# xiaochuanle/hifimeth

Measured on AMD Instinct MI355X. Metric: cytosine sites/sec (CpG+CHG+CHH), higher is better.
Workload: dtype f16x3+f32acc

## Files before the change

### hifimeth_amd/_lib.py

```python
from __future__ import annotations

import ctypes as C
import os
import subprocess

HERE = os.path.dirname(os.path.abspath(__file__))
LIB_PATH = os.environ.get("HM_LIB_PATH") or os.path.join(HERE, "libhifimeth_hip.so")
CSRC = os.path.join(HERE, "csrc")
WEIGHTS_DIR = os.path.join(HERE, "weights")


class hm_call_t(C.Structure):
    _fields_ = [("read_id", C.c_int32), ("qoff", C.c_int32), ("strand", C.c_uint8), ("ctx", C.c_uint8),
                ("scaled_prob", C.c_uint8), ("reserved", C.c_uint8), ("p", C.c_float)]


class hm_read_t(C.Structure):
    _fields_ = [("read_id", C.c_int32), ("l_qseq", C.c_int32), ("flag", C.c_int32), ("width", C.c_uint8 * 4),
                ("seq4", C.c_void_p), ("kin", C.c_void_p * 4)]


class hm_timing_t(C.Structure):
    _fields_ = [("prep_ms", C.c_double), ("scan_ms", C.c_double), ("emit_ms", C.c_double), ("window_ms", C.c_double),
                ("front_ms", C.c_double * 3), ("tail_ms", C.c_double * 3),
                ("prep_launches", C.c_int64), ("scan_launches", C.c_int64), ("emit_launches", C.c_int64),
                ("window_launches", C.c_int64), ("front_launches", C.c_int64 * 3), ("tail_launches", C.c_int64 * 3),
                ("front_sites", C.c_int64 * 3), ("window_sites", C.c_int64),
                ("pack_ms", C.c_double), ("empty_ms", C.c_double),
                ("pack_launches", C.c_int64), ("empty_launches", C.c_int64),
                ("trunk_ms", C.c_double * 3), ("edge_ms", C.c_double * 3),
                ("trunk_launches", C.c_int64 * 3), ("edge_launches", C.c_int64 * 3),
                ("trunk_positions", C.c_int64 * 3),
                ("trunk_list_steps", C.c_int64 * 3), ("trunk_const_steps", C.c_int64 * 3),
                ("group_bases", C.c_int64), ("group_bytes", C.c_int64), ("tail_strip_passes", C.c_int64)]


HM_ABI_VERSION = 5


def build(force: bool = False) -> str:
    if force:
        subprocess.check_call(["make", "-C", CSRC, "clean"], stdout=subprocess.DEVNULL)
    subprocess.check_call(["make", "-C", CSRC], stdout=subprocess.DEVNULL)
    return LIB_PATH


_lib = None


def lib():
    global _lib
    if _lib is not None:
        return _lib
    if not os.path.exists(LIB_PATH):
        raise ImportError(f"{LIB_PATH} is missing: run `python -c 'import __graft_entry__ as g; g.build()'` "
                          "(hifimeth_amd has no CPU fallback)")
    try:
        import torch
    except ImportError:
        pass
    L = C.CDLL(LIB_PATH)
    vp, i32, i64, cp = C.c_void_p, C.c_int32, C.c_int64, C.c_char_p
    sig = {
        "hm_create": (C.c_int, [C.POINTER(vp), cp, C.c_int, C.c_int]),
        "hm_destroy": (None, [vp]),
        "hm_last_error": (cp, [vp]),
        "hm_set_option": (C.c_int, [vp, cp, i64]),
        "hm_submit_read": (C.c_int, [vp, i32, i32, i32, vp, vp, C.c_int, vp, C.c_int, vp, C.c_int, vp, C.c_int]),
        "hm_clear": (C.c_int, [vp]),
        "hm_upload": (C.c_int, [vp]),
        "hm_run": (C.c_int, [vp]),
        "hm_sync": (C.c_int, [vp]),
        "hm_num_sites": (i64, [vp, C.c_int]),
        "hm_fetch": (i64, [vp, vp, i64]),
        "hm_flush": (C.c_int, [vp]),
        "hm_drain": (i64, [vp, vp, i64]),
        "hm_batch_begin": (vp, [vp]),
        "hm_batch_submit_read": (C.c_int, [vp, i32, i32, i32, vp, vp, C.c_int, vp, C.c_int, vp, C.c_int, vp, C.c_int]),
        "hm_batch_submit_reads": (i64, [vp, vp, i64, C.c_int, vp]),
        "hm_trunk_mask_for_reads": (C.c_int, [vp, i64, C.c_int]),
        "hm_batch_staged_bases": (i64, [vp]),
        "hm_batch_enqueue": (C.c_int, [vp]),
        "hm_batch_done": (C.c_int, [vp]),
        "hm_batch_wait": (i64, [vp, C.POINTER(vp)]),
        "hm_batch_num_sites": (i64, [vp, C.c_int]),
        "hm_batch_release": (C.c_int, [vp]),
        "hm_scan_sites": (i64, [vp, C.c_int, vp, vp, vp, i64]),
        "hm_site_logits": (i64, [vp, C.c_int, vp, i64]),
        "hm_windows": (C.c_int, [vp, C.c_int, i64, i64, vp]),
        "hm_cnn_logits": (C.c_int, [vp, C.c_int, vp, i64, vp, vp, vp]),
        "hm_debug_layer": (i64, [vp, C.c_int, vp, C.c_int, vp, i64]),
        "hm_convert_model": (C.c_int, [cp, cp]),
        "hm_get_stamps": (C.c_int, [vp, C.POINTER(C.c_uint64), C.c_int]),
        "hm_get_timing": (C.c_int, [vp, C.POINTER(hm_timing_t)]),
        "hm_abi_version": (C.c_int, []),
        "hm_timing_size": (C.c_size_t, []),
        "hm_reset_timing": (C.c_int, [vp]),
        "hm_pileup_create": (C.c_int, [C.POINTER(vp), C.c_int]),
        "hm_pileup_destroy": (None, [vp]),
        "hm_pileup_last_error": (cp, [vp]),
        "hm_pileup_set_option": (C.c_int, [vp, cp, C.c_double]),
        "hm_pileup_set_reference": (C.c_int, [vp, i32, vp, vp]),
        "hm_pileup_use_planes": (C.c_int, [vp, vp, vp, vp]),
        "hm_pileup_planes": (C.c_int, [vp, C.POINTER(vp), C.POINTER(vp), C.POINTER(vp), C.POINTER(i64)]),
        "hm_pileup_submit_read": (C.c_int, [vp, C.c_uint32, i32, i32, i64, i32, i32, vp, i32, vp, i64, vp]),
        "hm_pileup_submit_read_hp": (C.c_int, [vp, C.c_uint32, i32, i32, i64, i32, i32, vp, i32, vp, i64, vp, i32]),
        "hm_pileup_submit_read_calls": (C.c_int, [vp, C.c_uint32, i32, i32, i64, i32, i32, vp, i32, vp, i64, vp, i32]),
        "hm_pileup_use_partition_planes": (C.c_int, [vp, i32, vp, vp]),
        "hm_pileup_partition_planes": (C.c_int, [vp, i32, C.POINTER(vp), C.POINTER(vp)]),
        "hm_pileup_run": (C.c_int, [vp]),
        "hm_pileup_num_records": (i64, [vp]),
        "hm_pileup_histograms": (C.c_int, [vp, vp]),
        "hm_pileup_fetch_records": (i64, [vp, vp, vp, vp, vp, i64]),
        "hm_pileup_label_histograms": (C.c_int, [vp, vp, i64, vp]),
        "hm_pileup_count": (C.c_int, [vp, vp]),
        "hm_pileup_fetch_loci": (i64, [vp, vp, vp, vp, i64, i64, i64, vp, i64]),
        "hm_pileup_fetch_asm": (i64, [vp, vp, vp, vp, vp, vp, i64, i64, i64, i32, vp, i64]),
        "hm_pileup_asm_histogram": (i64, [vp, vp, vp, vp, vp, vp, i64, i64, i64, i32, vp, vp, i64]),
        "hm_pileup_asm_bin_pvalues": (i64, [vp, vp, vp, i64]),
        "hm_asm_qvalues": (C.c_int, [vp, i64, vp, i64, vp, vp]),
        "hm_pileup_fetch_asm_q": (i64, [vp, vp, vp, vp, vp, vp, i64, i64, i64, i32, vp, i64, vp, vp, i64, vp, i64]),
        "hm_pileup_fetch_asm_regions": (i64, [vp, vp, vp, vp, vp, vp, i64, i64, i64, i32, i32, C.c_double, i64, i32, i32,
                                              C.POINTER(i64), vp, i64]),
        "hm_pileup_load_loci": (i64, [vp, i32, vp, i64]),
        "hm_pileup_group_sample": (C.c_int, [vp, i32]),
        "hm_pileup_load_sample_loci": (i64, [vp, vp, i64]),
        "hm_pileup_fetch_groups": (i64, [vp, i64, i64, i32, vp, i64]),
        "hm_pileup_group_planes": (C.c_int, [vp, i32, i64, i64, vp, vp]),
        "hm_group_qvalues": (C.c_int, [vp, i64, vp, vp]),
        "hm_dmr_fetch_regions": (i64, [vp, i64, i64, i32, i32, C.c_double, C.c_double, i64, i32, i32, C.POINTER(i64),
                                       C.POINTER(i64), vp, i64]),
        "hm_dmr_p_cutoff": (C.c_int, [vp, vp, i64, C.c_double, vp]),
        "hm_sample_geometry": (C.c_int, [vp]),
        "hm_sample_open": (C.c_int, [vp]),
        "hm_sample_load": (i64, [vp, vp, i64]),
        "hm_sample_fetch_sums": (i64, [vp, i64, i64, i32, vp]),
        "hm_sample_plane": (C.c_int, [vp, i32, i64, i64, vp]),
        "hm_sample_corr": (C.c_int, [vp, i64, vp, vp, vp]),
        "hm_sample_fetch_intervals": (i64, [vp, i64, i64, i32, i32, vp, vp, i64, vp]),
        "hm_sample_interval_test": (C.c_int, [vp, i64, i32, vp, i64, i32, vp]),
        "hm_sample_qvalues": (C.c_int, [vp, i64, vp]),
        "hm_pileup_control_sums": (C.c_int, [vp, vp, vp, vp, i64, i64, vp]),
        "hm_pileup_site_histogram": (i64, [vp, vp, vp, vp, i64, i64, i64, vp, vp, i64]),
        "hm_sites_table": (C.c_int, [vp, vp, vp, i64, vp, vp, vp, vp, vp]),
        "hm_pileup_fetch_sites": (i64, [vp, vp, vp, vp, i64, i64, i64, i32, vp, vp, vp, vp, vp, i64, vp, i64]),
        "hm_pileup_fetch_domains": (i64, [vp, vp, vp, vp, i64, i64, i64, i32, i64, i64, i64, i64, C.POINTER(i64), vp, i64]),
        "hm_pileup_fetch_domains_part": (i64, [vp, vp, vp, vp, i64, i64, i64, i32, i64, i64, i64, i64, i32, vp, vp, i64]),
        "hm_domain_scores": (C.c_int, [C.c_double, C.c_double, C.c_double, C.POINTER(i64), C.POINTER(i64), C.POINTER(i64)]),
        "hm_pileup_domain_sums": (i64, [vp, vp, vp, vp, i64, i64, i64, i32, i64, i64, i64, i64, C.POINTER(i64)]),
        "hm_pileup_domain_sums_part": (i64, [vp, vp, vp, vp, i64, i64, i64, i32, i64, i64, i64, i64, vp, C.POINTER(i64)]),
        "hm_domain_refit": (C.c_int, [C.POINTER(i64), C.c_double, C.POINTER(C.c_double), C.POINTER(C.c_double)]),
        "hm_pileup_num_pattern_records": (i64, [vp]),
        "hm_pileup_fetch_patterns": (i64, [vp, i64, i64, i64, vp, i64]),
        "hm_pattern_stats": (C.c_int, [vp, vp]),
        "hm_pileup_fetch_bedmethyl": (i64, [vp, i32, i64, i64, i64, vp, i64]),
        "hm_pileup_fetch_linkage": (i64, [vp, i64, vp, i64]),
        "hm_linkage_stats": (C.c_int, [vp, vp]),
        "hm_pileup_fetch_readpos": (i64, [vp, i64, vp, i64]),
        "hm_pileup_readpos_histograms": (i64, [vp, vp, i64]),
        "hm_pileup_add_readpos": (C.c_int, [vp, vp, i64]),
        "hm_readpos_stats": (C.c_int, [vp, vp]),
        "hm_region_geometry": (C.c_int, [vp]),
        "hm_pileup_fetch_regions": (C.c_int, [vp, vp, vp, vp, i64, i64, i64, i64, vp, vp, i64, vp]),
        "hm_pileup_fetch_metaplot": (C.c_int, [vp, vp, vp, vp, i64, i64, i64, i64, vp, vp, vp, vp, vp, i64, i32, i64, i32, vp,
                                               C.POINTER(i64)]),
        "hm_region_stats": (C.c_int, [vp, vp]),
        "hm_context_geometry": (C.c_int, [vp]),
        "hm_pileup_fetch_context": (i64, [vp, vp, vp, vp, i64, i64, i64, i64, i32, vp, i64]),
        "hm_pileup_fetch_context_path": (i64, [vp, vp, vp, vp, i64, i64, i64, i64, i32, i32, vp, i64]),
    }
    for name, (res, args) in sig.items():
        fn = getattr(L, name)
        fn.restype = res
        fn.argtypes = args
    L._hm_symbols = tuple(sig)
    if L.hm_abi_version() != HM_ABI_VERSION or L.hm_timing_size() != C.sizeof(hm_timing_t):
        raise ImportError(f"{LIB_PATH}: ABI {L.hm_abi_version()} / hm_timing_t {L.hm_timing_size()} bytes, this package expects "
                          f"{HM_ABI_VERSION} / {C.sizeof(hm_timing_t)}: rebuild (python -c 'import __graft_entry__ as g; g.build()')")
    _lib = L
    return L
```

### hifimeth_amd/caller.py

```python
from __future__ import annotations

import ctypes as C
from typing import Iterable, Optional

import numpy as np

from . import _lib

CPG, CHG, CHH = 0, 1, 2
CTX_NAMES = ("CpG", "CHG", "CHH")
KMER, FEATS = 401, 8

READ_DTYPE = np.dtype([("read_id", "<i4"), ("l_qseq", "<i4"), ("flag", "<i4"), ("width", "u1", 4), ("seq4", "<u8"),
                       ("kin", "<u8", 4)], align=True)
assert READ_DTYPE.itemsize == C.sizeof(_lib.hm_read_t)

CALL_DTYPE = np.dtype([("read_id", "<i4"), ("qoff", "<i4"), ("strand", "u1"), ("ctx", "u1"),
                       ("scaled_prob", "u1"), ("reserved", "u1"), ("p", "<f4")])
assert CALL_DTYPE.itemsize == C.sizeof(_lib.hm_call_t) == 16


class HifimethError(RuntimeError):
    pass


def parse_contexts(spec: str) -> int:
    mask = 0
    for tok in spec.lower().split(","):
        tok = tok.strip()
        if tok not in ("cpg", "chg", "chh"):
            raise ValueError(f"unknown methylation context '{tok}'")
        mask |= 1 << ("cpg", "chg", "chh").index(tok)
    return mask


def _vp(a: Optional[np.ndarray]):
    return None if a is None else a.ctypes.data_as(C.c_void_p)


class MethylationCaller:
    def __init__(self, model_dir: Optional[str] = None, contexts: str = "cpg,chg,chh", device: int = 0,
                 min_read_size: int = 1000, timing: bool = False):
        self._L = _lib.lib()
        self._h = C.c_void_p()
        self.ctx_mask = parse_contexts(contexts)
        rc = self._L.hm_create(C.byref(self._h), (model_dir or _lib.WEIGHTS_DIR).encode(), self.ctx_mask, device)
        if rc < 0:
            self._h = None
            raise HifimethError(f"hm_create failed ({rc}): {self._L.hm_last_error(None).decode()}")
        self.set_option("min_read_size", min_read_size)
        self.set_option("timing", int(timing))

    def close(self):
        if getattr(self, "_h", None):
            self._L.hm_destroy(self._h)
            self._h = None

    __del__ = close

    def __enter__(self):
        return self

    def __exit__(self, *exc):
        self.close()

    def _check(self, rc, what):
        if rc < 0:
            raise HifimethError(f"{what} failed ({rc}): {self._L.hm_last_error(self._h).decode()}")
        return rc

    def set_option(self, key: str, value: int):
        self._check(self._L.hm_set_option(self._h, key.encode(), int(value)), f"hm_set_option({key})")

    def new_sample(self):
        self.set_option("trunk", 2)

    @staticmethod
    def _read_args(read):
        arrs, widths = [], []
        for nm in ("fi", "fp", "ri", "rp"):
            a = getattr(read, nm)
            if a is not None:
                if len(a) != read.l_qseq:
                    a = None
                else:
                    a = np.ascontiguousarray(a)
                    if a.dtype.itemsize not in (1, 2):
                        raise ValueError("kinetics arrays must be uint8 (B:C) or uint16 (B:S)")
            arrs.append(a)
            widths.append(1 if a is None else a.dtype.itemsize)
        seq4 = np.ascontiguousarray(read.seq4, np.uint8)
        return (read.l_qseq, read.flag, _vp(seq4), _vp(arrs[0]), widths[0], _vp(arrs[1]), widths[1],
                _vp(arrs[2]), widths[2], _vp(arrs[3]), widths[3]), (seq4, arrs)

    def submit(self, read_id: int, read) -> bool:
        args, _keep = self._read_args(read)
        return bool(self._check(self._L.hm_submit_read(self._h, read_id, *args), "hm_submit_read"))

    def submit_all(self, reads: Iterable, first_id: int = 0) -> int:
        n = 0
        for i, r in enumerate(reads):
            n += self.submit(first_id + i, r)
        return n

    def clear(self):
        self._check(self._L.hm_clear(self._h), "hm_clear")

    def upload(self):
        self._check(self._L.hm_upload(self._h), "hm_upload")

    def run(self):
        self._check(self._L.hm_run(self._h), "hm_run")

    def sync(self):
        self._check(self._L.hm_sync(self._h), "hm_sync")

    def num_sites(self, ctx: int = 3) -> int:
        return self._check(self._L.hm_num_sites(self._h, ctx), "hm_num_sites")

    def fetch(self) -> np.ndarray:
        self.sync()
        n = self.num_sites(3)
        out = np.empty(n, CALL_DTYPE)
        got = self._check(self._L.hm_fetch(self._h, _vp(out), n), "hm_fetch")
        return out[:got]

    def call(self, reads: Iterable, first_id: int = 0) -> np.ndarray:
        self.clear()
        self.submit_all(reads, first_id)
        self.upload()
        self.run()
        out = self.fetch()
        self.clear()
        return out

    def begin_batch(self) -> "Batch":
        h = self._L.hm_batch_begin(self._h)
        if not h:
            raise HifimethError(f"hm_batch_begin failed: {self._L.hm_last_error(self._h).decode()}")
        return Batch(self, h)

    def stream(self, slabs: Iterable, on_batch=None) -> int:
        inflight, total, k_done = [], 0, 0

        def collect(b):
            nonlocal total, k_done
            calls = b.wait()
            total += len(calls)
            if on_batch is not None:
                on_batch(k_done, b, calls)
            k_done += 1
            b.release()

        for slab in slabs:
            b = self.begin_batch()
            if isinstance(slab, ReadBlock):
                b.submit_block(slab, self.stage_threads)
            else:
                b.submit_all(slab)
            b.enqueue()
            inflight.append(b)
            while len(inflight) > 1 and (inflight[0].done() or len(inflight) >= self.max_inflight):
                collect(inflight.pop(0))
        while inflight:
            collect(inflight.pop(0))
        return total

    max_inflight = 3
    stage_threads = 4

    def scan_sites(self, ctx: int):
        self.sync()
        n = self.num_sites(ctx)
        rid, qoff, strand = np.empty(n, np.int32), np.empty(n, np.int32), np.empty(n, np.uint8)
        self._check(self._L.hm_scan_sites(self._h, ctx, _vp(rid), _vp(qoff), _vp(strand), n), "hm_scan_sites")
        return rid, qoff, strand

    def site_logits(self, ctx: int) -> np.ndarray:
        self.sync()
        n = self.num_sites(ctx)
        out = np.empty((n, 2), np.float32)
        got = self._check(self._L.hm_site_logits(self._h, ctx, _vp(out), n), "hm_site_logits")
        return out[:got]

    def windows(self, ctx: int, first: int = 0, n: Optional[int] = None, fetch: bool = True):
        if n is None:
            n = self.num_sites(ctx) - first
        out = np.empty((n, KMER, FEATS), np.float32) if fetch else None
        self._check(self._L.hm_windows(self._h, ctx, first, n, _vp(out)), "hm_windows")
        return out

    def cnn_logits(self, ctx: int, windows: np.ndarray):
        w = np.ascontiguousarray(windows, np.float32).reshape(-1, KMER, FEATS)
        n = w.shape[0]
        lg, p, ml = np.empty((n, 2), np.float32), np.empty(n, np.float32), np.empty(n, np.uint8)
        self._check(self._L.hm_cnn_logits(self._h, ctx, _vp(w), n, _vp(lg), _vp(p), _vp(ml)), "hm_cnn_logits")
        return lg, p, ml

    def debug_layer(self, ctx: int, window: np.ndarray, layer: int) -> np.ndarray:
        w = np.ascontiguousarray(window, np.float32).reshape(KMER, FEATS)
        out = np.empty(197 * 128, np.float32)
        n = self._check(self._L.hm_debug_layer(self._h, ctx, _vp(w), layer, _vp(out), out.size), "hm_debug_layer")
        chans = (8, 128, 128, 128, 96, 96, 96, 64, 64)[layer]
        return out[:n].reshape(-1, chans).copy()

    def stamps(self) -> list:
        buf = (C.c_uint64 * 256)()
        n = self._check(self._L.hm_get_stamps(self._h, buf, 256), "hm_get_stamps")
        return [int(buf[i]) for i in range(n)]

    def timing(self, reset: bool = False) -> dict:
        t = _lib.hm_timing_t()
        self._check(self._L.hm_get_timing(self._h, C.byref(t)), "hm_get_timing")
        d = {k: (list(getattr(t, k)) if hasattr(getattr(t, k), "__len__") else getattr(t, k)) for k, _ in t._fields_}
        if reset:
            self._L.hm_reset_timing(self._h)
        return d


def trunk_mask_for_reads(block: "ReadBlock", ctx_mask: int = 7) -> int:
    rc = _lib.lib().hm_trunk_mask_for_reads(block.desc.ctypes.data_as(C.c_void_p), len(block.desc), ctx_mask)
    if rc < 0:
        raise HifimethError(f"hm_trunk_mask_for_reads failed ({rc})")
    return rc


class ReadBlock:

    def __init__(self, reads, first_id: int = 0):
        self.reads = list(reads)
        self.desc = np.zeros(len(self.reads), READ_DTYPE)
        self._keep = []
        for i, r in enumerate(self.reads):
            d = self.desc[i]
            d["read_id"], d["l_qseq"], d["flag"] = first_id + i, r.l_qseq, r.flag
            seq4 = np.ascontiguousarray(r.seq4, np.uint8)
            d["seq4"] = seq4.ctypes.data
            self._keep.append(seq4)
            for k, nm in enumerate(("fi", "fp", "ri", "rp")):
                a = getattr(r, nm)
                if a is None or len(a) != r.l_qseq:
                    d["kin"][k], d["width"][k] = 0, 1
                    continue
                a = np.ascontiguousarray(a)
                if a.dtype.itemsize not in (1, 2):
                    raise ValueError("kinetics arrays must be uint8 (B:C) or uint16 (B:S)")
                d["kin"][k], d["width"][k] = a.ctypes.data, a.dtype.itemsize
                self._keep.append(a)

    def __len__(self):
        return len(self.reads)


class Batch:

    def __init__(self, mc: MethylationCaller, handle):
        self._mc, self._L, self._h = mc, mc._L, C.c_void_p(handle)

    def submit(self, read_id: int, read) -> bool:
        args, _keep = MethylationCaller._read_args(read)
        return bool(self._mc._check(self._L.hm_batch_submit_read(self._h, read_id, *args), "hm_batch_submit_read"))

    def submit_all(self, reads: Iterable, first_id: int = 0) -> int:
        n = 0
        for i, r in enumerate(reads):
            n += self.submit(first_id + i, r)
        return n

    def submit_block(self, block: "ReadBlock", threads: int = 4) -> int:
        rc = self._L.hm_batch_submit_reads(self._h, block.desc.ctypes.data_as(C.c_void_p), len(block.desc), threads, None)
        return self._mc._check(rc, "hm_batch_submit_reads")

    def staged_bases(self) -> int:
        return self._L.hm_batch_staged_bases(self._h)

    def enqueue(self):
        self._mc._check(self._L.hm_batch_enqueue(self._h), "hm_batch_enqueue")

    def done(self) -> bool:
        return bool(self._mc._check(self._L.hm_batch_done(self._h), "hm_batch_done"))

    def num_sites(self, ctx: int = 3) -> int:
        return self._mc._check(self._L.hm_batch_num_sites(self._h, ctx), "hm_batch_num_sites")

    def wait(self) -> np.ndarray:
        ptr = C.c_void_p()
        n = self._mc._check(self._L.hm_batch_wait(self._h, C.byref(ptr)), "hm_batch_wait")
        if n == 0:
            return np.empty(0, CALL_DTYPE)
        buf = (C.c_char * (n * CALL_DTYPE.itemsize)).from_address(ptr.value)
        return np.frombuffer(buf, CALL_DTYPE, n)

    def release(self):
        if self._h:
            self._L.hm_batch_release(self._h)
            self._h = None
```

### hifimeth_amd/csrc/hm_edge.h

```cpp
#pragma once
#include "hm_convh.h"

namespace hm {

namespace {

constexpr int TR_RS = 136;
constexpr int TR_WRS = 8;

__device__ __forceinline__ uint4 feature_row(int b, uint32_t k, int view) {
    uint4 row = make_uint4(0u, 0u, 0u, 0u);
    if (b < 0) return row;
    if (view) {
        if (b < 4) b = 3 - b;
        k = (k >> 16) | (k << 16);
    }
    row.x = b == 0 ? 0x3c00u : b == 1 ? 0x3c000000u : 0u;
    row.y = b == 2 ? 0x3c00u : b == 3 ? 0x3c000000u : 0u;
    half_t f[4];
#pragma unroll
    for (int c = 0; c < 4; ++c) {
        const uint32_t tt = (k >> (8 * c)) & 255u;
        f[c] = (half_t)((float)((int)(((tt & 63u) + 64u) << (tt >> 6)) - 64) * 0.03125f);
    }
    row.z = (uint32_t)__builtin_bit_cast(uint16_t, f[0]) | ((uint32_t)__builtin_bit_cast(uint16_t, f[1]) << 16);
    row.w = (uint32_t)__builtin_bit_cast(uint16_t, f[2]) | ((uint32_t)__builtin_bit_cast(uint16_t, f[3]) << 16);
    return row;
}

template <int K1>
struct EdgeGeo {
    static constexpr int L1 = (KMER + 2 - K1) / 2 + 1, L2 = (L1 - 1) / 2 + 1, L3 = (L2 - 1) / 2 + 1;
    static constexpr bool PAD2 = 2 * (L2 - 1) + 1 == L1, PAD3 = 2 * (L3 - 1) + 1 == L2, PAD4 = 2 * (C4_LEN - 1) + 1 == L3;
    static constexpr int R1 = -201 + 2 * (2 * (L2 - 1) - 1), R2 = -203 + 4 * (2 * (L3 - 1) - 1), R3 = -207 + 8 * (2 * (C4_LEN - 1) - 1);
    static constexpr int LEFT = -199;
    static constexpr int X_LEFT = -201, X_RIGHT = -201 + 2 * (L1 - 1);
};
static_assert(EdgeGeo<11>::PAD2 && EdgeGeo<11>::PAD3 && !EdgeGeo<11>::PAD4 && EdgeGeo<11>::R1 == 189 && EdgeGeo<11>::R2 == 185 && EdgeGeo<11>::R3 == 169, "k1 = 11 edge geometry");
static_assert(!EdgeGeo<13>::PAD2 && !EdgeGeo<13>::PAD3 && EdgeGeo<13>::PAD4 && EdgeGeo<13>::R1 == 185 && EdgeGeo<13>::R2 == 177 && EdgeGeo<13>::R3 == 169, "k1 = 13 edge geometry");


constexpr int EG_S = 32, EG_M = 2 * EG_S;
constexpr int EG_XROWS = 16;
constexpr int EG_OP = EG_M * 3 * TR_RS;
constexpr int EG_SP = EG_M * TR_RS;
constexpr int EG_XH = EG_M * EG_XROWS * TR_WRS;

struct EdgeSite {
    int64_t bo;
    int64_t vrow;
    int L, off, view, valid;
};

enum { SRC_ZERO = 0, SRC_SPEC = 1, SRC_MAP = 2 };
struct TapSrc {
    int kind, delta;
};

template <int K1>
__device__ __forceinline__ TapSrc tap_source(int layer, int side, int tap) {
    using G = EdgeGeo<K1>;
    if (side == 0) return tap == 0 ? TapSrc{SRC_ZERO, 0} : tap == 1 ? TapSrc{SRC_SPEC, 0} : TapSrc{SRC_MAP, G::LEFT};
    const bool pad = layer == 2 ? G::PAD2 : layer == 3 ? G::PAD3 : G::PAD4;
    const int r = layer == 2 ? G::R1 : layer == 3 ? G::R2 : G::R3, step = layer == 2 ? 2 : layer == 3 ? 4 : 8;
    if (pad) return tap == 0 ? TapSrc{SRC_MAP, r} : tap == 1 ? TapSrc{SRC_SPEC, 0} : TapSrc{SRC_ZERO, 0};
    return tap == 0 ? TapSrc{SRC_MAP, r} : tap == 1 ? TapSrc{SRC_MAP, r + step} : TapSrc{SRC_SPEC, 0};
}

struct EpiSpec {
    half_t* hi;
    half_t* lo;
    const float* __restrict__ bias;
    __device__ __forceinline__ void operator()(int m, int col, const f32x4& acc) const {
        half4 h, l;
        split4(acc, h, l);
        *reinterpret_cast<half4*>(hi + m * TR_RS + col) = h;
        *reinterpret_cast<half4*>(lo + m * TR_RS + col) = l;
    }
};

struct EpiSpecC1 {
    half_t* hi;
    half_t* lo;
    const float* __restrict__ bias;
    float4 c0, c1;
    __device__ __forceinline__ void operator()(int m, int col, const f32x4& acc) const {
        const float4 c = m >= EG_S ? c1 : c0;
        half4 h, l;
        split4(f32x4{acc[0] - c.x, acc[1] - c.y, acc[2] - c.z, acc[3] - c.w}, h, l);
        *reinterpret_cast<half4*>(hi + m * TR_RS + col) = h;
        *reinterpret_cast<half4*>(lo + m * TR_RS + col) = l;
    }
};

struct EpiEdgeOut {
    half_t* __restrict__ out;
    const float* __restrict__ bias;
    int nvalid;
    __device__ __forceinline__ void operator()(int m, int col, const f32x4& acc) const {
        const int side = m >= EG_S, site = m - side * EG_S;
        if (site < nvalid) {
            half4 h, l;
            split4(acc, h, l);
            half_t* o = out + (size_t)site * (4 * C4_CH) + side * (2 * C4_CH) + col;
            *reinterpret_cast<half4*>(o) = h;
            *reinterpret_cast<half4*>(o + C4_CH) = l;
        }
    }
};


}

}
```

### hifimeth_amd/csrc/hm_edge2.hip

```cpp
#include "hm_edge.h"
#ifdef HM_TRUNK_STAMP
#include "hm_stamp.h"
namespace hm { __device__ unsigned long long g_edge2_stamp[8][16]; }
extern "C" int hm_debug_edge2_stamps(unsigned long long* out, int reset) {
    if (out && hipMemcpyFromSymbol(out, HIP_SYMBOL(hm::g_edge2_stamp), sizeof(hm::g_edge2_stamp)) != hipSuccess) return -1;
    if (reset) {
        static unsigned long long z[8][16];
        if (hipMemcpyToSymbol(HIP_SYMBOL(hm::g_edge2_stamp), z, sizeof(z)) != hipSuccess) return -1;
    }
    return 0;
}
#endif

namespace hm {

namespace {

constexpr int E2_NW = 8;
constexpr int E2_MROWS = 3 * EG_S;
constexpr int E2_SLACK = 256;
constexpr int E2_MRS = 264;
constexpr int E2_MSET = E2_MROWS * E2_MRS + E2_SLACK;
constexpr int E2_SPLANE = EG_M * TR_RS;
constexpr int E2_XRS = EG_XROWS * TR_WRS + 8;
constexpr int E2_XH = EG_M * E2_XRS;
constexpr int E2_AHEAD = 2;
static_assert(E2_MRS * 2 == 33 * 16, "a map-set row is 33 sixteen-byte chunks (32 + pad)");

template <int I, int N, class F>
__device__ __forceinline__ void e2_for(F&& f) {
    if constexpr (I < N) {
        f(std::integral_constant<int, I>{});
        e2_for<I + 1, N>(f);
    }
}

__device__ __forceinline__ void e2_barrier() {
    __builtin_amdgcn_fence(__ATOMIC_RELEASE, "workgroup", "local");
    __builtin_amdgcn_s_barrier();
    __builtin_amdgcn_fence(__ATOMIC_ACQUIRE, "workgroup", "local");
}
template <int N>
__device__ __forceinline__ void e2_vmwait() {
    __builtin_amdgcn_s_waitcnt(0x0F70 | (N & 15) | ((N >> 4) << 14));
}

template <int K1, int LAYER>
struct E2L {
    using G = EdgeGeo<K1>;
    static constexpr bool PAD = LAYER == 2 ? G::PAD2 : LAYER == 3 ? G::PAD3 : G::PAD4;
    static constexpr int R = LAYER == 2 ? G::R1 : LAYER == 3 ? G::R2 : G::R3, STEP = LAYER == 2 ? 2 : LAYER == 3 ? 4 : 8;
    static constexpr int COUT = LAYER == 4 ? C4_CH : 128;
    static constexpr int ROWS = PAD ? 2 * EG_S : 3 * EG_S;
    static constexpr int NI = (ROWS * 33 + 63) / 64;
    static constexpr int kind(int side, int tap) {
        if (side == 0) return tap == 0 ? SRC_ZERO : tap == 1 ? SRC_SPEC : SRC_MAP;
        if (PAD) return tap == 0 ? SRC_MAP : tap == 1 ? SRC_SPEC : SRC_ZERO;
        return tap == 2 ? SRC_SPEC : SRC_MAP;
    }
    static constexpr int map_j(int side, int tap) { return side == 1 && !PAD && tap == 1 ? 1 : 0; }
    static constexpr bool live(int side, int kb) { return kind(side, kb / 4) != SRC_ZERO; }
    static constexpr int nblocks() { int n = 0; for (int kb = 0; kb < 12; ++kb) n += live(1, kb) + live(0, kb); return n; }
    static constexpr int NB = nblocks();
    static constexpr int find(int b, bool want_side) {
        int n = 0;
        for (int kb = 0; kb < 12; ++kb)
            for (int s = 1; s >= 0; --s)
                if (live(s, kb) && n++ == b) return want_side ? s : kb;
        return -1;
    }
    static constexpr int side_of(int b) { return find(b, true); }
    static constexpr int kb_of(int b) { return find(b, false); }
    static constexpr int dies_at(int b) { return b + 1 < NB && kb_of(b + 1) == kb_of(b) ? -1 : kb_of(b); }
};
static_assert(E2L<13, 2>::NB == 20 && E2L<13, 4>::NB == 16 && E2L<11, 4>::NB == 20 && E2L<13, 2>::kb_of(4) == 4 && E2L<13, 2>::side_of(5) == 0 &&
              E2L<13, 2>::dies_at(4) == -1 && E2L<13, 2>::dies_at(5) == 4 && E2L<13, 4>::kb_of(15) == 11 && E2L<11, 2>::NB == 16 && E2L<11, 2>::side_of(15) == 0 && E2L<11, 2>::kb_of(15) == 11,
              "edge layer schedules");

struct E2Site {
    int64_t vrow;
    int32_t off, L;
    int64_t bo;
    int32_t view, valid;
};

}

template <int K1>
__global__ __launch_bounds__(512) void edge2_kernel(SiteRange sr, const RInfo* __restrict__ rinfo, const uint8_t* __restrict__ bases,
                                                     const uint32_t* __restrict__ kin, CtxWeights W, TrunkMaps mp,
                                                     uint16_t* __restrict__ edge4, int32_t* __restrict__ e4row) {
    using G = EdgeGeo<K1>;
    constexpr int NW = E2_NW;
    const Site* sites;
    const int n_sites = resolve_sites(sr, sites);
    __shared__ __attribute__((aligned(16))) half_t smem[2 * E2_MSET + 2 * E2_SPLANE + E2_XH];
    __shared__ E2Site sinfo2[2][EG_S];
    __shared__ int32_t rowtab[2][3][E2_MROWS];
    half_t* mset = smem;
    half_t* sp_hi = smem + 2 * E2_MSET;
    half_t* sp_lo = sp_hi + E2_SPLANE;
    half_t* xb = sp_lo + E2_SPLANE;
    if ((int)blockIdx.x * EG_S >= n_sites) return;
    int tid = threadIdx.x, lane = tid & 63, wave = __builtin_amdgcn_readfirstlane(tid >> 6);
    int li = lane & 15, lk = lane >> 4;
    auto wf = [&](int i) { return reinterpret_cast<const half_t*>(W.wfrag_h[i]); };
    const uint32_t lds_mset = (uint32_t)(uintptr_t)(const __attribute__((address_space(3))) half_t*)mset;

    struct Desc {
        Site st;
        RInfo ri;
        int bs, valid;
    } nd;
    auto desc_a = [&](const int s0) __attribute__((always_inline)) {
        const int sc = min(s0, max(n_sites - 1, 0));
        const int nvalid = s0 < n_sites ? min(EG_S, n_sites - s0) : 0;
        const int t = tid & (EG_S - 1);
        nd.valid = t < nvalid;
        nd.st = sites[min(sc + t, max(n_sites - 1, 0))];
    };
    auto desc_b = [&]() __attribute__((always_inline)) { nd.ri = rinfo[nd.st.read_idx]; };
    auto desc_c = [&]() __attribute__((always_inline)) { nd.bs = bases[nd.ri.base_off + nd.st.qoff]; };
    auto desc_d = [&](const int s0, E2Site* si, int32_t (*rt)[E2_MROWS]) __attribute__((always_inline)) {
        if (tid < EG_S) {
            E2Site es;
            es.bo = nd.ri.base_off;
            es.L = nd.ri.len;
            es.view = nd.bs == 2;
            es.off = es.view ? nd.ri.len - 1 - nd.st.qoff : nd.st.qoff;
            es.vrow = (int64_t)es.view * mp.view_rows + nd.ri.map_off + TR_PAD;
            es.valid = nd.valid;
            si[tid] = es;
            if (es.valid) e4row[s0 + tid] = (int32_t)(es.vrow + es.off - 215);
        }
        if (tid < 3 * E2_MROWS) {
            const int l = tid / E2_MROWS, j = (tid - l * E2_MROWS) >> 5;
            const int view = nd.bs == 2, off = view ? nd.ri.len - 1 - nd.st.qoff : nd.st.qoff;
            const int r0 = l == 0 ? G::R1 : l == 1 ? G::R2 : G::R3, step = 2 << l;
            const int delta = j == 0 ? G::LEFT : r0 + (j - 1) * step;
            (&rt[0][0])[tid] = (int32_t)((int64_t)view * mp.view_rows + nd.ri.map_off + TR_PAD + off + delta);
        }
    };
    auto build_rows = [&](const E2Site* si, const int t, auto nt_, auto between) __attribute__((always_inline)) {
        constexpr int NT = decltype(nt_)::value, NR = EG_M * EG_XROWS / NT, PER = EG_XROWS / NR;
        static_assert(NR >= 1 && NR <= EG_XROWS && EG_XROWS % NR == 0, "a thread's rows lie in one pseudo-row");
        const int row = t / PER, t0 = (t - row * PER) * NR;
        const int side = row >= EG_S, site = row - side * EG_S;
        const E2Site es = si[site];
        uint32_t b[NR], k[NR];
        bool live[NR];
#pragma unroll
        for (int u = 0; u < NR; ++u) {
            const int tt = t0 + u;
            const int x = es.off + (side ? G::X_RIGHT : G::X_LEFT) + tt;
            const bool is_pad = side ? tt == K1 - 1 : tt == 0;
            live[u] = tt < K1 && !is_pad && x >= 0 && x < es.L;
            const int xc = min(max(x, 0), es.L - 1);
            const int64_t j = es.bo + (es.view ? es.L - 1 - xc : xc);
            b[u] = bases[j];
            k[u] = kin[j];
        }
        between();
#pragma unroll
        for (int u = 0; u < NR; ++u)
            *reinterpret_cast<uint4*>(xb + row * E2_XRS + (t0 + u) * TR_WRS) = feature_row(live[u] ? (int)b[u] : -1, k[u], es.view);
    };

    struct DmaSrc {
        int32_t rn;
        uint32_t ch;
    };
    auto dma_src = [&](auto ltag, const int32_t* rt, const int i) __attribute__((always_inline)) {
        using L = E2L<K1, decltype(ltag)::value>;
        const uint32_t c = (uint32_t)min(i, L::NI - 1) * 64u + (uint32_t)lane;
        const uint32_t row = (c * 1986u) >> 16;
        const uint32_t ch = min(c - 33u * row, 31u);
        return DmaSrc{rt[min(row, (uint32_t)(L::ROWS - 1))], ch};
    };
    auto dma_issue = [&](auto ltag, const DmaSrc& d, const int set, const int i) __attribute__((always_inline)) {
        using L = E2L<K1, decltype(ltag)::value>;
        const char* __restrict__ map = reinterpret_cast<const char*>(mp.e[decltype(ltag)::value - 2]);
        if (i < L::NI) {
            const char* src = map + (uint64_t)((uint32_t)d.rn * 32u + d.ch) * 16u;
            const uint32_t dst = __builtin_amdgcn_readfirstlane(lds_mset + (uint32_t)((set * E2_MSET) * 2 + i * 1024));
            uint32_t km;
            asm volatile(
                "s_mov_b32 %0, m0\n\t"
                "s_mov_b32 m0, %1\n\t"
                "s_nop 0\n\t"
                "global_load_lds_dwordx4 %2, off\n\t"
                "s_mov_b32 m0, %0"
                : "=&s"(km)
                : "s"(dst), "v"(src));
        }
    };
    auto dma_maps = [&](auto ltag, const int32_t* rt, const int set, const int w0, auto nw_) __attribute__((always_inline)) {
        using L = E2L<K1, decltype(ltag)::value>;
        constexpr int nw = decltype(nw_)::value;
#pragma unroll
        for (int t = 0; t < (L::NI + nw - 1) / nw; ++t) dma_issue(ltag, dma_src(ltag, rt, w0 + nw * t), set, w0 + nw * t);
    };
    using L2t = std::integral_constant<int, 2>;
    using L3t = std::integral_constant<int, 3>;
    using L4t = std::integral_constant<int, 4>;
    using NW8 = std::integral_constant<int, 8>;

    constexpr int KB1 = (2 * K1 + 3) / 4 * 4 * 8 / 32;
    struct Head1 {
        half8 w[KB1];
        float4 bz;
    };
    auto load_head1 = [&](Head1& h) __attribute__((always_inline)) {
        const char* wp = reinterpret_cast<const char*>(W.c1f) + (size_t)wave * (KB1 * 1024);
        const uint32_t lo = (uint32_t)lane * 16u;
#pragma unroll
        for (int kb = 0; kb < KB1; ++kb) h.w[kb] = *reinterpret_cast<const half8*>(wp + kb * 1024 + lo);
        const int col = wave * 16 + 4 * lk;
        h.bz = *reinterpret_cast<const float4*>(W.c1f_bias + col);
    };
    auto conv1 = [&](const Head1& h) __attribute__((always_inline)) {
        const float4 c0 = *reinterpret_cast<const float4*>(W.c1f_corr + wave * 16 + 4 * lk);
        const float4 c1 = *reinterpret_cast<const float4*>(W.c1f_corr + 128 + wave * 16 + 4 * lk);
        f32x4 acc[4];
#pragma unroll
        for (int i = 0; i < 4; ++i) acc[i] = f32x4{h.bz.x, h.bz.y, h.bz.z, h.bz.w};
        auto stack_off = [&](int kb) __attribute__((always_inline)) {
            int t = 4 * kb + lk;
            t = t >= 2 * K1 ? 0 : t >= K1 ? t - K1 : t;
            return t * TR_WRS;
        };
        const int a0 = li * E2_XRS;
        half8 x[2][4];
#pragma unroll
        for (int i = 0; i < 4; ++i) x[0][i] = *reinterpret_cast<const half8*>(xb + a0 + i * (16 * E2_XRS) + stack_off(0));
#pragma unroll
        for (int kb = 0; kb < KB1; ++kb) {
            if (kb + 1 < KB1) {
                const int bo = stack_off(kb + 1);
#pragma unroll
                for (int i = 0; i < 4; ++i) x[(kb + 1) & 1][i] = *reinterpret_cast<const half8*>(xb + a0 + i * (16 * E2_XRS) + bo);
            }
#pragma unroll
            for (int i = 0; i < 4; ++i) acc[i] = __builtin_amdgcn_mfma_f32_16x16x32_f16(h.w[kb], x[kb & 1][i], acc[i], 0, 0, 0);
        }
        const EpiSpecC1 epi{sp_hi, sp_lo, nullptr, c0, c1};
#pragma unroll
        for (int i = 0; i < 4; ++i) epi(i * 16 + li, wave * 16 + 4 * lk, acc[i]);
    };

    struct LW {
        half8 w[12][2];
        float4 bz;
    };
    auto wptr = [&](auto ltag) __attribute__((always_inline)) {
        constexpr int LAYER = decltype(ltag)::value;
        const int nt = LAYER == 4 ? min(wave, C4_CH / 16 - 1) : wave;
        return reinterpret_cast<const char*>(wf(LAYER - 1)) + (size_t)nt * (12 * 128 * 16);
    };
    auto load_kb = [&](auto ltag, auto kb_, LW& lw) __attribute__((always_inline)) {
        constexpr int LAYER = decltype(ltag)::value, kb = decltype(kb_)::value;
        const char* wp = wptr(ltag) + kb * 2048;
        const uint32_t lo = (uint32_t)lane * 16u;
        lw.w[kb][0] = *reinterpret_cast<const half8*>(wp + lo);
        lw.w[kb][1] = *reinterpret_cast<const half8*>(wp + 1024 + lo);
        if constexpr (kb == 0) lw.bz = *reinterpret_cast<const float4*>(W.bias[LAYER - 1] + (LAYER == 4 ? min(wave, C4_CH / 16 - 1) : wave) * 16 + 4 * lk);
    };
    auto layer = [&](auto ltag, const LW& lw, const half_t* mx, f32x4 (&acc)[4], auto slide, auto job) __attribute__((always_inline)) {
        constexpr int LAYER = decltype(ltag)::value;
        using L = E2L<K1, LAYER>;
#pragma unroll
        for (int i = 0; i < 4; ++i) acc[i] = f32x4{lw.bz.x, lw.bz.y, lw.bz.z, lw.bz.w};
        const int a0 = li * TR_RS + 8 * lk;
        const int am = li * E2_MRS + 8 * lk;
        constexpr int LA = 2, NX = LA + 1;
        half8 x[NX][2][2];
        auto reads = [&](auto b_) __attribute__((always_inline)) {
            constexpr int b = decltype(b_)::value, side = L::side_of(b), kb = L::kb_of(b), tap = kb / 4, q = kb % 4;
            constexpr int kind = L::kind(side, tap);
            static_assert(kind != SRC_ZERO, "live taps only");
#pragma unroll
            for (int i = 0; i < 2; ++i) {
                if constexpr (kind == SRC_MAP) {
                    const int o = am + ((2 * side + i) * 16 + 32 * L::map_j(side, tap)) * E2_MRS + 32 * q;
                    x[b % NX][i][0] = *reinterpret_cast<const half8*>(mx + o);
                    x[b % NX][i][1] = *reinterpret_cast<const half8*>(mx + o + 128);
                } else {
                    const int o = a0 + ((2 * side + i) * 16) * TR_RS + 32 * q;
                    x[b % NX][i][0] = *reinterpret_cast<const half8*>(sp_hi + o);
                    x[b % NX][i][1] = *reinterpret_cast<const half8*>(sp_lo + o);
                }
            }
        };
        e2_for<0, E2_AHEAD>(slide);
        e2_for<0, LA>(reads);
        e2_for<0, L::NB>([&](auto b_) __attribute__((always_inline)) {
            constexpr int b = decltype(b_)::value, side = L::side_of(b), kb = L::kb_of(b);
            if constexpr (b + LA < L::NB) reads(std::integral_constant<int, (b + LA < L::NB ? b + LA : 0)>{});
            job(b_);
#pragma unroll
            for (int pr = 0; pr < 3; ++pr)
#pragma unroll
                for (int i = 0; i < 2; ++i)
                    acc[2 * side + i] = __builtin_amdgcn_mfma_f32_16x16x32_f16(lw.w[kb][pr == 2 ? 1 : 0], x[b % NX][i][pr == 1 ? 1 : 0],
                                                                               acc[2 * side + i], 0, 0, 0);
            constexpr int dead = L::dies_at(b);
            constexpr bool sl = dead >= 0 && dead + E2_AHEAD < 12;
            if constexpr (sl) slide(std::integral_constant<int, (sl ? dead + E2_AHEAD : 0)>{});
            {
                constexpr int NRD = b + LA < L::NB ? 4 : 0;
#pragma unroll
                for (int r = 0; r < NRD; ++r) {
                    __builtin_amdgcn_sched_group_barrier(0x008, 1, 0);
                    __builtin_amdgcn_sched_group_barrier(0x100, 1, 0);
                }
                if (sl) {
                    __builtin_amdgcn_sched_group_barrier(0x008, 1, 0);
                    __builtin_amdgcn_sched_group_barrier(0x020, 2, 0);
                }
            }
            __builtin_amdgcn_sched_barrier(0);
        });
    };

#ifdef HM_TRUNK_STAMP
    unsigned long long ets[16], eacc[16] = {};
    unsigned long long en_it = 0, e_prev = 0;
    const bool est_on = blockIdx.x == 0;
#define ETS(i) do { if (est_on) ets[i] = hm_stamp(); } while (0)
#else
#define ETS(i)
#endif

    Head1 h1;
    LW lw;
    {
        const int s0 = blockIdx.x * EG_S;
        desc_a(s0);
        desc_b();
        desc_c();
        desc_d(s0, sinfo2[0], rowtab[0]);
        load_head1(h1);
        __syncthreads();
        build_rows(sinfo2[0], tid, std::integral_constant<int, NW * 64>{}, [] {});
        e2_vmwait<0>();
        dma_maps(L2t{}, rowtab[0][0], 0, wave, NW8{});
        e2_vmwait<0>();
    }
    int cur = 0, sel = 0;
    for (int s0 = blockIdx.x * EG_S; s0 < n_sites; s0 += gridDim.x * EG_S) {
        const int nvalid = min(EG_S, n_sites - s0);
        const E2Site* si_next = sinfo2[cur ^ 1];
        const half_t* mA = mset + (size_t)sel * E2_MSET;
        const half_t* mB = mset + (size_t)(sel ^ 1) * E2_MSET;
        tid = threadIdx.x;
        asm volatile("" : "+v"(tid));
        lane = tid & 63, wave = __builtin_amdgcn_readfirstlane(tid >> 6), li = lane & 15, lk = lane >> 4;
        e2_barrier();
        ETS(0);
#ifdef HM_TRUNK_STAMP
        if (est_on && e_prev) eacc[9] += ets[0] - e_prev;
#endif
        const int sn = s0 + gridDim.x * EG_S;
        desc_a(sn);
        e2_for<0, 12>([&](auto k_) __attribute__((always_inline)) { load_kb(L2t{}, k_, lw); });
        conv1(h1);
        ETS(1);
        e2_vmwait<0>();
        e2_barrier();
        ETS(2);
        f32x4 acc[4];
        desc_b();
        {
            LW ln;
            DmaSrc ds;
            layer(L2t{}, lw, mA, acc, [&](auto k_) __attribute__((always_inline)) { load_kb(L3t{}, k_, ln); },
                  [&](auto b_) __attribute__((always_inline)) {
                      constexpr int b = decltype(b_)::value, NP = (E2L<K1, 3>::NI + NW - 1) / NW;
                      static_assert(NP < E2L<K1, 2>::NB, "the pieces fit the layer's blocks");
                      if constexpr (b >= 1 && b - 1 < NP) dma_issue(L3t{}, ds, sel ^ 1, wave + NW * (b - 1));
                      if constexpr (b < NP) ds = dma_src(L3t{}, rowtab[cur][1], wave + NW * b);
                  });
            ETS(3);
            e2_vmwait<0>();
            e2_barrier();
            ETS(4);
            const EpiSpec epi{sp_hi, sp_lo, nullptr};
#pragma unroll
            for (int i = 0; i < 4; ++i) epi(i * 16 + li, wave * 16 + 4 * lk, acc[i]);
            lw = ln;
        }
        e2_barrier();
        ETS(5);
        desc_c();
        {
            LW ln;
            DmaSrc ds;
            layer(L3t{}, lw, mB, acc, [&](auto k_) __attribute__((always_inline)) { load_kb(L4t{}, k_, ln); },
                  [&](auto b_) __attribute__((always_inline)) {
                      constexpr int b = decltype(b_)::value, NP = (E2L<K1, 4>::NI + NW - 1) / NW;
                      static_assert(NP < E2L<K1, 3>::NB, "the pieces fit the layer's blocks");
                      if constexpr (b >= 1 && b - 1 < NP) dma_issue(L4t{}, ds, sel, wave + NW * (b - 1));
                      if constexpr (b < NP) ds = dma_src(L4t{}, rowtab[cur][2], wave + NW * b);
                  });
            ETS(6);
            e2_vmwait<0>();
            e2_barrier();
            ETS(7);
            const EpiSpec epi{sp_hi, sp_lo, nullptr};
#pragma unroll
            for (int i = 0; i < 4; ++i) epi(i * 16 + li, wave * 16 + 4 * lk, acc[i]);
            desc_d(sn, sinfo2[cur ^ 1], rowtab[cur ^ 1]);
            lw = ln;
        }
        e2_barrier();
        ETS(8);
        if (wave >= C4_CH / 16) {
            build_rows(si_next, tid - 64 * (C4_CH / 16), std::integral_constant<int, 128>{}, [&]() __attribute__((always_inline)) { load_head1(h1); });
        } else {
            DmaSrc ds;
            constexpr int NWC = C4_CH / 16;
            layer(L4t{}, lw, mA, acc, [&](auto k_) __attribute__((always_inline)) {
                if constexpr (decltype(k_)::value == 11) load_head1(h1);
            }, [&](auto b_) __attribute__((always_inline)) {
                constexpr int b = decltype(b_)::value, NP = (E2L<K1, 2>::NI + NWC - 1) / NWC;
                static_assert(NP < E2L<K1, 4>::NB, "the pieces fit the layer's blocks");
                if constexpr (b >= 1 && b - 1 < NP) dma_issue(L2t{}, ds, sel ^ 1, wave + NWC * (b - 1));
                if constexpr (b < NP) ds = dma_src(L2t{}, rowtab[cur ^ 1][0], wave + NWC * b);
            });
            const EpiEdgeOut epi{reinterpret_cast<half_t*>(edge4) + (size_t)s0 * (4 * C4_CH), nullptr, nvalid};
#pragma unroll
            for (int i = 0; i < 4; ++i) epi(i * 16 + li, wave * 16 + 4 * lk, acc[i]);
        }
        ETS(9);
        e2_vmwait<0>();
        cur ^= 1;
        sel ^= 1;
#ifdef HM_TRUNK_STAMP
        if (est_on) {
            for (int i = 0; i < 9; ++i) eacc[i] += ets[i + 1] - ets[i];
            e_prev = ets[9];
            ++en_it;
        }
#endif
    }
#ifdef HM_TRUNK_STAMP
    if (est_on && (threadIdx.x & 63) == 0) {
        for (int i = 0; i < 10; ++i) atomicAdd(&g_edge2_stamp[threadIdx.x >> 6][i], eacc[i]);
        atomicAdd(&g_edge2_stamp[threadIdx.x >> 6][10], en_it);
    }
#endif
#undef ETS
}

void launch_edge2(hipStream_t st, int k1, const SiteRange& sr, const RInfo* rinfo, const uint8_t* bases, const uint32_t* kin,
                  const CtxWeights& w, const TrunkMaps& maps, uint16_t* edge4, int32_t* e4row, int grid) {
    if (sr.cap <= 0) return;
    const dim3 g(sr.totals ? grid : max(1, min((sr.cap + EG_S - 1) / EG_S, grid))), b(512);
    if (k1 == 11) hipLaunchKernelGGL(edge2_kernel<11>, g, b, 0, st, sr, rinfo, bases, kin, w, maps, edge4, e4row);
    else hipLaunchKernelGGL(edge2_kernel<13>, g, b, 0, st, sr, rinfo, bases, kin, w, maps, edge4, e4row);
}

}
```

### hifimeth_amd/csrc/hm_engine.cpp

```cpp
#include <hip/hip_runtime.h>

#include <algorithm>
#include <atomic>
#include <cmath>
#include <condition_variable>
#include <cstdio>
#include <cstring>
#include <memory>
#include <mutex>
#include <string>
#include <thread>
#include <vector>

#include "../../include/hifimeth_hip.h"
#include "hm_device.h"
#include "hm_host.h"
#include "hm_kernels.h"
#include "hm_weights.h"

using namespace hm;

namespace {

thread_local std::string g_create_error;

enum Kind { K_PREP, K_SCAN, K_EMIT, K_PACK, K_WINDOW, K_FRONT, K_TAIL, K_TRUNK, K_EDGE, K_TAILG };

struct TimedSpan {
    int kind, ctx;
    int64_t off, cap;
    Event a, b;
};

struct DeviceModel {
    bool loaded = false;
    int k1 = 0;
    DevBuf params;
    CtxWeights w{};
};

}

struct hm_batch {
    hm_engine* e = nullptr;
    int id = 0;
    enum State { FREE, STAGING, QUEUED } state = FREE;
    bool uploaded = false, ran = false, have_totals = false, have_calls = false;
    Stream s_io;
    Event ev_in, ev_comp, ev_out;

    PinnedArr<uint8_t> slab;
    PinnedArr<ReadDesc> reads;
    PinnedArr<Chunk> chunks;
    PinnedArr<RInfo> rinfo;
    PinnedArr<TrunkTile> tiles;
    PinnedArr<int32_t> tcost;
    struct Group {
        int chunk_lo, chunk_hi, tile_lo, tile_hi;
        int64_t bases, rows;
        int cost_lo;
    };
    std::vector<Group> groups;
    int64_t total_bases = 0;

    DevBuf d_raw, d_reads, d_chunks, d_rinfo, d_tiles, d_tcost, d_bases, d_kin, d_sctx, d_counts, d_offs, d_totals, d_err;
    DevBuf d_usites, d_utag, d_csites, d_opos, d_logits, d_p, d_ml, d_calls;
    Pinned<int32_t> h_totals;
    Pinned<int32_t> h_err;
    PinnedArr<hm_call_t> h_calls;
    int32_t totals[TOT_COUNT] = {};

    std::vector<TimedSpan> spans;

    ~hm_batch() {
        if (s_io) (void)hipStreamSynchronize(s_io);
    }
};

namespace {

struct GroupBufs {
    DevBuf d_map[3], d_e4, d_edge4, d_e4row, d_rowlist;
    DevBuf d_x6;
    DevBuf d_mark, d_ccnt, d_order, d_okey;
    DevBuf d_odst;
    DevBuf d_x8;
    DevBuf d_dump;
    int64_t bytes() const {
        const DevBuf* all[] = {&d_map[0], &d_map[1], &d_map[2], &d_e4, &d_edge4, &d_e4row, &d_rowlist, &d_x6, &d_mark, &d_ccnt, &d_order, &d_okey, &d_odst, &d_x8, &d_dump};
        static_assert(sizeof(GroupBufs) == sizeof all / sizeof *all * sizeof(DevBuf), "a member of GroupBufs is missing from bytes()");
        int64_t sum = 0;
        for (const DevBuf* d : all) sum += (int64_t)d->cap;
        return sum;
    }
};

}

struct hm_engine {
    int device = 0;
    int num_cu = 256;
    int ctx_mask = 7;
    int min_read_size = 1000;
    int64_t sub_batch = 65536;
    int front_waves = 8;
    int precision = 1;
    int conv3_w16 = 0;
    int max_slots = 3;
    int trunk = 2;
    int trunk_impl = 3;
    int edge_impl = 1;
    int tail_impl = 3;
    int64_t tail_slice = int64_t(1) << 21;
    int trunk_mask_auto = -1;
    int64_t group_bases = 0;
    std::atomic<int64_t> group_bases_eff{0};
    bool stamps_on = false;
    std::vector<unsigned long long> stamp_sum;
    bool timing = false;
    std::string err;

    std::mutex mu;
    std::mutex order_mu;
    std::condition_variable cv;
    hm_timing_t acc{};
    int64_t x6_sites = 0;

    Stream stream;
    std::vector<Event> pool;
    DevBuf d_act4, d_win, d_dbg, d_stamps, d_zeros;
    GroupBufs grp;
    DeviceModel model[3];
    std::vector<std::unique_ptr<hm_batch>> slots;

    ~hm_engine() {
        (void)hipSetDevice(device);
        if (stream) (void)hipStreamSynchronize(stream);
    }
};

namespace {

constexpr int64_t GROUP_BYTES_PER_BASE = (3 * 2 * 512 + 2 * 384 + 768 + 4 + 8 + 2 * 4 + 8 + 4 + TAIL_STRIP_HANDOVER_BYTES) * 5 / 4;

int64_t effective_group_bases(hm_engine* e) {
    if (e->group_bases > 0) return e->group_bases;
    if (const int64_t have = e->group_bases_eff.load(std::memory_order_relaxed)) return have;
    size_t free_b = 0, total_b = 0;
    int64_t gb = int64_t(2) << 20;
    int prev = -1;
    (void)hipGetDevice(&prev);
    if (hipSetDevice(e->device) == hipSuccess && hipMemGetInfo(&free_b, &total_b) == hipSuccess && free_b > 0) {
        gb = (int64_t)(free_b / 4) / GROUP_BYTES_PER_BASE;
        gb = std::min<int64_t>(gb, int64_t(16) << 20);
        gb = std::max<int64_t>(gb >> 20 << 20, int64_t(1) << 20);
    }
    if (prev >= 0 && prev != e->device) (void)hipSetDevice(prev);
    int64_t none = 0;
    if (!e->group_bases_eff.compare_exchange_strong(none, gb, std::memory_order_relaxed)) gb = none;
    return gb;
}

constexpr int TILE_COST = 8, TILE_COST_CONST = 1;
void add_read_tiles(hm_engine* e, hm_batch* b, int ridx, int l_qseq) {
    if (b->groups.empty() || b->groups.back().rows >= effective_group_bases(e)) {
        b->groups.push_back(hm_batch::Group{(int)b->chunks.n, (int)b->chunks.n, (int)b->tiles.n, (int)b->tiles.n, 0, 0, (int)b->tcost.n});
        b->tcost.push_back(0);
    }
    hm_batch::Group& g = b->groups.back();
    const int ntile = (l_qseq + 2 * TR_PAD + TR_OWN - 1) / TR_OWN;
    b->rinfo.push_back(RInfo{b->total_bases, l_qseq, (int32_t)g.rows});
    for (int t = 0; t < ntile; ++t) {
        const int u0 = -TR_PAD + t * TR_OWN;
        b->tiles.push_back(TrunkTile{ridx, u0});
        b->tcost.push_back(b->tcost.p[b->tcost.n - 1] + (t == 0 ? 2 * TILE_COST_CONST : u0 >= l_qseq ? TILE_COST_CONST : TILE_COST));
    }
    for (int st = 0; st < l_qseq; st += CHUNK) b->chunks.push_back(Chunk{ridx, st});
    g.rows += (int64_t)ntile * TR_OWN + TR_SLACK;
    if (2 * g.rows >= (int64_t(1) << 27)) throw HipErr{hipErrorInvalidValue, "a read group's maps exceed 2^27 rows (group_bases too large)"};
    g.bases += l_qseq;
    g.chunk_hi = (int)b->chunks.n;
    g.tile_hi = (int)b->tiles.n;
}

int fail(hm_engine* e, int code, const std::string& msg) {
    if (e) {
        std::lock_guard<std::mutex> lk(e->mu);
        e->err = msg;
    } else {
        g_create_error = msg;
    }
    return code;
}

int fail_hip(hm_engine* e, const HipErr& h) {
    return fail(e, HM_EDEVICE, hip_error_text(h));
}

template <class Body>
auto guarded(hm_engine* e, Body&& body) -> decltype(body()) {
    return hip_guard(e->device, [e](const HipErr& h) { return fail_hip(e, h); }, body);
}

Event get_event(hm_engine* e) {
    Event ev;
    {
        std::lock_guard<std::mutex> lk(e->mu);
        if (!e->pool.empty()) {
            ev = std::move(e->pool.back());
            e->pool.pop_back();
            return ev;
        }
    }
    HIP_TRY(hipEventCreate(&ev.h));
    return ev;
}

struct Span {
    hm_engine* e;
    std::vector<TimedSpan>* sink;
    TimedSpan ts{};
    bool on;
    Span(hm_engine* eng, std::vector<TimedSpan>* out, int kind, int ctx = 0, int64_t off = 0, int64_t cap = 0)
        : e(eng), sink(out), on(eng->timing && out) {
        if (!on) return;
        ts.kind = kind;
        ts.ctx = ctx;
        ts.off = off;
        ts.cap = cap;
        ts.a = get_event(e);
        ts.b = get_event(e);
        HIP_TRY(hipEventRecord(ts.a, e->stream));
    }
    void end() {
        if (!on) return;
        HIP_TRY(hipEventRecord(ts.b, e->stream));
        sink->push_back(std::move(ts));
        on = false;
    }
};

void collect_timing(hm_engine* e, std::vector<TimedSpan>& spans, const int32_t* totals) {
    if (!spans.empty() && totals) {
        std::lock_guard<std::mutex> lk(e->mu);
        for (int c = 0; c < 3; ++c) e->acc.trunk_list_steps[c] += totals[TOT_LIST_STEPS + c];
        for (int c = 0; c < 3; ++c) e->acc.trunk_const_steps[c] += totals[TOT_CONST_STEPS + c];
        e->acc.tail_strip_passes += totals[TOT_STRIP_PASSES];
    }
    for (auto& s : spans) {
        float ms = 0.f;
        HIP_TRY(hipEventElapsedTime(&ms, s.a, s.b));
        std::lock_guard<std::mutex> lk(e->mu);
        hm_timing_t& t = e->acc;
        const int64_t n = totals ? std::clamp<int64_t>((int64_t)totals[s.ctx] - s.off, 0, s.cap) : s.cap;
        switch (s.kind) {
        case K_PREP: t.prep_ms += ms; ++t.prep_launches; break;
        case K_SCAN: t.scan_ms += ms; ++t.scan_launches; break;
        case K_EMIT: t.emit_ms += ms; ++t.emit_launches; break;
        case K_PACK: t.pack_ms += ms; ++t.pack_launches; break;
        case K_WINDOW: t.window_ms += ms; ++t.window_launches; t.window_sites += s.cap; break;
        case K_TRUNK: t.trunk_ms[s.ctx] += ms; ++t.trunk_launches[s.ctx]; t.trunk_positions[s.ctx] += s.cap; break;
        case K_EDGE: t.edge_ms[s.ctx] += ms; ++t.edge_launches[s.ctx]; break;
        case K_TAILG: t.tail_ms[s.ctx] += ms; ++t.tail_launches[s.ctx]; break;
        case K_FRONT:
            if (n > 0) { t.front_ms[s.ctx] += ms; ++t.front_launches[s.ctx]; t.front_sites[s.ctx] += n; }
            else { t.empty_ms += ms; ++t.empty_launches; }
            break;
        default:
            if (n > 0) { t.tail_ms[s.ctx] += ms; ++t.tail_launches[s.ctx]; }
            else { t.empty_ms += ms; ++t.empty_launches; }
            break;
        }
        e->pool.push_back(std::move(s.a));
        e->pool.push_back(std::move(s.b));
    }
    spans.clear();
}

void upload_model(hm_engine* e, int ctx, const HostModel& hmw) {
    DeviceModel& dm = e->model[ctx];
    PackedModel pk = pack_model(hmw);
    dm.params.reserve(pk.blob.size() * sizeof(float));
    HIP_TRY(hipMemcpy(dm.params.p, pk.blob.data(), pk.blob.size() * sizeof(float), hipMemcpyHostToDevice));
    const float* base = dm.params.as<float>();
    for (int i = 0; i < 9; ++i) {
        dm.w.wfrag[i] = base + pk.wfrag_off[i];
        dm.w.bias[i] = base + pk.bias_off[i];
    }
    dm.w.fc2_w = base + pk.fc2_w_off;
    dm.w.fc2_b = base + pk.fc2_b_off;
    dm.w.bn = reinterpret_cast<const BnTables*>(base + pk.bn_off);
    for (int i = 0; i < 9; ++i) dm.w.wfrag_h[i] = reinterpret_cast<const uint16_t*>(base + pk.wfrag_h_off[i]);
    dm.w.bn_h = reinterpret_cast<const BnTablesH*>(base + pk.bn_h_off);
    dm.w.c1f = reinterpret_cast<const uint16_t*>(base + pk.c1f_off);
    dm.w.c1f_bias = base + pk.c1f_bias_off;
    dm.w.c1f_corr = base + pk.c1f_corr_off;
    dm.w.k1 = hmw.k1;
    dm.k1 = hmw.k1;
    dm.loaded = true;
}

size_t align16(size_t x) { return (x + 15) & ~size_t(15); }

void accumulate_stamps(hm_engine* e) {
    const int ns = front_stamp_slots();
    const size_t n = (size_t)e->num_cu * 8 * ns;
    std::vector<unsigned long long> h(n);
    HIP_TRY(hipStreamSynchronize(e->stream));
    HIP_TRY(hipMemcpy(h.data(), e->d_stamps.p, n * sizeof(unsigned long long), hipMemcpyDeviceToHost));
    HIP_TRY(hipMemset(e->d_stamps.p, 0, n * sizeof(unsigned long long)));
    e->stamp_sum.resize((size_t)ns * 8, 0);
    for (size_t i = 0; i < n; ++i) e->stamp_sum[i % ((size_t)ns * 8)] += h[i];
}

void launch_cnn_pair(hm_engine* e, std::vector<TimedSpan>* spans, int ctx, const SiteRange& sr, const hm_batch* b,
                     const float* windows, float* logits, float* p, uint8_t* ml, float* dbg, int dbg_layer) {
    const DeviceModel& dm = e->model[ctx];
    const ReadDesc* reads = b ? b->d_reads.as<ReadDesc>() : nullptr;
    const uint8_t* bases = b ? b->d_bases.as<uint8_t>() : nullptr;
    const uint32_t* kin = b ? b->d_kin.as<uint32_t>() : nullptr;
    {
        Span sp(e, spans, K_FRONT, ctx, sr.off, sr.cap);
        if (e->precision >= 1)
            launch_front_h(e->stream, dm.k1, sr, reads, bases, kin, windows, dm.w, e->d_act4.as<float>(), e->num_cu, dbg,
                           dbg_layer, e->stamps_on ? e->d_stamps.as<unsigned long long>() : nullptr);
        else
            launch_front(e->stream, dm.k1, sr, reads, bases, kin, windows, dm.w, e->d_act4.as<float>(), e->num_cu, dbg,
                         dbg_layer, e->front_waves, e->stamps_on ? e->d_stamps.as<unsigned long long>() : nullptr);
        if (e->stamps_on) accumulate_stamps(e);
        sp.end();
    }
    {
        Span sp(e, spans, K_TAIL, ctx, sr.off, sr.cap);
        if (e->precision >= 1)
            launch_tail_h(e->stream, e->d_act4.as<float>(), sr, dm.w, logits, p, ml, e->num_cu, dbg, dbg_layer);
        else
            launch_tail(e->stream, e->d_act4.as<float>(), sr, dm.w, logits, p, ml, e->num_cu, dbg, dbg_layer);
        sp.end();
    }
}

void run_cnn_windows(hm_engine* e, int ctx, const float* windows, int64_t n, float* logits, float* p, uint8_t* ml,
                     float* dbg, int dbg_layer) {
    const int64_t sb = e->sub_batch;
    e->d_act4.reserve((size_t)std::min<int64_t>(std::max<int64_t>(n, 1), sb) * ACT4_FLOATS * sizeof(float));
    std::vector<TimedSpan> spans;
    for (int64_t off = 0; off < n; off += sb) {
        const int m = (int)std::min<int64_t>(sb, n - off);
        const SiteRange sr{nullptr, nullptr, ctx, 0, m};
        launch_cnn_pair(e, e->timing ? &spans : nullptr, ctx, sr, nullptr, windows + (size_t)off * KMER * FEATS,
                        logits + 2 * off, p + off, ml + off, dbg, dbg_layer);
    }
    HIP_TRY(hipGetLastError());
    HIP_TRY(hipStreamSynchronize(e->stream));
    collect_timing(e, spans, nullptr);
}

hm_batch* new_slot(hm_engine* e, int id) {
    std::unique_ptr<hm_batch> b(new hm_batch());
    b->e = e;
    b->id = id;
    HIP_TRY(hipStreamCreateWithFlags(&b->s_io.h, hipStreamNonBlocking));
    for (Event* ev : {&b->ev_in, &b->ev_comp, &b->ev_out}) HIP_TRY(hipEventCreateWithFlags(&ev->h, hipEventDisableTiming));
    b->h_totals.alloc(TOT_COUNT);
    b->h_err.alloc();
    b->d_totals.reserve(TOT_COUNT * sizeof(int32_t));
    b->d_err.reserve(sizeof(int32_t));
    HIP_TRY(hipMemset(b->d_err.p, 0, sizeof(int32_t)));
    HIP_TRY(hipMemset(b->d_totals.p, 0, TOT_COUNT * sizeof(int32_t)));
    hm_batch* raw = b.get();
    e->slots.push_back(std::move(b));
    return raw;
}

void reset_staging(hm_batch* b) {
    b->slab.n = 0;
    b->reads.n = 0;
    b->chunks.n = 0;
    b->rinfo.n = 0;
    b->tiles.n = 0;
    b->tcost.n = 0;
    b->groups.clear();
    b->total_bases = 0;
    b->uploaded = b->ran = b->have_totals = b->have_calls = false;
    memset(b->totals, 0, sizeof b->totals);
}


int check_read(hm_engine* e, const hm_read_t& r, int64_t tb, const char* who, const char* full) {
    if (r.l_qseq < 0) return fail(e, HM_EINVAL, std::string(who) + ": negative read length");
    if (r.l_qseq < e->min_read_size) return 0;
    if (r.l_qseq == 0) return 0;
    if (!r.kin[0] || !r.kin[1] || !r.kin[2] || !r.kin[3]) return 0;
    if (!r.seq4) return fail(e, HM_EINVAL, std::string(who) + ": seq4 is NULL");
    for (int k = 0; k < 4; ++k)
        if (r.width[k] != 1 && r.width[k] != 2) return fail(e, HM_EINVAL, "kinetics element width must be 1 (B:C) or 2 (B:S)");
    if (tb + (int64_t)r.l_qseq + 4 >= (int64_t(1) << 31)) return fail(e, HM_ENOMEM, std::string(who) + ": batch would exceed 2^31 bases; " + full);
    return 1;
}

int64_t padded_bases(int32_t l_qseq) { return ((int64_t)l_qseq + 3) & ~int64_t(3); }

struct SlabCopy {
    const void* src;
    size_t off, bytes;
};

void place_read(hm_batch* b, const hm_read_t& r, SlabCopy* copies) {
    const size_t L = (size_t)r.l_qseq;
    auto place = [&](const void* src, size_t bytes) {
        const int64_t off = (int64_t)b->slab.n;
        *copies++ = SlabCopy{src, (size_t)off, bytes};
        b->slab.n += align16(bytes);
        return off;
    };
    ReadDesc rd{};
    rd.off_seq = place(r.seq4, (L + 1) / 2);
    rd.off_fi = place(r.kin[0], L * r.width[0]);
    rd.off_fp = place(r.kin[1], L * r.width[1]);
    rd.off_ri = place(r.kin[2], L * r.width[2]);
    rd.off_rp = place(r.kin[3], L * r.width[3]);
    rd.base_off = b->total_bases;
    rd.len = r.l_qseq;
    rd.flag = r.flag;
    rd.read_id = r.read_id;
    for (int k = 0; k < 4; ++k) rd.w[k] = r.width[k];
    const int ridx = (int)b->reads.n;
    b->reads.push_back(rd);
    add_read_tiles(b->e, b, ridx, r.l_qseq);
    b->total_bases += padded_bases(r.l_qseq);
}

int stage_read(hm_batch* b, int32_t read_id, int32_t l_qseq, int32_t flag, const uint8_t* seq4, const void* fi, int fi_w,
               const void* fp, int fp_w, const void* ri, int ri_w, const void* rp, int rp_w) {
    auto width = [](int w) { return (uint8_t)std::clamp(w, 0, 255); };
    const hm_read_t r{read_id, l_qseq, flag, {width(fi_w), width(fp_w), width(ri_w), width(rp_w)}, seq4, {fi, fp, ri, rp}};
    const int rc = check_read(b->e, r, b->total_bases, "hm_submit_read", "flush / queue it first");
    if (rc <= 0) return rc;
    return guarded(b->e, [&] {
        const size_t L = (size_t)l_qseq;
        const size_t need = align16((L + 1) / 2) + align16(L * fi_w) + align16(L * fp_w) + align16(L * ri_w) + align16(L * rp_w);
        if (b->slab.n + need > b->slab.cap) b->slab.reserve(std::max<size_t>((b->slab.n + need) * 2, size_t(64) << 20));
        SlabCopy copies[5];
        place_read(b, r, copies);
        for (const SlabCopy& c : copies) memcpy(b->slab.p + c.off, c.src, c.bytes);
        return 1;
    });
}

void enqueue_upload(hm_batch* b) {
    const size_t nr = b->reads.n, nc = b->chunks.n;
    b->d_raw.reserve(std::max<size_t>(b->slab.n, 16));
    b->d_reads.reserve(std::max<size_t>(nr, 1) * sizeof(ReadDesc));
    b->d_chunks.reserve(std::max<size_t>(nc, 1) * sizeof(Chunk));
    const size_t tb = (size_t)std::max<int64_t>(b->total_bases, 4);
    b->d_bases.reserve(tb);
    b->d_sctx.reserve(tb);
    b->d_kin.reserve(tb * sizeof(uint32_t));
    b->d_counts.reserve((nc + 1) * NCNT * sizeof(int32_t));
    b->d_offs.reserve((nc + 1) * NCNT * sizeof(int32_t));
    b->d_usites.reserve(tb * sizeof(USite));
    b->d_utag.reserve(tb);
    b->d_csites.reserve(tb * sizeof(Site));
    b->d_opos.reserve(tb * sizeof(int32_t));
    b->d_logits.reserve(tb * 2 * sizeof(float));
    b->d_p.reserve(tb * sizeof(float));
    b->d_ml.reserve(tb);
    b->d_calls.reserve(tb * sizeof(hm_call_t));
    if (b->slab.n) HIP_TRY(hipMemcpyAsync(b->d_raw.p, b->slab.p, b->slab.n, hipMemcpyHostToDevice, b->s_io));
    if (nr) HIP_TRY(hipMemcpyAsync(b->d_reads.p, b->reads.p, nr * sizeof(ReadDesc), hipMemcpyHostToDevice, b->s_io));
    if (nc) HIP_TRY(hipMemcpyAsync(b->d_chunks.p, b->chunks.p, nc * sizeof(Chunk), hipMemcpyHostToDevice, b->s_io));
    b->d_rinfo.reserve(std::max<size_t>(nr, 1) * sizeof(RInfo));
    b->d_tiles.reserve(std::max<size_t>(b->tiles.n, 1) * sizeof(TrunkTile));
    if (nr) HIP_TRY(hipMemcpyAsync(b->d_rinfo.p, b->rinfo.p, nr * sizeof(RInfo), hipMemcpyHostToDevice, b->s_io));
    if (b->tiles.n) HIP_TRY(hipMemcpyAsync(b->d_tiles.p, b->tiles.p, b->tiles.n * sizeof(TrunkTile), hipMemcpyHostToDevice, b->s_io));
    b->d_tcost.reserve(std::max<size_t>(b->tcost.n, 1) * sizeof(int32_t));
    if (b->tcost.n) HIP_TRY(hipMemcpyAsync(b->d_tcost.p, b->tcost.p, b->tcost.n * sizeof(int32_t), hipMemcpyHostToDevice, b->s_io));
    HIP_TRY(hipEventRecord(b->ev_in, b->s_io));
    b->uploaded = true;
    b->ran = b->have_totals = b->have_calls = false;
}

void run_trunk_path(hm_batch* b, std::vector<TimedSpan>* spans, int ctx_mask) {
    hm_engine* e = b->e;
    int64_t max_rows = 1, max_bases = 1;
    for (const auto& g : b->groups) {
        max_rows = std::max(max_rows, g.rows);
        max_bases = std::max(max_bases, g.bases);
    }
    for (int i = 0; i < 3; ++i) e->grp.d_map[i].reserve((size_t)max_rows * 2 * 256 * sizeof(uint16_t));
    e->grp.d_e4.reserve((size_t)max_rows * 2 * C4_CH * sizeof(float));
    e->grp.d_rowlist.reserve(std::max((size_t)(max_rows / TR_OWN + 1) * 2 * 3 * TR_OWN, trunk3_rowlist_bytes((max_rows / TR_OWN + 1) * 2)));
    e->grp.d_dump.reserve(trunk3_dump_bytes(e->num_cu));
    e->grp.d_edge4.reserve((size_t)max_bases * 2 * C4_CH * sizeof(float));
    e->grp.d_e4row.reserve((size_t)max_bases * sizeof(int32_t));
    if (e->tail_impl == 3 && e->precision >= 1 && (ctx_mask >> CHH & 1)) {
        e->grp.d_mark.reserve(tail_strip_mark_bytes(2 * max_rows));
        e->grp.d_ccnt.reserve(tail_strip_count_bytes(2 * max_rows));
        e->grp.d_order.reserve((size_t)max_bases * sizeof(int32_t));
        e->grp.d_okey.reserve((size_t)max_bases * sizeof(int32_t));
        e->grp.d_odst.reserve((size_t)max_bases * sizeof(int32_t));
        e->grp.d_x8.reserve(tail_strip_handover_bytes(max_bases));
    }
    if (!e->d_zeros.p) {
        e->d_zeros.reserve(1024);
        HIP_TRY(hipMemsetAsync(e->d_zeros.p, 0, 1024, e->stream));
    }
    const int32_t* offs = b->d_offs.as<int32_t>();
    for (const auto& g : b->groups) {
        const TrunkMaps maps{{e->grp.d_map[0].as<uint16_t>(), e->grp.d_map[1].as<uint16_t>(), e->grp.d_map[2].as<uint16_t>()},
                             e->grp.d_e4.as<uint16_t>(), g.rows, e->d_zeros.as<uint16_t>(), e->grp.d_rowlist.as<uint8_t>()};
        const int n_tiles = g.tile_hi - g.tile_lo;
        for (int c = 0; c < 3; ++c) {
            if (!(ctx_mask >> c & 1)) continue;
            const DeviceModel& dm = e->model[c];
            const int n_views = c == CHH ? 2 : 1;
            const SiteRange sr{b->d_csites.as<Site>(), b->d_totals.as<int32_t>(), c, 0, (int32_t)std::min<int64_t>(g.bases, INT32_MAX),
                               offs + (size_t)NCNT * g.chunk_lo + c, offs + (size_t)NCNT * g.chunk_hi + c};
            if (e->precision == 0) {
                {
                    Span sp(e, spans, K_TRUNK, c, 0, (int64_t)n_tiles * TR_OWN * n_views);
                    launch_trunk_f32(e->stream, dm.k1, b->d_tiles.as<TrunkTile>() + g.tile_lo, n_tiles, n_views, c, b->d_rinfo.as<RInfo>(),
                                     b->d_bases.as<uint8_t>(), b->d_kin.as<uint32_t>(), b->d_sctx.as<uint8_t>(), dm.w, maps, e->num_cu);
                    sp.end();
                }
                {
                    Span sp(e, spans, K_EDGE, c);
                    launch_edge_f32(e->stream, dm.k1, sr, b->d_rinfo.as<RInfo>(), b->d_bases.as<uint8_t>(), b->d_kin.as<uint32_t>(), dm.w,
                                    maps, e->grp.d_edge4.as<float>(), e->grp.d_e4row.as<int32_t>(), e->num_cu);
                    sp.end();
                }
                Span sp(e, spans, K_TAILG, c);
                launch_tail_gather_f32(e->stream, sr, dm.w, maps, e->grp.d_edge4.as<float>(), e->grp.d_e4row.as<int32_t>(),
                                       b->d_logits.as<float>(), b->d_p.as<float>(), b->d_ml.as<uint8_t>(), e->num_cu);
                sp.end();
                continue;
            }
            {
                Span sp(e, spans, K_TRUNK, c, 0, (int64_t)n_tiles * TR_OWN * n_views);
                if (e->trunk_impl == 3)
                    launch_trunk3(e->stream, dm.k1, b->d_tiles.as<TrunkTile>() + g.tile_lo, n_tiles, n_views, c, b->d_rinfo.as<RInfo>(),
                                  b->d_bases.as<uint8_t>(), b->d_kin.as<uint32_t>(), b->d_sctx.as<uint8_t>(), b->total_bases, dm.w, maps, e->grp.d_dump.as<uint16_t>(),
                                  b->d_totals.as<int32_t>() + TOT_LIST_STEPS, b->d_tcost.as<int32_t>() + g.cost_lo, e->num_cu, e->conv3_w16 != 0);
                else if (e->trunk_impl)
                    launch_trunk2(e->stream, dm.k1, b->d_tiles.as<TrunkTile>() + g.tile_lo, n_tiles, n_views, c, b->d_rinfo.as<RInfo>(),
                                  b->d_bases.as<uint8_t>(), b->d_kin.as<uint32_t>(), b->d_sctx.as<uint8_t>(), dm.w, maps, e->num_cu,
                                  e->trunk_impl == 2);
                else
                    launch_trunk(e->stream, dm.k1, b->d_tiles.as<TrunkTile>() + g.tile_lo, n_tiles, n_views, c, b->d_rinfo.as<RInfo>(),
                                 b->d_bases.as<uint8_t>(), b->d_kin.as<uint32_t>(), b->d_sctx.as<uint8_t>(), dm.w, maps, e->num_cu);
                sp.end();
            }
            {
                Span sp(e, spans, K_EDGE, c);
                if (e->edge_impl == 1)
                    launch_edge2(e->stream, dm.k1, sr, b->d_rinfo.as<RInfo>(), b->d_bases.as<uint8_t>(), b->d_kin.as<uint32_t>(), dm.w,
                                 maps, e->grp.d_edge4.as<uint16_t>(), e->grp.d_e4row.as<int32_t>(), e->num_cu);
                else
                    launch_edge(e->stream, dm.k1, sr, b->d_rinfo.as<RInfo>(), b->d_bases.as<uint8_t>(), b->d_kin.as<uint32_t>(), dm.w,
                                maps, e->grp.d_edge4.as<uint16_t>(), e->grp.d_e4row.as<int32_t>(), e->num_cu);
                sp.end();
            }
            {
                Span sp(e, spans, K_TAILG, c);
                if (e->tail_impl == 2 && e->precision >= 1) {
                    const int64_t slice = std::min<int64_t>(e->tail_slice, std::max<int64_t>(max_bases, 1));
                    if (slice > e->x6_sites) {
                        e->grp.d_x6.reserve(tail_split_x6_bytes(slice));
                        HIP_TRY(hipMemsetAsync(e->grp.d_x6.p, 0, tail_split_x6_bytes(slice), e->stream));
                        e->x6_sites = slice;
                    }
                    const size_t ph = tail_split_x6_plane_halves(e->x6_sites);
                    for (int64_t off = 0; off < g.bases; off += e->x6_sites) {
                        SiteRange s2 = sr;
                        s2.off = (int32_t)off;
                        s2.cap = (int32_t)std::min<int64_t>(e->x6_sites, g.bases - off);
                        launch_tail_split(e->stream, s2, dm.w, maps, e->grp.d_edge4.as<uint16_t>() + (size_t)off * (4 * C4_CH),
                                          e->grp.d_e4row.as<int32_t>() + off, e->grp.d_x6.as<uint16_t>(), ph, b->d_logits.as<float>(),
                                          b->d_p.as<float>(), b->d_ml.as<uint8_t>(), e->num_cu);
                    }
                } else if (e->tail_impl == 3 && e->precision >= 1 && c == CHH) {
                    launch_tail_strip(e->stream, sr, dm.w, maps, n_views, e->grp.d_edge4.as<uint16_t>(), e->grp.d_e4row.as<int32_t>(), e->grp.d_mark.as<int32_t>(),
                                      e->grp.d_ccnt.as<int32_t>(), e->grp.d_order.as<int32_t>(), e->grp.d_okey.as<int32_t>(), e->grp.d_odst.as<int32_t>(), e->grp.d_x8.as<uint16_t>(),
                                      b->d_logits.as<float>(), b->d_p.as<float>(), b->d_ml.as<uint8_t>(), b->d_totals.as<int32_t>() + TOT_STRIP_PASSES, e->num_cu, e->precision == 2);
                } else if ((e->tail_impl == 1 || e->tail_impl == 3) && e->precision >= 1)
                    launch_tail_gather_r(e->stream, sr, dm.w, maps, e->grp.d_edge4.as<uint16_t>(), e->grp.d_e4row.as<int32_t>(),
                                         b->d_logits.as<float>(), b->d_p.as<float>(), b->d_ml.as<uint8_t>(), e->num_cu, e->precision == 2);
                else
                    launch_tail_gather(e->stream, sr, dm.w, maps, e->grp.d_edge4.as<uint16_t>(), e->grp.d_e4row.as<int32_t>(),
                                       b->d_logits.as<float>(), b->d_p.as<float>(), b->d_ml.as<uint8_t>(), e->num_cu);
                sp.end();
            }
        }
    }
}

struct SeqView {
    const uint8_t* sq;
    int len;
};
template <class Get>
int trunk_mask_from_sample(size_t n, Get get, int ctx_mask) {
    static const int8_t code[16] = {4, 0, 1, 4, 2, 4, 4, 4, 3, 4, 4, 4, 4, 4, 4, 4};
    int64_t cnt[3] = {0, 0, 0}, bases = 0;
    for (size_t r = 0; r < n && bases < (int64_t(4) << 20); ++r) {
        const SeqView v = get(r);
        if (!v.sq || v.len <= 0) continue;
        const uint8_t* sq = v.sq;
        const int L = v.len;
        auto at = [&](int i) { return (int)code[(sq[i >> 1] >> ((~i & 1) << 2)) & 15]; };
        int c0 = at(0), c1 = L > 1 ? at(1) : -1;
        for (int i = 0; i + 1 < L; ++i) {
            const int c2 = i + 2 < L ? at(i + 2) : -1;
            if (c0 == 1 && c1 == 2) ++cnt[CPG];
            if (c2 >= 0) {
                const bool h1 = c1 == 0 || c1 == 1 || c1 == 3, h2 = c2 == 0 || c2 == 1 || c2 == 3;
                if (c0 == 1 && h1 && c2 == 2) ++cnt[CHG];
                if (c0 == 1 && h1 && h2) ++cnt[CHH];
                else if ((c0 == 0 || c0 == 2 || c0 == 3) && (c1 == 0 || c1 == 2 || c1 == 3) && c2 == 2) ++cnt[CHH];
            }
            c0 = c1;
            c1 = c2;
        }
        bases += L;
    }
    int m = 0;
    for (int c = 0; c < 3; ++c)
        if ((ctx_mask >> c & 1) && bases > 0 && (double)cnt[c] >= (c == CHH ? 0.033 : 0.017) * (double)bases) m |= 1 << c;
    return m;
}

int trunk_mask_of(hm_batch* b) {
    hm_engine* e = b->e;
    if (e->trunk == 0) return 0;
    if (e->trunk == 1) return e->ctx_mask;
    std::lock_guard<std::mutex> lk(e->mu);
    if (e->trunk_mask_auto < 0) {
        if (b->reads.n == 0) return e->ctx_mask;
        e->trunk_mask_auto = trunk_mask_from_sample(
            b->reads.n, [&](size_t r) { return SeqView{b->slab.p + b->reads.p[r].off_seq, b->reads.p[r].len}; }, e->ctx_mask);
    }
    return e->trunk_mask_auto;
}

void enqueue_run(hm_batch* b) {
    hm_engine* e = b->e;
    std::vector<TimedSpan>* spans = e->timing ? &b->spans : nullptr;
    const int nc = (int)b->chunks.n;
    HIP_TRY(hipStreamWaitEvent(e->stream, b->ev_in, 0));
    {
        Span sp(e, spans, K_PREP);
        launch_prep(e->stream, b->d_raw.as<uint8_t>(), b->d_reads.as<ReadDesc>(), b->d_chunks.as<Chunk>(), nc, e->ctx_mask,
                    b->d_bases.as<uint8_t>(), b->d_kin.as<uint32_t>(), b->d_sctx.as<uint8_t>(), b->d_counts.as<int32_t>(),
                    b->d_err.as<int32_t>());
        sp.end();
    }
    {
        Span sp(e, spans, K_SCAN);
        launch_scan(e->stream, b->d_counts.as<int32_t>(), nc, b->d_offs.as<int32_t>(), b->d_totals.as<int32_t>());
        sp.end();
    }
    {
        Span sp(e, spans, K_EMIT);
        launch_emit(e->stream, b->d_reads.as<ReadDesc>(), b->d_chunks.as<Chunk>(), nc, e->ctx_mask, b->d_bases.as<uint8_t>(),
                    b->d_offs.as<int32_t>(), b->d_totals.as<int32_t>(), b->d_usites.as<USite>(), b->d_utag.as<uint8_t>(),
                    b->d_csites.as<Site>(), b->d_opos.as<int32_t>());
        sp.end();
    }
    const int trunk_mask = trunk_mask_of(b);
    if (trunk_mask) run_trunk_path(b, spans, trunk_mask);
    if ((e->ctx_mask & ~trunk_mask) != 0) {
    const int64_t bound = nc ? b->total_bases : 0;
    int64_t sb = std::max<int64_t>(e->sub_batch, (bound / 48 + TAIL_SITES) / TAIL_SITES * TAIL_SITES);
    sb = std::min<int64_t>(sb, int64_t(1) << 20);
    e->d_act4.reserve((size_t)std::min<int64_t>(std::max<int64_t>(bound, 1), sb) * ACT4_FLOATS * sizeof(float));
    for (int c = 0; c < 3; ++c) {
        if (!(e->ctx_mask >> c & 1) || (trunk_mask >> c & 1)) continue;
        for (int64_t off = 0; off < bound; off += sb) {
            const SiteRange sr{b->d_csites.as<Site>(), b->d_totals.as<int32_t>(), c, (int32_t)off,
                               (int32_t)std::min<int64_t>(sb, bound - off)};
            launch_cnn_pair(e, spans, c, sr, b, nullptr, b->d_logits.as<float>(), b->d_p.as<float>(), b->d_ml.as<uint8_t>(),
                            nullptr, 0);
        }
    }
    }
    {
        Span sp(e, spans, K_PACK);
        const int64_t bound = nc ? b->total_bases : 0;
        const int grid = (int)std::clamp<int64_t>((bound / 3 + 255) / 256, 1, (int64_t)e->num_cu * 8);
        launch_pack(e->stream, b->d_usites.as<USite>(), b->d_utag.as<uint8_t>(), b->d_opos.as<int32_t>(), b->d_p.as<float>(),
                    b->d_ml.as<uint8_t>(), b->d_reads.as<ReadDesc>(), b->d_totals.as<int32_t>(), b->d_calls.p, grid);
        sp.end();
    }
    HIP_TRY(hipGetLastError());
    HIP_TRY(hipEventRecord(b->ev_comp, e->stream));
    HIP_TRY(hipStreamWaitEvent(b->s_io, b->ev_comp, 0));
    HIP_TRY(hipMemcpyAsync(b->h_totals, b->d_totals.p, TOT_COUNT * sizeof(int32_t), hipMemcpyDeviceToHost, b->s_io));
    HIP_TRY(hipMemcpyAsync(b->h_err, b->d_err.p, sizeof(int32_t), hipMemcpyDeviceToHost, b->s_io));
    HIP_TRY(hipEventRecord(b->ev_out, b->s_io));
    b->ran = true;
    b->have_totals = b->have_calls = false;
}

int wait_totals(hm_batch* b) {
    hm_engine* e = b->e;
    if (!b->ran) return HM_OK;
    if (!b->have_totals) {
        HIP_TRY(hipEventSynchronize(b->ev_out));
        memcpy(b->totals, b->h_totals, sizeof b->totals);
        b->have_totals = true;
        collect_timing(e, b->spans, b->totals);
    }
    if (*b->h_err) {
        *b->h_err = 0;
        HIP_TRY(hipMemsetAsync(b->d_err.p, 0, sizeof(int32_t), b->s_io));
        HIP_TRY(hipStreamSynchronize(b->s_io));
        return fail(e, HM_EDATA, "illegal BAM base encoded value in a staged read");
    }
    return HM_OK;
}

int fetch_calls(hm_batch* b) {
    int rc = wait_totals(b);
    if (rc < 0) return rc;
    if (b->have_calls) return HM_OK;
    const size_t n = (size_t)b->totals[TOT_ALL];
    b->h_calls.reserve(std::max<size_t>(n, 1));
    if (n) {
        HIP_TRY(hipMemcpyAsync(b->h_calls.p, b->d_calls.p, n * sizeof(hm_call_t), hipMemcpyDeviceToHost, b->s_io));
        HIP_TRY(hipStreamSynchronize(b->s_io));
    }
    b->h_calls.n = n;
    b->have_calls = true;
    return HM_OK;
}

hm_batch* legacy(hm_engine* e) { return e->slots[0].get(); }

}

extern "C" {

int hm_create(hm_engine_t** out, const char* model_dir, int ctx_mask, int device) {
    if (!out || !model_dir || !(ctx_mask & 7)) return fail(nullptr, HM_EINVAL, "hm_create: bad argument");
    *out = nullptr;
    int ndev = 0;
    if (hipGetDeviceCount(&ndev) != hipSuccess || ndev <= 0 || device < 0 || device >= ndev)
        return fail(nullptr, HM_EDEVICE, "hm_create: no usable HIP device (this library has no CPU fallback)");
    std::unique_ptr<hm_engine> e(new hm_engine());
    e->device = device;
    const int rc = hip_guard(device, [](const HipErr& h) { return fail_hip(nullptr, h); }, [&] {
        hipDeviceProp_t prop;
        HIP_TRY(hipGetDeviceProperties(&prop, device));
        e->num_cu = prop.multiProcessorCount > 0 ? prop.multiProcessorCount : 256;
        e->ctx_mask = ctx_mask & 7;
        HIP_TRY(hipStreamCreateWithFlags(&e->stream.h, hipStreamNonBlocking));
        static const char* names[3] = {"CpG", "CHG", "CHH"};
        for (int c = 0; c < 3; ++c) {
            if (!(e->ctx_mask >> c & 1)) continue;
            HostModel hmw;
            std::string msg;
            if (!load_model_dir(model_dir, names[c], hmw, msg) || !check_model(hmw, names[c], msg)) return fail(nullptr, HM_EMODEL, msg);
            upload_model(e.get(), c, hmw);
        }
        new_slot(e.get(), 0)->state = hm_batch::STAGING;
        return HM_OK;
    });
    if (rc < 0) return rc;
    *out = e.release();
    return HM_OK;
}

void hm_destroy(hm_engine_t* e) { delete e; }

const char* hm_last_error(const hm_engine_t* e) { return e ? e->err.c_str() : g_create_error.c_str(); }

int hm_set_option(hm_engine_t* e, const char* key, int64_t value) {
    if (!e || !key) return HM_EINVAL;
    const std::string k(key);
    if (k == "min_read_size") e->min_read_size = (int)value;
    else if (k == "timing") e->timing = value != 0;
    else if (k == "precision") {
        if (value < 0 || value > 2)
            return fail(e, HM_EINVAL, "precision must be 0 (fp32 MFMA), 1 (split-half f16x3 MFMA, fp32 accumulate) or 2 (as 1 with plain fp16 weights in "
                                      "conv8 and fc1: |dp| <= 1e-3)");
        if (value == 2 && (e->tail_impl == 0 || e->tail_impl == 2))
            return fail(e, HM_EINVAL, "precision 2 needs tail_impl 1 or 3 (the resident / strip tail kernels carry the fp16-weight variants)");
        e->precision = (int)value;
    } else if (k == "conv3_w16") {
        e->conv3_w16 = value != 0;
    } else if (k == "stamps") {
        e->stamps_on = value != 0;
        if (e->stamps_on)
            return guarded(e, [&] {
                const size_t bytes = (size_t)e->num_cu * 8 * front_stamp_slots() * sizeof(unsigned long long);
                e->d_stamps.reserve(bytes);
                HIP_TRY(hipMemset(e->d_stamps.p, 0, bytes));
                e->stamp_sum.assign((size_t)front_stamp_slots() * 8, 0);
                return HM_OK;
            });
    } else if (k == "front_waves") {
        if (value != 4 && value != 8) return fail(e, HM_EINVAL, "front_waves must be 4 or 8");
        e->front_waves = (int)value;
    } else if (k == "sub_batch_sites") {
        if (value < TAIL_SITES) return fail(e, HM_EINVAL, "sub_batch_sites too small");
        e->sub_batch = value / TAIL_SITES * TAIL_SITES;
    } else if (k == "trunk") {
        if (value < 0 || value > 2) return fail(e, HM_EINVAL, "trunk must be 0 (per site), 1 (dense trunk) or 2 (by the site density of the first batch)");
        std::lock_guard<std::mutex> lk(e->mu);
        e->trunk = (int)value;
        e->trunk_mask_auto = -1;
    } else if (k == "trunk_mask") {
        if (value < 0 || value > 7) return fail(e, HM_EINVAL, "trunk_mask must be 0..7");
        std::lock_guard<std::mutex> lk(e->mu);
        e->trunk = 2;
        e->trunk_mask_auto = (int)value & e->ctx_mask;
    } else if (k == "trunk_impl") {
        if (value < 0 || value > 3) return HM_EINVAL;
        e->trunk_impl = (int)value;
    } else if (k == "num_cu") {
        if (value < 1 || value > 1024) return fail(e, HM_EINVAL, "num_cu must be 1..1024");
        e->num_cu = (int)value;
    } else if (k == "edge_impl") {
        if (value < 0 || value > 1) return fail(e, HM_EINVAL, "edge_impl must be 0 or 1");
        e->edge_impl = (int)value;
    } else if (k == "tail_impl") {
        if (value < 0 || value > 3) return fail(e, HM_EINVAL, "tail_impl must be 0, 1, 2 or 3");
        if (e->precision == 2 && (value == 0 || value == 2))
            return fail(e, HM_EINVAL, "tail_impl 0 and 2 do not carry precision 2 (fp16 weights in conv8 and fc1): use tail_impl 1 or 3");
        e->tail_impl = (int)value;
    } else if (k == "tail_slice") {
        if (value < 16) return fail(e, HM_EINVAL, "tail_slice must be at least 16");
        e->tail_slice = value;
    } else if (k == "group_bases") {
        if (value < 0 || value > (int64_t(48) << 20))
            return fail(e, HM_EINVAL, "group_bases must be 1 .. 48 Mi (0: sized from free device memory)");
        e->group_bases = value;
    } else if (k == "slots") {
        if (value < 1 || value > 16) return fail(e, HM_EINVAL, "slots must be 1..16");
        e->max_slots = (int)value;
    } else return fail(e, HM_EINVAL, "unknown option " + k);
    return HM_OK;
}

int hm_submit_read(hm_engine_t* e, int32_t read_id, int32_t l_qseq, int32_t flag, const uint8_t* seq4,
                   const void* fi, int fi_w, const void* fp, int fp_w, const void* ri, int ri_w, const void* rp,
                   int rp_w) {
    if (!e) return HM_EINVAL;
    hm_batch* b = legacy(e);
    if (b->uploaded) return fail(e, HM_ESTATE, "hm_submit_read: batch already uploaded; hm_clear first");
    return stage_read(b, read_id, l_qseq, flag, seq4, fi, fi_w, fp, fp_w, ri, ri_w, rp, rp_w);
}

int hm_clear(hm_engine_t* e) {
    if (!e) return HM_EINVAL;
    hm_batch* b = legacy(e);
    (void)hipSetDevice(e->device);
    if (b->ran && !b->have_totals) (void)hipEventSynchronize(b->ev_out);
    if (b->s_io) (void)hipStreamSynchronize(b->s_io);
    try {
        collect_timing(e, b->spans, b->ran ? b->h_totals : nullptr);
    } catch (const HipErr&) {
    }
    reset_staging(b);
    return HM_OK;
}

int hm_upload(hm_engine_t* e) {
    if (!e) return HM_EINVAL;
    return guarded(e, [&] {
        enqueue_upload(legacy(e));
        return HM_OK;
    });
}

int hm_run(hm_engine_t* e) {
    if (!e) return HM_EINVAL;
    hm_batch* b = legacy(e);
    if (!b->uploaded) return fail(e, HM_ESTATE, "hm_run: nothing uploaded");
    return guarded(e, [&] {
        if (b->ran && !b->have_totals) {
            int rc = wait_totals(b);
            if (rc < 0) return rc;
        }
        enqueue_run(b);
        return HM_OK;
    });
}

int hm_sync(hm_engine_t* e) {
    if (!e) return HM_EINVAL;
    hm_batch* b = legacy(e);
    return guarded(e, [&] {
        if (!b->ran) {
            if (b->uploaded) HIP_TRY(hipEventSynchronize(b->ev_in));
            return HM_OK;
        }
        return wait_totals(b);
    });
}

int64_t hm_num_sites(hm_engine_t* e, int ctx) {
    if (!e || ctx < 0 || ctx > 3) return HM_EINVAL;
    hm_batch* b = legacy(e);
    if (!b->ran) return fail(e, HM_ESTATE, "hm_num_sites: hm_run first");
    const int rc = guarded(e, [&] { return wait_totals(b); });
    return rc < 0 ? rc : b->totals[ctx];
}

int64_t hm_fetch(hm_engine_t* e, hm_call_t* out, int64_t cap) {
    if (!e || (!out && cap > 0)) return HM_EINVAL;
    hm_batch* b = legacy(e);
    if (!b->ran) return fail(e, HM_ESTATE, "hm_fetch: hm_run first");
    const int rc = guarded(e, [&] { return fetch_calls(b); });
    if (rc < 0) return rc;
    const int64_t n = b->totals[TOT_ALL];
    if (n > cap) return fail(e, HM_EINVAL, "hm_fetch: output capacity too small");
    if (n) memcpy(out, b->h_calls.p, (size_t)n * sizeof(hm_call_t));
    return n;
}

int hm_flush(hm_engine_t* e) {
    int rc = hm_upload(e);
    return rc < 0 ? rc : hm_run(e);
}

int64_t hm_drain(hm_engine_t* e, hm_call_t* out, int64_t cap) {
    const int64_t n = hm_fetch(e, out, cap);
    if (n >= 0) hm_clear(e);
    return n;
}

hm_batch_t* hm_batch_begin(hm_engine_t* e) {
    if (!e) return nullptr;
    std::unique_lock<std::mutex> lk(e->mu);
    for (;;) {
        for (size_t i = 1; i < e->slots.size(); ++i)
            if (e->slots[i]->state == hm_batch::FREE) {
                hm_batch* b = e->slots[i].get();
                b->state = hm_batch::STAGING;
                reset_staging(b);
                return b;
            }
        if ((int)e->slots.size() - 1 < e->max_slots) {
            auto failed = [e](const HipErr& h) {
                e->err = hip_error_text(h);
                return nullptr;
            };
            return hip_guard(e->device, failed, [e] {
                hm_batch* b = new_slot(e, (int)e->slots.size());
                b->state = hm_batch::STAGING;
                return b;
            });
        }
        e->cv.wait(lk);
    }
}

int hm_batch_submit_read(hm_batch_t* b, int32_t read_id, int32_t l_qseq, int32_t flag, const uint8_t* seq4, const void* fi,
                         int fi_w, const void* fp, int fp_w, const void* ri, int ri_w, const void* rp, int rp_w) {
    if (!b) return HM_EINVAL;
    if (b->state != hm_batch::STAGING) return fail(b->e, HM_ESTATE, "hm_batch_submit_read: batch is not being staged");
    return stage_read(b, read_id, l_qseq, flag, seq4, fi, fi_w, fp, fp_w, ri, ri_w, rp, rp_w);
}

int64_t hm_batch_submit_reads(hm_batch_t* b, const hm_read_t* reads, int64_t n, int threads, uint8_t* accepted) {
    if (!b || (!reads && n > 0) || n < 0) return HM_EINVAL;
    hm_engine* e = b->e;
    if (b->state != hm_batch::STAGING) return fail(e, HM_ESTATE, "hm_batch_submit_reads: batch is not being staged");
    std::vector<SlabCopy> copies;
    copies.reserve((size_t)n * 5);
    const int64_t taken = guarded(e, [&]() -> int64_t {
        std::vector<uint8_t> take((size_t)n);
        size_t need_total = 0;
        int64_t tb = b->total_bases;
        for (int64_t i = 0; i < n; ++i) {
            const int rc = check_read(e, reads[i], tb, "hm_batch_submit_reads", "nothing was staged -- submit fewer reads per batch");
            if (rc < 0) return rc;
            take[(size_t)i] = (uint8_t)rc;
            const size_t L = (size_t)reads[i].l_qseq;
            need_total += align16((L + 1) / 2) + 4 * align16(L * 2);
            if (rc) tb += padded_bases(reads[i].l_qseq);
        }
        if (b->slab.n + need_total > b->slab.cap) b->slab.reserve(std::max<size_t>(b->slab.n + need_total, size_t(64) << 20));
        int64_t placed = 0;
        for (int64_t i = 0; i < n; ++i) {
            if (accepted) accepted[i] = take[(size_t)i];
            if (!take[(size_t)i]) continue;
            copies.resize(copies.size() + 5);
            place_read(b, reads[i], &copies[copies.size() - 5]);
            ++placed;
        }
        return placed;
    });
    if (taken < 0) return taken;
    const int nt = (int)std::clamp<int64_t>(threads, 1, 64);
    uint8_t* base = b->slab.p;
    auto run = [&](int t) {
        for (size_t i = (size_t)t; i < copies.size(); i += (size_t)nt) memcpy(base + copies[i].off, copies[i].src, copies[i].bytes);
    };
    if (nt == 1 || copies.size() < 64) {
        for (int t = 0; t < nt; ++t) run(t);
    } else {
        std::vector<std::thread> pool;
        for (int t = 1; t < nt; ++t) pool.emplace_back(run, t);
        run(0);
        for (auto& th : pool) th.join();
    }
    return taken;
}

int hm_trunk_mask_for_reads(const hm_read_t* reads, int64_t n, int ctx_mask) {
    if ((!reads && n > 0) || n < 0) return HM_EINVAL;
    return trunk_mask_from_sample((size_t)n, [&](size_t r) { return SeqView{reads[r].seq4, reads[r].l_qseq}; }, ctx_mask & 7);
}

int64_t hm_batch_staged_bases(const hm_batch_t* b) { return b ? b->total_bases : HM_EINVAL; }

int hm_batch_enqueue(hm_batch_t* b) {
    if (!b) return HM_EINVAL;
    hm_engine* e = b->e;
    if (b->state != hm_batch::STAGING) return fail(e, HM_ESTATE, "hm_batch_enqueue: batch is not being staged");
    return guarded(e, [&] {
        enqueue_upload(b);
        {
            std::lock_guard<std::mutex> lk(e->mu);
            b->state = hm_batch::QUEUED;
        }
        std::lock_guard<std::mutex> lk(e->order_mu);
        enqueue_run(b);
        return HM_OK;
    });
}

int hm_batch_done(hm_batch_t* b) {
    if (!b) return HM_EINVAL;
    if (b->state != hm_batch::QUEUED) return fail(b->e, HM_ESTATE, "hm_batch_done: batch was not queued");
    if (b->have_totals) return 1;
    const hipError_t q = hipEventQuery(b->ev_out);
    if (q == hipSuccess) return 1;
    if (q == hipErrorNotReady) return 0;
    return fail(b->e, HM_EDEVICE, std::string("HIP error: ") + hipGetErrorString(q));
}

int64_t hm_batch_wait(hm_batch_t* b, const hm_call_t** calls) {
    if (!b) return HM_EINVAL;
    hm_engine* e = b->e;
    if (b->state != hm_batch::QUEUED) return fail(e, HM_ESTATE, "hm_batch_wait: batch was not queued");
    const int rc = guarded(e, [&] { return calls ? fetch_calls(b) : wait_totals(b); });
    if (rc < 0) return rc;
    if (calls) *calls = b->h_calls.p;
    return b->totals[TOT_ALL];
}

int64_t hm_batch_num_sites(hm_batch_t* b, int ctx) {
    if (!b || ctx < 0 || ctx > 3) return HM_EINVAL;
    const int64_t rc = hm_batch_wait(b, nullptr);
    return rc < 0 ? rc : b->totals[ctx];
}

int hm_batch_release(hm_batch_t* b) {
    if (!b) return HM_EINVAL;
    hm_engine* e = b->e;
    if (b->state == hm_batch::QUEUED) {
        (void)hipSetDevice(e->device);
        (void)hipEventSynchronize(b->ev_out);
        (void)hipStreamSynchronize(b->s_io);
        try {
            collect_timing(e, b->spans, b->h_totals);
        } catch (const HipErr&) {
        }
    }
    {
        std::lock_guard<std::mutex> lk(e->mu);
        b->state = hm_batch::FREE;
    }
    e->cv.notify_all();
    return HM_OK;
}

int64_t hm_scan_sites(hm_engine_t* e, int ctx, int32_t* read_id, int32_t* qoff, uint8_t* strand, int64_t cap) {
    if (!e || ctx < 0 || ctx > 2) return HM_EINVAL;
    hm_batch* b = legacy(e);
    if (!b->ran) return fail(e, HM_ESTATE, "hm_scan_sites: hm_run first");
    int rc = hm_sync(e);
    if (rc < 0) return rc;
    const int64_t n = b->totals[ctx];
    if (n > cap) return fail(e, HM_EINVAL, "hm_scan_sites: output capacity too small");
    if (n == 0) return 0;
    return guarded(e, [&] {
        std::vector<Site> s((size_t)n);
        std::vector<uint8_t> tag((size_t)b->totals[TOT_ALL]);
        HIP_TRY(hipMemcpy(s.data(), b->d_csites.as<Site>() + b->totals[TOT_CTX_BASE + ctx], (size_t)n * sizeof(Site), hipMemcpyDeviceToHost));
        HIP_TRY(hipMemcpy(tag.data(), b->d_utag.p, tag.size(), hipMemcpyDeviceToHost));
        for (int64_t i = 0; i < n; ++i) {
            if (read_id) read_id[i] = b->reads.p[(size_t)s[(size_t)i].read_idx].read_id;
            if (qoff) qoff[i] = s[(size_t)i].qoff;
            if (strand) strand[i] = tag[(size_t)s[(size_t)i].uidx] >> 2;
        }
        return n;
    });
}

int64_t hm_site_logits(hm_engine_t* e, int ctx, float* logits, int64_t cap) {
    if (!e || ctx < 0 || ctx > 2) return HM_EINVAL;
    hm_batch* b = legacy(e);
    if (!b->ran) return fail(e, HM_ESTATE, "hm_site_logits: hm_run first");
    int rc = hm_sync(e);
    if (rc < 0) return rc;
    const int64_t n = b->totals[ctx];
    if (n > cap) return fail(e, HM_EINVAL, "hm_site_logits: output capacity too small");
    if (n == 0) return 0;
    if (!logits) return HM_EINVAL;
    return guarded(e, [&]() -> int64_t {
        std::vector<Site> s((size_t)n);
        std::vector<float> lg((size_t)b->totals[TOT_ALL] * 2);
        HIP_TRY(hipMemcpy(s.data(), b->d_csites.as<Site>() + b->totals[TOT_CTX_BASE + ctx], (size_t)n * sizeof(Site), hipMemcpyDeviceToHost));
        HIP_TRY(hipMemcpy(lg.data(), b->d_logits.p, lg.size() * sizeof(float), hipMemcpyDeviceToHost));
        for (int64_t i = 0; i < n; ++i) {
            const size_t u = (size_t)s[(size_t)i].uidx;
            if (u >= (size_t)b->totals[TOT_ALL]) return fail(e, HM_EDEVICE, "hm_site_logits: site index out of range");
            logits[2 * i] = lg[2 * u];
            logits[2 * i + 1] = lg[2 * u + 1];
        }
        return n;
    });
}

int hm_windows(hm_engine_t* e, int ctx, int64_t first, int64_t n, float* out_host) {
    if (!e || ctx < 0 || ctx > 2 || first < 0 || n < 0) return HM_EINVAL;
    hm_batch* b = legacy(e);
    if (!b->ran) return fail(e, HM_ESTATE, "hm_windows: hm_run first");
    int rc = hm_sync(e);
    if (rc < 0) return rc;
    if (first + n > b->totals[ctx]) return fail(e, HM_EINVAL, "hm_windows: site range out of bounds");
    if (n == 0) return HM_OK;
    return guarded(e, [&] {
        const size_t bytes = (size_t)n * KMER * FEATS * sizeof(float);
        e->d_win.reserve(bytes);
        std::vector<TimedSpan> spans;
        Span sp(e, &spans, K_WINDOW, 0, 0, n);
        launch_windows(e->stream, b->d_csites.as<Site>() + b->totals[TOT_CTX_BASE + ctx] + first, (int)n, b->d_reads.as<ReadDesc>(),
                       b->d_bases.as<uint8_t>(), b->d_kin.as<uint32_t>(), e->model[ctx].w.bn, e->d_win.as<float>(),
                       e->num_cu * 8);
        sp.end();
        HIP_TRY(hipGetLastError());
        if (out_host) HIP_TRY(hipMemcpyAsync(out_host, e->d_win.p, bytes, hipMemcpyDeviceToHost, e->stream));
        HIP_TRY(hipStreamSynchronize(e->stream));
        collect_timing(e, spans, nullptr);
        return HM_OK;
    });
}

int hm_cnn_logits(hm_engine_t* e, int ctx, const float* windows, int64_t n, float* logits, float* p, uint8_t* ml) {
    if (!e || ctx < 0 || ctx > 2 || n < 0 || (!windows && n)) return HM_EINVAL;
    if (!e->model[ctx].loaded) return fail(e, HM_EINVAL, "hm_cnn_logits: context not enabled");
    if (n == 0) return HM_OK;
    return guarded(e, [&] {
        const size_t bytes = (size_t)n * KMER * FEATS * sizeof(float);
        e->d_win.reserve(bytes);
        DevBuf d_lg, d_p, d_ml;
        d_lg.reserve((size_t)n * 2 * sizeof(float));
        d_p.reserve((size_t)n * sizeof(float));
        d_ml.reserve((size_t)n);
        HIP_TRY(hipMemcpyAsync(e->d_win.p, windows, bytes, hipMemcpyHostToDevice, e->stream));
        run_cnn_windows(e, ctx, e->d_win.as<float>(), n, d_lg.as<float>(), d_p.as<float>(), d_ml.as<uint8_t>(), nullptr, 0);
        if (logits) HIP_TRY(hipMemcpy(logits, d_lg.p, (size_t)n * 2 * sizeof(float), hipMemcpyDeviceToHost));
        if (p) HIP_TRY(hipMemcpy(p, d_p.p, (size_t)n * sizeof(float), hipMemcpyDeviceToHost));
        if (ml) HIP_TRY(hipMemcpy(ml, d_ml.p, (size_t)n, hipMemcpyDeviceToHost));
        return HM_OK;
    });
}

int64_t hm_debug_layer(hm_engine_t* e, int ctx, const float* window, int layer, float* out, int64_t cap) {
    if (!e || ctx < 0 || ctx > 2 || !window || !out || layer < 1 || layer > 8) return HM_EINVAL;
    if (!e->model[ctx].loaded) return fail(e, HM_EINVAL, "hm_debug_layer: context not enabled");
    static const int chans[9] = {8, 128, 128, 128, 96, 96, 96, 64, 64};
    int len = KMER;
    const int k1 = e->model[ctx].k1;
    for (int i = 1; i <= layer; ++i) len = (len + 2 - (i == 1 ? k1 : 3)) / 2 + 1;
    const int64_t nf = (int64_t)len * chans[layer];
    if (nf > cap) return fail(e, HM_EINVAL, "hm_debug_layer: output capacity too small");
    return guarded(e, [&] {
        const size_t bytes = (size_t)KMER * FEATS * sizeof(float);
        e->d_win.reserve(bytes);
        e->d_dbg.reserve((size_t)nf * sizeof(float));
        DevBuf res;
        res.reserve(64);
        HIP_TRY(hipMemcpyAsync(e->d_win.p, window, bytes, hipMemcpyHostToDevice, e->stream));
        run_cnn_windows(e, ctx, e->d_win.as<float>(), 1, res.as<float>(), res.as<float>() + 2,
                        reinterpret_cast<uint8_t*>(res.as<float>() + 3), e->d_dbg.as<float>(), layer);
        const void* src = layer == 4 ? e->d_act4.p : e->d_dbg.p;
        HIP_TRY(hipMemcpy(out, src, (size_t)nf * sizeof(float), hipMemcpyDeviceToHost));
        return nf;
    });
}

int hm_convert_model(const char* src_path, const char* dst_hmw_path) {
    if (!src_path || !dst_hmw_path) return fail(nullptr, HM_EINVAL, "hm_convert_model: bad argument");
    const std::string src(src_path);
    HostModel m;
    std::string msg;
    const bool is_hmw = src.size() > 4 && src.compare(src.size() - 4, 4, ".hmw") == 0;
    if (!(is_hmw ? load_hmw(src, m, msg) : load_onnx(src, m, msg))) return fail(nullptr, HM_EMODEL, msg);
    if (!save_hmw(m, dst_hmw_path, msg)) return fail(nullptr, HM_EMODEL, msg);
    return HM_OK;
}

int hm_get_stamps(hm_engine_t* e, uint64_t* out, int cap) {
    if (!e || !out) return HM_EINVAL;
    const int n = (int)std::min<size_t>(e->stamp_sum.size(), (size_t)std::max(cap, 0));
    for (int i = 0; i < n; ++i) out[i] = e->stamp_sum[(size_t)i];
    return n;
}

int hm_get_timing(hm_engine_t* e, hm_timing_t* t) {
    if (!e || !t) return HM_EINVAL;
    std::lock_guard<std::mutex> lk(e->mu);
    *t = e->acc;
    t->group_bases = effective_group_bases(e);
    t->group_bytes = e->grp.bytes();
    return HM_OK;
}

int hm_abi_version(void) { return HM_ABI_VERSION; }
size_t hm_timing_size(void) { return sizeof(hm_timing_t); }

int hm_reset_timing(hm_engine_t* e) {
    if (!e) return HM_EINVAL;
    std::lock_guard<std::mutex> lk(e->mu);
    memset(&e->acc, 0, sizeof e->acc);
    return HM_OK;
}

}
```

### hifimeth_amd/csrc/hm_kernels.h

```cpp
#pragma once
#include <hip/hip_runtime.h>

#include "hm_device.h"

namespace hm {

void launch_prep(hipStream_t st, const uint8_t* raw, const ReadDesc* reads, const Chunk* chunks, int n_chunks,
                 int ctx_mask, uint8_t* bases, uint32_t* kin, uint8_t* sctx, int32_t* chunk_counts, int32_t* err);
void launch_scan(hipStream_t st, const int32_t* chunk_counts, int n_chunks, int32_t* chunk_offs, int32_t* totals);
void launch_emit(hipStream_t st, const ReadDesc* reads, const Chunk* chunks, int n_chunks, int ctx_mask,
                 const uint8_t* bases, const int32_t* chunk_offs, const int32_t* totals, USite* usites,
                 uint8_t* utag, Site* csites, int32_t* opos);
void launch_pack(hipStream_t st, const USite* usites, const uint8_t* utag, const int32_t* opos, const float* prob,
                 const uint8_t* ml, const ReadDesc* reads, const int32_t* totals, void* calls, int grid);
void launch_windows(hipStream_t st, const Site* sites, int n, const ReadDesc* reads, const uint8_t* bases,
                    const uint32_t* kin, const BnTables* bn, float* out, int grid);

void launch_front(hipStream_t st, int k1, const SiteRange& sr, const ReadDesc* reads, const uint8_t* bases,
                  const uint32_t* kin, const float* windows, const CtxWeights& w, float* act4, int grid,
                  float* dbg, int dbg_layer, int waves, unsigned long long* stamps);
int front_stamp_slots();
void launch_front_h(hipStream_t st, int k1, const SiteRange& sr, const ReadDesc* reads, const uint8_t* bases,
                    const uint32_t* kin, const float* windows, const CtxWeights& w, float* act4, int grid, float* dbg,
                    int dbg_layer, unsigned long long* stamps);
void launch_tail_h(hipStream_t st, const float* act4, const SiteRange& sr, const CtxWeights& w, float* logits,
                   float* p, uint8_t* ml, int grid, float* dbg, int dbg_layer);
void launch_tail(hipStream_t st, const float* act4, const SiteRange& sr, const CtxWeights& w, float* logits,
                 float* p, uint8_t* ml, int grid, float* dbg, int dbg_layer);

#ifdef __HIPCC__
__device__ __forceinline__ int resolve_sites(const SiteRange& sr, const Site*& sites) {
    if (!sr.totals) {
        sites = sr.base;
        return sr.cap;
    }
    const int first = sr.lo ? *sr.lo : 0, last = sr.hi ? *sr.hi : sr.totals[sr.ctx];
    int n = last - first - sr.off;
    n = n < 0 ? 0 : (n > sr.cap ? sr.cap : n);
    sites = sr.base + sr.totals[4 + sr.ctx] + first + sr.off;
    return n;
}
#endif

void launch_trunk(hipStream_t st, int k1, const TrunkTile* tiles, int n_tiles, int n_views, int ctx, const RInfo* rinfo,
                  const uint8_t* bases, const uint32_t* kin, const uint8_t* sctx, const CtxWeights& w,
                  const TrunkMaps& maps, int grid);
void launch_edge(hipStream_t st, int k1, const SiteRange& sr, const RInfo* rinfo, const uint8_t* bases,
                 const uint32_t* kin, const CtxWeights& w, const TrunkMaps& maps, uint16_t* edge4, int32_t* e4row, int grid);
void launch_edge2(hipStream_t st, int k1, const SiteRange& sr, const RInfo* rinfo, const uint8_t* bases, const uint32_t* kin,
                  const CtxWeights& w, const TrunkMaps& maps, uint16_t* edge4, int32_t* e4row, int grid);
void launch_tail_gather(hipStream_t st, const SiteRange& sr, const CtxWeights& w, const TrunkMaps& maps, const uint16_t* edge4,
                        const int32_t* e4row, float* logits, float* p, uint8_t* ml, int grid);
void launch_tail_gather_r(hipStream_t st, const SiteRange& sr, const CtxWeights& w, const TrunkMaps& maps, const uint16_t* edge4,
                          const int32_t* e4row, float* logits, float* p, uint8_t* ml, int grid, bool w16 = false);
size_t tail_split_x6_plane_halves(int64_t sites);
size_t tail_split_x6_bytes(int64_t sites);
void launch_tail_split(hipStream_t st, const SiteRange& sr, const CtxWeights& w, const TrunkMaps& maps, const uint16_t* edge4,
                       const int32_t* e4row, uint16_t* x6, size_t x6_plane_halves, float* logits, float* p, uint8_t* ml, int grid);
size_t tail_strip_mark_bytes(int64_t map_rows);
size_t tail_strip_count_bytes(int64_t map_rows);
void launch_tail_strip(hipStream_t st, const SiteRange& sr, const CtxWeights& w, const TrunkMaps& maps, int n_views, const uint16_t* edge4,
                       const int32_t* e4row, int32_t* mark, int32_t* cnt, int32_t* order, int32_t* okey, int32_t* odst, uint16_t* x8, float* logits, float* p,
                       uint8_t* ml, int32_t* pass_count, int grid, bool w16);
size_t tail_fc_x8_bytes(int64_t sites);
size_t tail_strip_handover_bytes(int64_t sites);
void launch_tail_fc(hipStream_t st, const SiteRange& sr, const CtxWeights& w, const uint16_t* x8, const int32_t* dst, float* logits, float* p,
                    uint8_t* ml, int grid, bool w16);
void launch_trunk2(hipStream_t st, int k1, const TrunkTile* tiles, int n_tiles, int n_views, int ctx, const RInfo* rinfo,
                   const uint8_t* bases, const uint32_t* kin, const uint8_t* sctx, const CtxWeights& w,
                   const TrunkMaps& maps, int grid, bool waves8 = false);
size_t trunk3_rowlist_bytes(int64_t n_work);
size_t trunk3_dump_bytes(int grid);
void launch_trunk3(hipStream_t st, int k1, const TrunkTile* tiles, int n_tiles, int n_views, int ctx, const RInfo* rinfo,
                   const uint8_t* bases, const uint32_t* kin, const uint8_t* sctx, int64_t n_bases, const CtxWeights& w, const TrunkMaps& maps,
                   uint16_t* dump, int32_t* list_steps, const int32_t* tcost, int grid, bool w3_single = false);
void launch_trunk_f32(hipStream_t st, int k1, const TrunkTile* tiles, int n_tiles, int n_views, int ctx, const RInfo* rinfo,
                      const uint8_t* bases, const uint32_t* kin, const uint8_t* sctx, const CtxWeights& w,
                      const TrunkMaps& maps, int grid);
void launch_edge_f32(hipStream_t st, int k1, const SiteRange& sr, const RInfo* rinfo, const uint8_t* bases, const uint32_t* kin,
                     const CtxWeights& w, const TrunkMaps& maps, float* edge4, int32_t* e4row, int grid);
void launch_tail_gather_f32(hipStream_t st, const SiteRange& sr, const CtxWeights& w, const TrunkMaps& maps, const float* edge4,
                            const int32_t* e4row, float* logits, float* p, uint8_t* ml, int grid);
size_t trunk_lds_bytes();

size_t front_lds_bytes(int k1);
size_t tail_lds_bytes();

}
```

### hifimeth_amd/csrc/hm_trunk3.hip

```cpp
#include "hm_convh.h"
#ifdef HM_TRUNK_STAMP
#include "hm_stamp.h"
namespace hm { __device__ unsigned long long g_trunk3_stamp[8][24]; }
extern "C" int hm_debug_trunk3_stamps(unsigned long long* out, int reset) {
    if (out && hipMemcpyFromSymbol(out, HIP_SYMBOL(hm::g_trunk3_stamp), sizeof(hm::g_trunk3_stamp)) != hipSuccess) return -1;
    if (reset) {
        static unsigned long long z[8][24];
        if (hipMemcpyToSymbol(HIP_SYMBOL(hm::g_trunk3_stamp), z, sizeof(z)) != hipSuccess) return -1;
    }
    return 0;
}
#endif
#include "hm_convs.h"
#include "hm_edge.h"

namespace hm {

namespace {

constexpr int T3_M = TR_OWN;
constexpr int T3_H1 = 4, T3_H2 = 8, T3_H3 = 16;
constexpr int T3_S3 = T3_H3, T3_S2 = T3_S3 + T3_H2, T3_S1 = T3_S2 + T3_H1;
constexpr int T3_AROWS = T3_M + T3_H3, T3_BROWS = T3_M + T3_H2;
constexpr int T3_XROWS = 128;
constexpr int T3_LDS_HALVES = 2 * T3_AROWS * TR_RS + 2 * T3_BROWS * TR_RS + 2 * (T3_H1 + T3_H3) * TR_RS;
constexpr int T3_N4 = 64, T3_RL3 = 3 * TR_OWN, T3_RL = T3_RL3 + T3_N4 + 4;
constexpr int T3_RLW = 3 * 32 + T3_N4 / 4 + 1;
constexpr int T3_TIER[] = {2, 4, 6};
constexpr int T3_NT = sizeof(T3_TIER) / sizeof(int), T3_CS_ALL = TR_OWN / 8;
static_assert(T3_M % 16 == 0 && T3_RL % 4 == 0 && T3_RL / 4 <= 256 && T3_XROWS >= T3_M + 12, "tile plan");

struct ListRows4 {
    static constexpr bool DENSE = false;
    static constexpr int M = T3_N4;
    const uint8_t* rows = nullptr;
    template <class C>
    __device__ __forceinline__ int off(int m) const { return (int)rows[m] * C::IRS; }
};
struct EpiE4L {
    half_t* __restrict__ g;
    const uint8_t* rows;
    __device__ __forceinline__ void operator()(int m, int col, const f32x4& acc) const {
        half4 h, l;
        split4(acc, h, l);
        const size_t o = (size_t)rows[m] * (2 * C4_CH) + col;
        *reinterpret_cast<half4*>(g + o) = h;
        *reinterpret_cast<half4*>(g + o + C4_CH) = l;
    }
};

struct EpiTrunk3 {
    half_t* hi;
    half_t* lo;
    __device__ __forceinline__ void operator()(int m, int col, const f32x4& acc) const {
        half4 h, l;
        split4(acc, h, l);
        *reinterpret_cast<half4*>(hi + m * TR_RS + col) = h;
        *reinterpret_cast<half4*>(lo + m * TR_RS + col) = l;
    }
};
struct EpiE43 {
    half_t* __restrict__ g;
    __device__ __forceinline__ void operator()(int m, int col, const f32x4& acc) const {
        half4 h, l;
        split4(acc, h, l);
        *reinterpret_cast<half4*>(g + (size_t)m * (2 * C4_CH) + col) = h;
        *reinterpret_cast<half4*>(g + (size_t)m * (2 * C4_CH) + C4_CH + col) = l;
    }
};
template <int NWV_, int CS_ = TR_OWN / (2 * NWV_)>
struct CopyRows3 {
    static constexpr int NWV = NWV_, CS = CS_;
    static_assert(CS_ >= 0 && 2 * NWV_ * CS_ <= TR_OWN, "slots within the list");
    const uint8_t* rows;
    half_t* g;
};
template <int NWV_>
struct CopyRows3T : CopyRows3<NWV_> {
    static constexpr bool TIERED = true;
    static constexpr int NT = T3_NT;
    static constexpr int tier(int i) { return T3_TIER[i]; }
    int need;
};

__device__ __forceinline__ void t3_lds_barrier() {
    __builtin_amdgcn_fence(__ATOMIC_RELEASE, "workgroup", "local");
    __builtin_amdgcn_s_barrier();
    __builtin_amdgcn_fence(__ATOMIC_ACQUIRE, "workgroup", "local");
}

template <int NROWS, int NT, int K = 0>
__device__ __forceinline__ void move_rows(half_t* dh, half_t* dl, const half_t* sh, const half_t* sl, int t) {
    constexpr int PER = NROWS * TR_RS / 8, N = 2 * PER;
    if constexpr (K * NT < N) {
        const int c = min(t + K * NT, N - 1), plane = c >= PER, o = (c - plane * PER) * 8;
        const uint4 v = *reinterpret_cast<const uint4*>((plane ? sl : sh) + o);
        move_rows<NROWS, NT, K + 1>(dh, dl, sh, sl, t);
        *reinterpret_cast<uint4*>((plane ? dl : dh) + o) = v;
    }
}

}

constexpr int T3_RPB = 4;
template <int K1>
__global__ __launch_bounds__(64) void rowlist3_kernel(const TrunkTile* __restrict__ tiles, int n_tiles, int n_work, int ctx,
                                                       const RInfo* __restrict__ rinfo, const uint8_t* __restrict__ sctx, int64_t n_bases,
                                                       uint8_t* __restrict__ rowlist) {
    using G = EdgeGeo<K1>;
    const int r = threadIdx.x;
    constexpr int first_new[3] = {T3_H1, T3_H2, T3_H3}, shift[3] = {T3_S1, T3_S2, T3_S3};
    constexpr int W0 = -176, WN = 528;
    __shared__ __attribute__((aligned(4))) uint8_t rec[T3_RPB][T3_RL];
    __shared__ __attribute__((aligned(4))) uint8_t sf[T3_RPB][WN];
    static_assert(-G::R1 - 2 + T3_S1 >= W0 && -G::R2 - 4 + T3_S2 >= W0 && -G::R3 - 8 + T3_S3 >= W0 && T3_S1 + TR_OWN - 1 - G::LEFT < W0 + WN &&
                  215 - 16 * 23 >= W0 && TR_OWN - 1 + 215 - 16 < W0 + WN, "the window covers every lookup");
    int kind[T3_RPB];
    TrunkTile tl[T3_RPB];
    RInfo ri[T3_RPB];
    bool warm[T3_RPB];
    int view[T3_RPB];
#pragma unroll
    for (int k = 0; k < T3_RPB; ++k) {
        const int blk = (int)blockIdx.x * T3_RPB + k;
        kind[k] = blk > 2 * n_work ? 0 : blk == 2 * n_work ? 2 : 1;
        warm[k] = blk >= n_work;
        const int w = min(warm[k] ? blk - n_work : blk, n_work - 1);
        view[k] = w >= n_tiles;
        tl[k] = tiles[view[k] ? w - n_tiles : w];
    }
    bool any = false;
#pragma unroll
    for (int k = 0; k < T3_RPB; ++k) {
        if (kind[k] == 1 && warm[k] && tl[k].u0 != -TR_PAD) kind[k] = 0;
        any |= kind[k] != 0;
    }
    if (!any) return;
#pragma unroll
    for (int k = 0; k < T3_RPB; ++k) ri[k] = rinfo[tl[k].read_idx];
    constexpr int NQ = (WN / 4 + 63) / 64;
    static_assert(WN % 4 == 0 && (-W0) % 4 == 0 && TR_PAD % 4 == 0 && TR_OWN % 4 == 0, "windows start on multiples of 4");
    uint32_t sw[T3_RPB][NQ];
#pragma unroll
    for (int k = 0; k < T3_RPB; ++k) {
        const int L = ri[k].len, u = tl[k].u0 - (warm[k] ? TR_OWN : 0);
#pragma unroll
        for (int q = 0; q < NQ; ++q) {
            const int y0 = u + W0 + 4 * (r + 64 * q);
            const int64_t a = view[k] ? ri[k].base_off + (L - 1 - y0 - 3) : ri[k].base_off + y0;
            if (a >= 0 && a + 4 <= n_bases) {
                uint32_t v;
                __builtin_memcpy(&v, sctx + a, 4);
                sw[k][q] = view[k] ? __builtin_bswap32(v) : v;
            } else {
                uint32_t v = 0;
#pragma unroll
                for (int t = 0; t < 4; ++t) {
                    const int64_t j = view[k] ? ri[k].base_off + (L - 1 - y0 - t) : ri[k].base_off + y0 + t;
                    v |= (uint32_t)(j >= 0 && j < n_bases ? sctx[j] : (uint8_t)CTX_NONE) << (8 * t);
                }
                sw[k][q] = v;
            }
        }
    }
#pragma unroll
    for (int k = 0; k < T3_RPB; ++k) {
        for (int i = r; i < T3_RL3; i += 64) rec[k][i] = (uint8_t)(first_new[i / TR_OWN] + TR_OWN - 1);
        const int L = ri[k].len, u = tl[k].u0 - (warm[k] ? TR_OWN : 0);
        const uint32_t key = (uint32_t)(ctx | (view[k] << 2)) * 0x01010101u;
#pragma unroll
        for (int q = 0; q < NQ; ++q) {
            const int y0 = u + W0 + 4 * (r + 64 * q);
            const uint32_t x = sw[k][q] ^ key;
            uint32_t hit = (~(((x & 0x7F7F7F7Fu) + 0x7F7F7F7Fu) | x | 0x7F7F7F7Fu)) >> 7;
            const int lo = min(max(-y0, 0), 4), hi = min(max(L - y0, 0), 4);
            const uint32_t m_hi = hi >= 4 ? 0xFFFFFFFFu : (1u << (8 * hi)) - 1u, m_lo = lo >= 4 ? 0xFFFFFFFFu : (1u << (8 * lo)) - 1u;
            hit &= m_hi & ~m_lo;
            if (r + 64 * q < WN / 4) reinterpret_cast<uint32_t*>(sf[k])[r + 64 * q] = hit;
        }
    }
    __syncthreads();
    const uint64_t below = (1ull << r) - 1;
#pragma unroll
    for (int k = 0; k < T3_RPB; ++k) {
        if (kind[k] == 0) continue;
        const int blk = (int)blockIdx.x * T3_RPB + k;
        int n4 = 255;
        uint32_t nst = 0;
        if (kind[k] == 1) {
            const int u = tl[k].u0 - (warm[k] ? TR_OWN : 0);
            auto sat = [&](int y) __attribute__((always_inline)) { return (int)sf[k][y - u - W0]; };
            const bool want4 = K1 == 11 && !warm[k];
            int f[2] = {0, 0}, need4[2] = {0, 0};
#pragma unroll
            for (int h = 0; h < 2; ++h) {
                const int row = r + 64 * h;
                if (row < TR_OWN) {
                    {
                        const int x = u + shift[0] + row;
                        f[h] |= (sat(x - G::LEFT) | sat(x - G::R1) | (G::PAD2 ? 0 : sat(x - G::R1 - 2))) << 0;
                    }
                    {
                        const int x = u + shift[1] + row;
                        f[h] |= (sat(x - G::LEFT) | sat(x - G::R2) | (G::PAD3 ? 0 : sat(x - G::R2 - 4))) << 1;
                    }
                    {
                        const int x = u + shift[2] + row;
                        f[h] |= (sat(x - G::LEFT) | sat(x - G::R3) | (G::PAD4 ? 0 : sat(x - G::R3 - 8))) << 2;
                    }
                    if (want4) {
#pragma unroll
                        for (int sidx = 1; sidx <= 23; ++sidx) need4[h] |= sat(u + row + 215 - 16 * sidx);
                    }
                }
            }
#pragma unroll
            for (int l = 0; l < 3; ++l) {
                const uint64_t b0 = __ballot((f[0] >> l) & 1), b1 = __ballot((f[1] >> l) & 1);
                if ((f[0] >> l) & 1) rec[k][l * TR_OWN + __popcll(b0 & below)] = (uint8_t)(first_new[l] + r);
                if ((f[1] >> l) & 1) rec[k][l * TR_OWN + __popcll(b0) + __popcll(b1 & below)] = (uint8_t)(first_new[l] + r + 64);
                nst |= (uint32_t)(__popcll(b0) + __popcll(b1) + (int)(~(b1 >> (TR_OWN - 1 - 64)) & 1)) << (8 * (l + 1));
            }
            const uint64_t n0 = __ballot(need4[0]), n1 = __ballot(need4[1]);
            if (want4) n4 = __popcll(n0) + __popcll(n1);
            if (want4 && n4 <= T3_N4) {
                if (need4[0]) rec[k][T3_RL3 + __popcll(n0 & below)] = (uint8_t)r;
                if (need4[1]) rec[k][T3_RL3 + __popcll(n0) + __popcll(n1 & below)] = (uint8_t)(r + 64);
                __syncthreads();
                if (r >= n4) rec[k][T3_RL3 + r] = n4 > 0 ? rec[k][T3_RL3] : (uint8_t)0;
            }
        }
        if (r == 0) *reinterpret_cast<uint32_t*>(&rec[k][T3_RL3 + T3_N4]) = (uint32_t)n4 | nst;
        __syncthreads();
        uint32_t* out = reinterpret_cast<uint32_t*>(rowlist + (size_t)blk * T3_RL);
        for (int i = r; i < T3_RL / 4; i += 64) out[i] = reinterpret_cast<const uint32_t*>(rec[k])[i];
    }
}

template <int K1, bool W3LO = true>
__global__ __launch_bounds__(256) __attribute__((amdgpu_waves_per_eu(1, 1)))
void trunk3_kernel(const TrunkTile* __restrict__ tiles, int n_tiles, int n_views, int ctx, const RInfo* __restrict__ rinfo,
                   const uint8_t* __restrict__ bases, const uint32_t* __restrict__ kin, CtxWeights W, TrunkMaps mp, half_t* __restrict__ dump,
                   int32_t* __restrict__ list_steps, const int32_t* __restrict__ tcost) {
    constexpr int NW = 4, NTW = 2;
    __shared__ __attribute__((aligned(16))) half_t smem[T3_LDS_HALVES + T3_XROWS * TR_WRS];
    static_assert(sizeof(smem) == 147840, "LDS plan");
    __shared__ uint32_t rlist[2][T3_RLW];
    __shared__ int64_t s_grow0;
    __shared__ int s_kind;
    __shared__ __attribute__((aligned(16))) half_t kc[3][2][128];
    __shared__ __attribute__((aligned(16))) half_t e4c[2 * C4_CH];
    half_t* a_hi = smem;
    half_t* a_lo = a_hi + T3_AROWS * TR_RS;
    half_t* b_hi = a_lo + T3_AROWS * TR_RS;
    half_t* b_lo = b_hi + T3_BROWS * TR_RS;
    half_t* h1_hi = b_lo + T3_BROWS * TR_RS;
    half_t* h1_lo = h1_hi + T3_H1 * TR_RS;
    half_t* h3_hi = h1_lo + T3_H1 * TR_RS;
    half_t* h3_lo = h3_hi + T3_H3 * TR_RS;
    half_t* xb = h3_lo + T3_H3 * TR_RS;
    const int n_work = n_tiles * n_views;
    const int lane = threadIdx.x & 63, wave = __builtin_amdgcn_readfirstlane(threadIdx.x >> 6);
    int w0, w1;
    if (tcost) {
        const int64_t c_view = tcost[n_tiles], c_all = c_view * n_views;
        auto cost_at = [&](const int wq) __attribute__((always_inline)) {
            const int v = wq >= n_tiles && wq < n_work ? 1 : wq >= n_work ? n_views : 0;
            return v * c_view + (wq >= n_work ? 0 : tcost[wq - (v ? n_tiles : 0)]);
        };
        auto first_at = [&](const int64_t target) __attribute__((always_inline)) {
            int lo = 0, hi = n_work;
            while (hi > lo) {
                const int stride = (hi - lo + 63) / 64;
                const int probe = lo + lane * stride;
                const bool ge = probe >= hi || cost_at(probe) >= target;
                const uint64_t bal = __ballot(ge);
                const int first = bal ? __builtin_ctzll(bal) : 64;
                if (first == 0) {
                    hi = lo;
                } else {
                    const int nlo = lo + (first - 1) * stride + 1;
                    hi = first < 64 ? min(lo + first * stride, hi) : hi;
                    lo = nlo;
                }
            }
            return __builtin_amdgcn_readfirstlane(lo);
        };
        const int64_t k = blockIdx.x, G = gridDim.x;
        w0 = first_at((k * c_all + G - 1) / G);
        w1 = k + 1 == G ? n_work : first_at(((k + 1) * c_all + G - 1) / G);
    } else {
        const int base_n = n_work / (int)gridDim.x, rem_n = n_work - base_n * (int)gridDim.x;
        w0 = (int)blockIdx.x * base_n + min((int)blockIdx.x, rem_n);
        w1 = w0 + base_n + ((int)blockIdx.x < rem_n);
    }
    if (w0 >= w1) return;

    for (int i = threadIdx.x; i < (T3_LDS_HALVES + T3_XROWS * TR_WRS) / 2; i += NW * 64) reinterpret_cast<uint32_t*>(smem)[i] = 0u;
    for (int i = threadIdx.x; i < 2 * T3_RLW; i += NW * 64) rlist[0][i] = 0;
    __syncthreads();

    struct Build {
        TrunkTile tl, tl2;
        RInfo ri;
        int w, view, warm, cst, calib, ueff, b;
        uint32_t k, rl;
    } bd;
    auto build_desc1 = [&](const int w) __attribute__((always_inline)) {
        bd.w = w;
        bd.view = w >= n_tiles;
        bd.tl = tiles[bd.view ? w - n_tiles : w];
        const int w2 = min(w + 1, n_work - 1);
        bd.tl2 = tiles[w2 >= n_tiles ? w2 - n_tiles : w2];
    };
    auto build_desc2 = [&](const int prev_warm, const bool first) __attribute__((always_inline)) {
        bd.tl.read_idx = __builtin_amdgcn_readfirstlane(bd.tl.read_idx);
        bd.tl.u0 = __builtin_amdgcn_readfirstlane(bd.tl.u0);
        bd.warm = first ? 1 : (prev_warm ? 0 : (bd.tl.u0 == -TR_PAD));
        bd.calib = 0;
        bd.ueff = bd.tl.u0 - (bd.warm ? TR_OWN : 0);
        bd.ri = rinfo[bd.tl.read_idx];
    };
    auto build_desc3 = [&]() __attribute__((always_inline)) {
        bd.ri.len = __builtin_amdgcn_readfirstlane(bd.ri.len);
        bd.ri.map_off = __builtin_amdgcn_readfirstlane(bd.ri.map_off);
        bd.ri.base_off = ((int64_t)__builtin_amdgcn_readfirstlane((int)(bd.ri.base_off >> 32)) << 32) |
                         (uint32_t)__builtin_amdgcn_readfirstlane((int)bd.ri.base_off);
        bd.cst = bd.tl.u0 == -TR_PAD || (!bd.warm && bd.tl.u0 >= bd.ri.len);
    };
    auto build_loads = [&]() __attribute__((always_inline)) {
        const int r = threadIdx.x, L = bd.ri.len, x = bd.ueff + T3_S1 + r;
        const int xc = min(max(x, 0), L - 1);
        const int64_t j = bd.ri.base_off + (bd.view ? L - 1 - xc : xc);
        bd.b = bases[j];
        bd.k = kin[j];
        const size_t li = bd.calib ? (size_t)2 * n_work : bd.warm ? (bd.tl.u0 == -TR_PAD ? (size_t)n_work + bd.w : (size_t)2 * n_work) : (size_t)bd.w;
        bd.rl = reinterpret_cast<const uint32_t*>(mp.rowlist + li * T3_RL)[min(r, T3_RL / 4 - 1)];
    };
    auto build_store = [&](const int buf) __attribute__((always_inline)) {
        const int r = threadIdx.x, x = bd.ueff + T3_S1 + r;
        if (r == 0) {
            s_grow0 = (int64_t)bd.view * mp.view_rows + bd.ri.map_off + (bd.ueff + TR_PAD);
            s_kind = bd.warm | (bd.cst << 1) | (bd.calib << 2);
        }
        if (r < T3_XROWS) {
            const bool in = !bd.calib && x >= 0 && x < bd.ri.len;
            *reinterpret_cast<uint4*>(xb + r * TR_WRS) = feature_row(in ? bd.b : -1, bd.k, bd.view);
        }
        if (r < T3_RL3 / 4) rlist[buf][r / (TR_OWN / 4) * 32 + r % (TR_OWN / 4)] = bd.rl;
        else if (r < T3_RL / 4) rlist[buf][3 * 32 + r - T3_RL3 / 4] = bd.rl;
    };

    using C1 = SCfg<8, (2 * K1 + 3) / 4 * 4, TR_WRS, 1, true, false, K1, 2, NTW>;
    using C2 = SCfg<128, 3, TR_RS, 2, true, true, 0, 1, NTW>;
    using C3 = SCfg<128, 3, TR_RS, 4, W3LO, true, 0, 1, NTW>;
    using C4 = SCfg<128, 3, TR_RS, 8, true, true, 0, 1, NTW>;
    using C4s = SCfg<128, 3, TR_RS, 8, true, true, 0, 1, 1>;
    const int nt04 = wave == 0 ? 0 : wave == 1 ? 1 : wave == 2 ? 3 : 4;
    using L1 = SConv<C1, C2, 0, 2, 2, 3>;
    using L2 = SConv<C2, C3, 0, 2, 2, 3>;
    using L3 = SConv<C3, C4, 0, 2, 2, 3>;
    static_assert(T3_XROWS <= NW * 64, "one feature row per thread");
    auto wf = [&](int i) { return reinterpret_cast<const half_t*>(W.wfrag_h[i]); };
    const half_t* c1f = reinterpret_cast<const half_t*>(W.c1f);
    const int nt0 = NTW * wave;

    WRegs wr;
    sconv_load_w<C1, 0, C1::KB>(c1f, nt0, lane, wr);
    sconv_load_bias<C1>(W.c1f_bias, nt0, lane, wr);
    build_desc1(w0);
    build_desc2(0, true);
    build_desc3();
    bd.calib = 1;
    bd.cst = 0;
    build_loads();
    build_store(0);
    int buf = 0;
    int w = w0, warm = 1;
    int n_list = 0;
    int n_const = 0;
    bool prev_calib = false;
    half_t* const dump_rows = dump + TR_OWN * 2 * C4_CH;
    half_t* const dump_cal = dump_rows + 128 * 256 + (size_t)blockIdx.x * (TR_OWN * 2 * C4_CH);
    constexpr int first_new[3] = {T3_H1, T3_H2, T3_H3};
#ifdef HM_TRUNK_STAMP
    unsigned long long ts[10], acc_t[16] = {};
    unsigned long long n_it = 0, acc_c = 0, n_c = 0;
    const bool st_on = blockIdx.x == 0;
    const unsigned long long tk0 = hm_stamp(), tr0 = __builtin_amdgcn_s_memrealtime();
#define TS(i) do { if (st_on) ts[i] = hm_stamp(); } while (0)
#else
#define TS(i)
#endif
    while (true) {
        t3_lds_barrier();
        TS(0);
        const int64_t grow0 = s_grow0;
        const int kind = __builtin_amdgcn_readfirstlane(s_kind);
        const int cur_warm = kind & 1, cur_const = (kind >> 1) & 1, cur_calib = kind >> 2;
        if (prev_calib) {
            prev_calib = false;
            __builtin_amdgcn_fence(__ATOMIC_ACQUIRE, "agent");
            const int t = threadIdx.x;
            if (t < 96) {
                const int l = t >> 5, plane = (t >> 4) & 1, col = (t & 15) * 8;
                const half_t* src = l == 0 ? (plane ? h1_lo : h1_hi) : l == 1 ? (plane ? b_lo : b_hi) : (plane ? h3_lo : h3_hi);
                *reinterpret_cast<uint4*>(&kc[l][plane][col]) = *reinterpret_cast<const uint4*>(src + col);
            } else if (t < 96 + 24) {
                reinterpret_cast<uint4*>(e4c)[t - 96] = reinterpret_cast<const uint4*>(dump_cal + (TR_OWN - 1) * 2 * C4_CH)[t - 96];
            }
            __syncthreads();
        }
        const int wn = cur_warm ? w : w + 1;
        const bool last = wn >= w1;
        half_t* g1 = cur_calib ? dump_rows : reinterpret_cast<half_t*>(mp.e[0]) + (grow0 + T3_S2) * 256;
        half_t* g2 = cur_calib ? dump_rows : reinterpret_cast<half_t*>(mp.e[1]) + (grow0 + T3_S3) * 256;
        half_t* g3 = cur_calib ? dump_rows : reinterpret_cast<half_t*>(mp.e[2]) + grow0 * 256;
        const uint8_t* rl = reinterpret_cast<const uint8_t*>(rlist[buf]);
        if (cur_const) {
            const int t = threadIdx.x;
            n_const += !cur_warm;
            const int wb = min(wn, w1 - 1);
            bool new_read = false;
            if (wb != bd.w) {
                const int prev_read = bd.tl.read_idx;
                bd.w = wb;
                bd.view = wb >= n_tiles;
                bd.tl.read_idx = __builtin_amdgcn_readfirstlane(bd.tl2.read_idx);
                bd.tl.u0 = __builtin_amdgcn_readfirstlane(bd.tl2.u0);
                const int w2 = min(wb + 1, n_work - 1);
                bd.tl2 = tiles[w2 >= n_tiles ? w2 - n_tiles : w2];
                new_read = bd.tl.read_idx != prev_read;
                if (new_read) bd.ri = rinfo[bd.tl.read_idx];
            }
            auto finish_desc = [&]() __attribute__((always_inline)) {
                bd.warm = cur_warm ? 0 : (bd.tl.u0 == -TR_PAD);
                bd.calib = 0;
                bd.ueff = bd.tl.u0 - (bd.warm ? TR_OWN : 0);
                bd.cst = bd.tl.u0 == -TR_PAD || (!bd.warm && bd.tl.u0 >= bd.ri.len);
                build_loads();
            };
            if (!new_read) finish_desc();
            if (!cur_warm) {
                uint4* g4 = reinterpret_cast<uint4*>(reinterpret_cast<half_t*>(mp.e4) + grow0 * (2 * C4_CH));
                const uint4 v = reinterpret_cast<const uint4*>(e4c)[t % 24];
                const uint4 v2 = reinterpret_cast<const uint4*>(e4c)[(t + 16) % 24], v3 = reinterpret_cast<const uint4*>(e4c)[(t + 8) % 24];
#pragma unroll
                for (int k = 0; k < (TR_OWN * 24 + 255) / 256; ++k) {
                    const int c = t + 256 * k;
                    if (c < TR_OWN * 24) g4[c] = k % 3 == 0 ? v : k % 3 == 1 ? v2 : v3;
                }
            }
#pragma unroll
            for (int l = 0; l < 3; ++l) {
                const uint8_t* rows = rl + 128 * l;
                half_t* g = l == 0 ? g1 : l == 1 ? g2 : g3;
                const int fill = first_new[l] + TR_OWN - 1, ch = t & 31;
                const uint4 v = reinterpret_cast<const uint4*>(&kc[l][0][0])[ch];
                int pr[TR_OWN / 8];
#pragma unroll
                for (int i = 0; i < TR_OWN / 8; ++i) pr[i] = rows[(t >> 5) + 8 * i];
#pragma unroll
                for (int i = 0; i < TR_OWN / 8; ++i)
                    if (pr[i] != fill) reinterpret_cast<uint4*>(g + (size_t)pr[i] * 256)[ch] = v;
                if (t < 32) reinterpret_cast<uint4*>(g + (size_t)fill * 256)[ch] = v;
            }
            for (int c = t; c < (T3_H1 + T3_H2 + T3_H3) * 32; c += NW * 64) {
                const int row = c >> 5, plane = (c >> 4) & 1, col = (c & 15) * 8;
                const int l = row < T3_H1 ? 0 : row < T3_H1 + T3_H2 ? 1 : 2, r = row - (l == 0 ? 0 : l == 1 ? T3_H1 : T3_H1 + T3_H2);
                half_t* dst = (l == 0 ? (plane ? h1_lo : h1_hi) : l == 1 ? (plane ? b_lo : b_hi) : (plane ? h3_lo : h3_hi)) + r * TR_RS + col;
                *reinterpret_cast<uint4*>(dst) = *reinterpret_cast<const uint4*>(&kc[l][plane][col]);
            }
            if (new_read) {
                build_desc3();
                finish_desc();
            }
            t3_lds_barrier();
            build_store(buf ^ 1);
            buf ^= 1;
#ifdef HM_TRUNK_STAMP
            if (st_on) {
                acc_c += hm_stamp() - ts[0];
                ++n_c;
            }
#endif
            if (last) break;
            w = wn;
            warm = bd.warm;
            continue;
        }
        using Cp23 = CopyRows3T<NW>;
        const uint32_t cw = (uint32_t)__builtin_amdgcn_readfirstlane((int)rlist[buf][T3_RLW - 1]);
        auto with_slots = [&](const int need, auto&& f) __attribute__((always_inline)) {
            auto pick = [&](auto self, auto i_) __attribute__((always_inline)) -> void {
                constexpr int i = decltype(i_)::value;
                if constexpr (i == T3_NT) f(std::integral_constant<int, T3_CS_ALL>{});
                else if (need <= 8 * T3_TIER[i]) f(std::integral_constant<int, T3_TIER[i]>{});
                else self(self, std::integral_constant<int, i + 1>{});
            };
            pick(pick, std::integral_constant<int, 0>{});
        };
        move_rows<T3_H1, NW * 64>(a_hi, a_lo, h1_hi, h1_lo, threadIdx.x);
        L1::run(xb, xb, wr, EpiTrunk3{a_hi + T3_H1 * TR_RS, a_lo + T3_H1 * TR_RS}, wf(1), W.bias[1], nt0, nt0);
        build_desc1(min(wn, w1 - 1));
        TS(1);
        __syncthreads();
        TS(2);
        build_desc2(cur_warm, cur_calib != 0);
        L2::run(a_hi, a_lo, wr, EpiTrunk3{b_hi + T3_H2 * TR_RS, b_lo + T3_H2 * TR_RS}, wf(2), W.bias[2], nt0, nt0, Cp23{{rl, g1}, (int)((cw >> 8) & 255)});
        move_rows<T3_H1, NW * 64>(h1_hi, h1_lo, a_hi + T3_M * TR_RS, a_lo + T3_M * TR_RS, threadIdx.x);
        TS(3);
        __syncthreads();
        TS(4);
        build_desc3();
        build_loads();
        move_rows<T3_H3, NW * 64>(a_hi, a_lo, h3_hi, h3_lo, threadIdx.x);
        L3::run(b_hi, b_lo, wr, EpiTrunk3{a_hi + T3_H3 * TR_RS, a_lo + T3_H3 * TR_RS}, wf(3), W.bias[3], nt0, nt04, Cp23{{rl + 128, g2}, (int)((cw >> 16) & 255)});
        TS(5);
        __syncthreads();
        TS(6);
        move_rows<T3_H3, NW * 64>(h3_hi, h3_lo, a_hi + T3_M * TR_RS, a_lo + T3_M * TR_RS, threadIdx.x);
        move_rows<T3_H2, NW * 64>(b_hi, b_lo, b_hi + T3_M * TR_RS, b_lo + T3_M * TR_RS, threadIdx.x);
        const EpiE43 e4{cur_calib ? dump_cal : cur_warm ? dump : reinterpret_cast<half_t*>(mp.e4) + grow0 * (2 * C4_CH)};
        const int n4 = cw & 255, ns3 = cw >> 24;
        if (!cur_warm && n4 <= T3_N4) {
            ++n_list;
            const uint8_t* rows4 = rl + 3 * 128;
            const ListRows4 rm{rows4};
            const EpiE4L e4l{reinterpret_cast<half_t*>(mp.e4) + grow0 * (2 * C4_CH), rows4};
            using NoCp = typename SConvR<C4, C1, ListRows4, 2, 2>::NoCopy;
            if (wave & 1) {
                with_slots(ns3, [&](auto cs_) __attribute__((always_inline)) {
                    SConvR<C4s, void, ListRows4, 0, 1, 1>::template run<1>(a_hi, a_lo, wr, e4l, c1f, W.c1f_bias, nt04, nt0, CopyRows3<NW, decltype(cs_)::value>{rl + 256, g3}, rm);
                });
                SConvR<C4, C1, ListRows4, 2, 2>::run(a_hi, a_lo, wr, e4l, c1f, W.c1f_bias, nt04, nt0, NoCp{}, rm);
            } else {
                with_slots(ns3, [&](auto cs_) __attribute__((always_inline)) {
                    SConvR<C4, void, ListRows4, 0, 1, 1>::run(a_hi, a_lo, wr, e4l, c1f, W.c1f_bias, nt04, nt0, CopyRows3<NW, decltype(cs_)::value>{rl + 256, g3}, rm);
                });
                SConvR<C4s, C1, ListRows4, 2, 2>::template run<0>(a_hi, a_lo, wr, e4l, c1f, W.c1f_bias, nt04, nt0, NoCp{}, rm);
            }
        } else
        if (wave & 1) {
            with_slots(ns3, [&](auto cs_) __attribute__((always_inline)) {
                SConv<C4s, void, 0, 2, 2>::template run<1>(a_hi, a_lo, wr, e4, c1f, W.c1f_bias, nt04, nt0, CopyRows3<NW, decltype(cs_)::value>{rl + 256, g3});
            });
            SConv<C4, C1, 4, 3>::run(a_hi, a_lo, wr, e4, c1f, W.c1f_bias, nt04, nt0);
        } else {
            with_slots(ns3, [&](auto cs_) __attribute__((always_inline)) {
                SConv<C4, void, 0, 2, 2>::run(a_hi, a_lo, wr, e4, c1f, W.c1f_bias, nt04, nt0, CopyRows3<NW, decltype(cs_)::value>{rl + 256, g3});
            });
            SConv<C4s, C1, 4, 3>::template run<0>(a_hi, a_lo, wr, e4, c1f, W.c1f_bias, nt04, nt0);
        }
        build_store(buf ^ 1);
        buf ^= 1;
        if (cur_calib) {
            __builtin_amdgcn_fence(__ATOMIC_RELEASE, "agent");
            prev_calib = true;
        }
        TS(7);
#ifdef HM_TRUNK_STAMP
        if (st_on) {
            __syncthreads();
            ts[8] = hm_stamp();
            for (int l = 0; l < 4; ++l) {
                acc_t[4 * l + 0] += ts[2 * l + 1] - ts[2 * l];
                acc_t[4 * l + 3] += ts[2 * l + 2] - ts[2 * l + 1];
            }
            ++n_it;
        }
#endif
        if (last) break;
        w = wn;
        warm = bd.warm;
    }
    (void)warm;
#ifdef HM_TRUNK_STAMP
    if (st_on && (threadIdx.x & 63) == 0) {
        for (int i = 0; i < 16; ++i) atomicAdd(&g_trunk3_stamp[threadIdx.x >> 6][i], acc_t[i]);
        atomicAdd(&g_trunk3_stamp[threadIdx.x >> 6][16], n_it);
        atomicAdd(&g_trunk3_stamp[threadIdx.x >> 6][17], acc_c);
        atomicAdd(&g_trunk3_stamp[threadIdx.x >> 6][18], n_c);
        atomicAdd(&g_trunk3_stamp[threadIdx.x >> 6][22], hm_stamp() - tk0);
        atomicAdd(&g_trunk3_stamp[threadIdx.x >> 6][23], __builtin_amdgcn_s_memrealtime() - tr0);
    }
#endif
#undef TS
    if (list_steps && threadIdx.x == 0 && n_list) atomicAdd(list_steps + ctx, n_list);
    if (list_steps && threadIdx.x == 0 && n_const) atomicAdd(list_steps + 4 + ctx, n_const);
}

size_t trunk3_rowlist_bytes(int64_t n_work) { return (size_t)(2 * n_work + 1) * T3_RL + 64; }
size_t trunk3_dump_bytes(int grid) { return ((size_t)(1 + grid) * TR_OWN * 2 * C4_CH + 128 * 256) * sizeof(uint16_t); }

void launch_trunk3(hipStream_t st, int k1, const TrunkTile* tiles, int n_tiles, int n_views, int ctx, const RInfo* rinfo,
                   const uint8_t* bases, const uint32_t* kin, const uint8_t* sctx, int64_t n_bases, const CtxWeights& w, const TrunkMaps& maps,
                   uint16_t* dump, int32_t* list_steps, const int32_t* tcost, int grid, bool w3_single) {
    if (n_tiles <= 0) return;
    const int n_work = n_tiles * n_views;
    const dim3 g(min(n_work, grid));
    if (k1 == 11) {
        hipLaunchKernelGGL(rowlist3_kernel<11>, dim3((2 * n_work + T3_RPB) / T3_RPB), dim3(64), 0, st, tiles, n_tiles, n_work, ctx, rinfo, sctx, n_bases, maps.rowlist);
        if (w3_single) hipLaunchKernelGGL((trunk3_kernel<11, false>), g, dim3(256), 0, st, tiles, n_tiles, n_views, ctx, rinfo, bases, kin, w, maps, reinterpret_cast<half_t*>(dump), list_steps, tcost);
        else hipLaunchKernelGGL((trunk3_kernel<11, true>), g, dim3(256), 0, st, tiles, n_tiles, n_views, ctx, rinfo, bases, kin, w, maps, reinterpret_cast<half_t*>(dump), list_steps, tcost);
    } else {
        hipLaunchKernelGGL(rowlist3_kernel<13>, dim3((2 * n_work + T3_RPB) / T3_RPB), dim3(64), 0, st, tiles, n_tiles, n_work, ctx, rinfo, sctx, n_bases, maps.rowlist);
        if (w3_single) hipLaunchKernelGGL((trunk3_kernel<13, false>), g, dim3(256), 0, st, tiles, n_tiles, n_views, ctx, rinfo, bases, kin, w, maps, reinterpret_cast<half_t*>(dump), list_steps, tcost);
        else hipLaunchKernelGGL((trunk3_kernel<13, true>), g, dim3(256), 0, st, tiles, n_tiles, n_views, ctx, rinfo, bases, kin, w, maps, reinterpret_cast<half_t*>(dump), list_steps, tcost);
    }
}

}
```

### include/hifimeth_hip.h

```cpp
#ifndef HIFIMETH_HIP_H
#define HIFIMETH_HIP_H

#include <stddef.h>
#include <stdint.h>

#ifdef __cplusplus
extern "C" {
#endif

#define HM_CTX_CPG 0
#define HM_CTX_CHG 1
#define HM_CTX_CHH 2
#define HM_CTX_ALL 3

#define HM_OK 0
#define HM_EINVAL (-1)
#define HM_EMODEL (-2)
#define HM_EDEVICE (-3)
#define HM_EDATA (-4)
#define HM_ESTATE (-5)
#define HM_ENOMEM (-6)

typedef struct hm_engine hm_engine_t;

typedef struct {
    int32_t read_id;
    int32_t qoff;
    uint8_t strand;
    uint8_t ctx;
    uint8_t scaled_prob;
    uint8_t reserved;
    float p;
} hm_call_t;

typedef struct {
    double prep_ms, scan_ms, emit_ms, window_ms;
    double front_ms[3], tail_ms[3];
    int64_t prep_launches, scan_launches, emit_launches, window_launches;
    int64_t front_launches[3], tail_launches[3];
    int64_t front_sites[3];
    int64_t window_sites;
    double pack_ms, empty_ms;
    int64_t pack_launches, empty_launches;
    double trunk_ms[3], edge_ms[3];
    int64_t trunk_launches[3], edge_launches[3];
    int64_t trunk_positions[3];
    int64_t trunk_list_steps[3];
    int64_t trunk_const_steps[3];
    int64_t group_bases;
    int64_t group_bytes;
    int64_t tail_strip_passes;
} hm_timing_t;

#define HM_ABI_VERSION 5
int hm_abi_version(void);
size_t hm_timing_size(void);

int hm_create(hm_engine_t** out, const char* model_dir, int ctx_mask, int device);
void hm_destroy(hm_engine_t* e);
const char* hm_last_error(const hm_engine_t* e);
int hm_set_option(hm_engine_t* e, const char* key, int64_t value);

int hm_submit_read(hm_engine_t* e, int32_t read_id, int32_t l_qseq, int32_t flag, const uint8_t* seq4,
                   const void* fi, int fi_width, const void* fp, int fp_width, const void* ri, int ri_width,
                   const void* rp, int rp_width);
int hm_clear(hm_engine_t* e);

int hm_upload(hm_engine_t* e);
int hm_run(hm_engine_t* e);
int hm_sync(hm_engine_t* e);
int64_t hm_num_sites(hm_engine_t* e, int ctx);
int64_t hm_fetch(hm_engine_t* e, hm_call_t* out, int64_t cap);
int hm_flush(hm_engine_t* e);
int64_t hm_drain(hm_engine_t* e, hm_call_t* out, int64_t cap);

typedef struct hm_batch hm_batch_t;
hm_batch_t* hm_batch_begin(hm_engine_t* e);
int hm_batch_submit_read(hm_batch_t* b, int32_t read_id, int32_t l_qseq, int32_t flag, const uint8_t* seq4,
                         const void* fi, int fi_width, const void* fp, int fp_width, const void* ri, int ri_width,
                         const void* rp, int rp_width);
typedef struct {
    int32_t read_id, l_qseq, flag;
    uint8_t width[4];
    const uint8_t* seq4;
    const void* kin[4];
} hm_read_t;
int64_t hm_batch_submit_reads(hm_batch_t* b, const hm_read_t* reads, int64_t n, int threads, uint8_t* accepted);
int hm_trunk_mask_for_reads(const hm_read_t* reads, int64_t n, int ctx_mask);
int64_t hm_batch_staged_bases(const hm_batch_t* b);
int hm_batch_enqueue(hm_batch_t* b);
int hm_batch_done(hm_batch_t* b);
int64_t hm_batch_wait(hm_batch_t* b, const hm_call_t** calls);
int64_t hm_batch_num_sites(hm_batch_t* b, int ctx);
int hm_batch_release(hm_batch_t* b);

int64_t hm_scan_sites(hm_engine_t* e, int ctx, int32_t* read_id, int32_t* qoff, uint8_t* strand, int64_t cap);
int64_t hm_site_logits(hm_engine_t* e, int ctx, float* logits, int64_t cap);
int hm_windows(hm_engine_t* e, int ctx, int64_t first, int64_t n, float* out_host);
int hm_cnn_logits(hm_engine_t* e, int ctx, const float* windows, int64_t n, float* logits, float* p, uint8_t* ml);
int64_t hm_debug_layer(hm_engine_t* e, int ctx, const float* window, int layer, float* out, int64_t cap);

int hm_convert_model(const char* src_path, const char* dst_hmw_path);

int hm_get_stamps(hm_engine_t* e, uint64_t* out, int cap);

int hm_get_timing(hm_engine_t* e, hm_timing_t* t);
int hm_reset_timing(hm_engine_t* e);

typedef struct hm_pileup hm_pileup_t;

typedef struct {
    int32_t qoff;
    uint8_t strand;
    char unmod_base;
    char code;
    uint8_t prob;
} hm_mod_t;

typedef struct {
    int64_t gpos;
    int32_t pcov, ncov;
    uint32_t motif;
    uint32_t reserved;
} hm_locus_t;

int hm_pileup_create(hm_pileup_t** out, int device);
void hm_pileup_destroy(hm_pileup_t* p);
const char* hm_pileup_last_error(const hm_pileup_t* p);
int hm_pileup_set_option(hm_pileup_t* p, const char* key, double value);
int hm_pileup_set_reference(hm_pileup_t* p, int32_t n_seqs, const int64_t* seq_len, const char* bases);
int hm_pileup_use_planes(hm_pileup_t* p, void* pcov, void* ncov, void* key);
int hm_pileup_planes(hm_pileup_t* p, void** pcov, void** ncov, void** key, int64_t* n_loci);
int hm_pileup_use_partition_planes(hm_pileup_t* p, int32_t part, void* pcov, void* ncov);
int hm_pileup_partition_planes(hm_pileup_t* p, int32_t part, void** pcov, void** ncov);
int hm_pileup_submit_read(hm_pileup_t* p, uint32_t order, int32_t flag, int32_t sid, int64_t pos, int32_t mapq,
                          int32_t l_qseq, const uint8_t* seq4, int32_t n_cigar, const uint32_t* cigar,
                          int64_t n_mods, const hm_mod_t* mods);
int hm_pileup_submit_read_hp(hm_pileup_t* p, uint32_t order, int32_t flag, int32_t sid, int64_t pos, int32_t mapq,
                             int32_t l_qseq, const uint8_t* seq4, int32_t n_cigar, const uint32_t* cigar,
                             int64_t n_mods, const hm_mod_t* mods, int32_t hp);
int hm_pileup_submit_read_calls(hm_pileup_t* p, uint32_t order, int32_t flag, int32_t sid, int64_t pos, int32_t mapq,
                                int32_t l_qseq, const uint8_t* seq4, int32_t n_cigar, const uint32_t* cigar,
                                int64_t n_calls, const hm_call_t* calls, int32_t hp);
int hm_pileup_run(hm_pileup_t* p);
int64_t hm_pileup_num_records(hm_pileup_t* p);
int hm_pileup_histograms(hm_pileup_t* p, uint64_t* bins768);
int64_t hm_pileup_fetch_records(hm_pileup_t* p, int64_t* gpos, uint8_t* prob, uint8_t* motif, uint32_t* order,
                                int64_t cap);
int hm_pileup_label_histograms(hm_pileup_t* p, const int8_t* labels, int64_t n_labels, uint64_t* bins1536);
int hm_pileup_count(hm_pileup_t* p, const uint8_t thr[3]);
int64_t hm_pileup_fetch_loci(hm_pileup_t* p, const void* pcov, const void* ncov, const void* key,
                             int64_t plane_base, int64_t lo, int64_t hi, hm_locus_t* out, int64_t cap);

typedef struct {
    int64_t gpos;
    int32_t pcov1, ncov1, pcov2, ncov2;
    uint32_t motif, reserved;
    double diff, pvalue;
} hm_asm_t;
int64_t hm_pileup_fetch_asm(hm_pileup_t* p, const void* pcov1, const void* ncov1, const void* pcov2, const void* ncov2,
                            const void* key, int64_t plane_base, int64_t lo, int64_t hi, int32_t min_cov,
                            hm_asm_t* out, int64_t cap);

#define HM_ASM_T 64
#define HM_ASM_PAIRS 2080
#define HM_ASM_BINS 12979200
typedef struct {
    uint32_t bin, reserved;
    uint64_t count;
    double pvalue, qvalue;
} hm_asm_bin_t;
typedef struct {
    int64_t gpos;
    int32_t pcov1, ncov1, pcov2, ncov2;
    uint32_t motif, reserved;
    double diff, pvalue, qvalue;
} hm_asmq_t;
int64_t hm_pileup_asm_histogram(hm_pileup_t* p, const void* pcov1, const void* ncov1, const void* pcov2, const void* ncov2,
                                const void* key, int64_t plane_base, int64_t lo, int64_t hi, int32_t min_cov, uint64_t* bins,
                                hm_asm_t* big, int64_t cap);
int64_t hm_pileup_asm_bin_pvalues(hm_pileup_t* p, const uint64_t* bins, hm_asm_bin_t* out, int64_t cap);
int hm_asm_qvalues(hm_asm_bin_t* tab, int64_t n_tab, const hm_asm_t* big, int64_t n_big, double* big_q, uint64_t m[3]);
int64_t hm_pileup_fetch_asm_q(hm_pileup_t* p, const void* pcov1, const void* ncov1, const void* pcov2, const void* ncov2,
                              const void* key, int64_t plane_base, int64_t lo, int64_t hi, int32_t min_cov,
                              const hm_asm_bin_t* tab, int64_t n_tab, const hm_asm_t* big, const double* big_q, int64_t n_big,
                              hm_asmq_t* out, int64_t cap);

#define HM_REGION_FIRST 1u
#define HM_REGION_LAST 2u
typedef struct {
    int64_t start, end;
    int64_t pcov1, ncov1, pcov2, ncov2;
    int32_t n_loci, sign;
    uint32_t motif, flags;
    double diff, pmin;
} hm_asm_region_t;
int64_t hm_pileup_fetch_asm_regions(hm_pileup_t* p, const void* pcov1, const void* ncov1, const void* pcov2, const void* ncov2,
                                    const void* key, int64_t plane_base, int64_t lo, int64_t hi, int32_t min_cov, int32_t ctx,
                                    double max_p, int64_t max_gap, int32_t min_loci, int32_t keep_edges, int64_t* n_ctx_rows,
                                    hm_asm_region_t* out, int64_t cap);

int64_t hm_pileup_load_loci(hm_pileup_t* p, int32_t part, const hm_locus_t* rows, int64_t n);

typedef struct {
    int64_t gpos;
    int32_t pcov1, ncov1, pcov2, ncov2;
    uint32_t motif;
    uint16_t m1, m2;
    double diff, D, phi, pvalue;
} hm_group_t;
int hm_pileup_group_sample(hm_pileup_t* p, int32_t part);
int64_t hm_pileup_load_sample_loci(hm_pileup_t* p, const hm_locus_t* rows, int64_t n);
int64_t hm_pileup_fetch_groups(hm_pileup_t* p, int64_t lo, int64_t hi, int32_t min_reps, hm_group_t* out, int64_t cap);
int hm_pileup_group_planes(hm_pileup_t* p, int32_t part, int64_t lo, int64_t hi, uint64_t* moment, uint8_t* samples);
int hm_group_qvalues(const hm_group_t* rows, int64_t n, double* q, uint64_t m[3]);
typedef struct {
    int64_t start, end;
    int64_t pcov1, ncov1, pcov2, ncov2;
    int32_t n_loci, sign;
    uint32_t motif, flags;
    uint16_t m1_min, m2_min;
    uint32_t reserved;
    double diff, pmin, phi_max;
} hm_group_region_t;
int64_t hm_dmr_fetch_regions(hm_pileup_t* p, int64_t lo, int64_t hi, int32_t min_reps, int32_t ctx, double max_p, double min_diff,
                             int64_t max_gap, int32_t min_loci, int32_t keep_edges, int64_t* n_ctx_rows, int64_t* n_hits,
                             hm_group_region_t* out, int64_t cap);
int hm_dmr_p_cutoff(const hm_group_t* rows, const double* q, int64_t n, double max_q, double cutoff[3]);

#define HM_SAMPLE_MAX 64
#define HM_SAMPLE_TILE 256
int hm_sample_geometry(int64_t out[2]);
typedef struct {
    int32_t i, j;
    uint32_t ctx, reserved;
    uint64_t n, si, sj, sii, sjj, sij;
} hm_sample_pair_t;
int hm_sample_open(hm_pileup_t* p);
int64_t hm_sample_load(hm_pileup_t* p, const hm_locus_t* rows, int64_t n);
int64_t hm_sample_fetch_sums(hm_pileup_t* p, int64_t lo, int64_t hi, int32_t complete, hm_sample_pair_t* out);
int hm_sample_plane(hm_pileup_t* p, int32_t s, int64_t lo, int64_t hi, uint16_t* out);
int hm_sample_corr(const hm_sample_pair_t* e, int64_t n, double* r, double* mean_i, double* mean_j);

typedef struct {
    uint64_t n, su;
} hm_sample_interval_t;
int64_t hm_sample_fetch_intervals(hm_pileup_t* p, int64_t lo, int64_t hi, int32_t ctx, int32_t complete, const int64_t* start,
                                  const int64_t* end, int64_t n_iv, hm_sample_interval_t* out);
typedef struct {
    int32_t m1, m2;
    uint64_t n1, n2;
    double mean1, mean2, t, df, pvalue;
} hm_sample_test_t;
int hm_sample_interval_test(const hm_sample_interval_t* sums, int64_t n_iv, int32_t M, const uint8_t* group, int64_t min_loci,
                            int32_t min_reps, hm_sample_test_t* out);
int hm_sample_qvalues(const double* p, int64_t n, double* q);

typedef struct {
    int64_t gpos;
    int32_t pcov, ncov;
    uint32_t motif, reserved;
    double pvalue, qvalue;
} hm_site_t;
#define HM_SITE_BINS 196608
int hm_pileup_control_sums(hm_pileup_t* p, const void* pcov, const void* ncov, const void* key, int64_t lo, int64_t hi,
                           uint64_t sums[6]);
int64_t hm_pileup_site_histogram(hm_pileup_t* p, const void* pcov, const void* ncov, const void* key, int64_t plane_base,
                                 int64_t lo, int64_t hi, uint64_t* bins, hm_locus_t* big, int64_t cap);
int hm_sites_table(const double rates[3], const uint64_t* bins, const hm_locus_t* big, int64_t n_big, double* ptab,
                   double* qtab, double* big_p, double* big_q, uint64_t m[3]);
int64_t hm_pileup_fetch_sites(hm_pileup_t* p, const void* pcov, const void* ncov, const void* key, int64_t plane_base,
                              int64_t lo, int64_t hi, int32_t ctx_mask, const double* ptab, const double* qtab,
                              const hm_locus_t* big, const double* big_p, const double* big_q, int64_t n_big,
                              hm_site_t* out, int64_t cap);

#define HM_DOMAIN_AFTER_BREAK 1u
#define HM_DOMAIN_BEFORE_BREAK 2u
typedef struct {
    int64_t start, end;
    int64_t pcov, ncov;
    int32_t n_loci;
    uint32_t state, motif, flags;
    double level, score;
} hm_domain_t;
int64_t hm_pileup_fetch_domains(hm_pileup_t* p, const void* pcov, const void* ncov, const void* key, int64_t plane_base,
                                int64_t lo, int64_t hi, int32_t ctx, int64_t A, int64_t B, int64_t S, int64_t max_gap,
                                int64_t* n_ctx_rows, hm_domain_t* out, int64_t cap);
#define HM_DOMAIN_PASS_SUMMARY 0
#define HM_DOMAIN_PASS_CODES 1
#define HM_DOMAIN_PASS_SEGMENTS 2
#define HM_DOMAIN_KEEP 2
typedef struct {
    int64_t prev_gpos, prev_d, next_gpos;
    int32_t has_prev, has_next, last_state;
    int32_t back;
    int64_t n_rows, first_gpos, last_gpos, e_first;
    int64_t c, lo, hi;
    int64_t d_last;
} hm_domain_part_t;
int64_t hm_pileup_fetch_domains_part(hm_pileup_t* p, const void* pcov, const void* ncov, const void* key, int64_t plane_base,
                                     int64_t lo, int64_t hi, int32_t ctx, int64_t A, int64_t B, int64_t S, int64_t max_gap,
                                     int32_t pass, hm_domain_part_t* part, hm_domain_t* out, int64_t cap);
int hm_domain_scores(double level_lo, double level_hi, double penalty, int64_t* A, int64_t* B, int64_t* S);

int64_t hm_pileup_domain_sums(hm_pileup_t* p, const void* pcov, const void* ncov, const void* key, int64_t plane_base, int64_t lo,
                              int64_t hi, int32_t ctx, int64_t A, int64_t B, int64_t S, int64_t max_gap, int64_t sums[6]);
int64_t hm_pileup_domain_sums_part(hm_pileup_t* p, const void* pcov, const void* ncov, const void* key, int64_t plane_base,
                                   int64_t lo, int64_t hi, int32_t ctx, int64_t A, int64_t B, int64_t S, int64_t max_gap,
                                   const hm_domain_part_t* part, int64_t sums[6]);
int hm_domain_refit(const int64_t sums[6], double penalty, double* level_lo, double* level_hi);

typedef struct {
    int64_t start, end;
    uint32_t counts[16];
    uint32_t n, k;
} hm_pattern_t;
int64_t hm_pileup_num_pattern_records(hm_pileup_t* p);
int64_t hm_pileup_fetch_patterns(hm_pileup_t* p, int64_t lo, int64_t hi, int64_t min_reads, hm_pattern_t* out, int64_t cap);
int hm_pattern_stats(const hm_pattern_t* w, double out[4]);

typedef struct {
    int64_t gpos;
    uint32_t n_mod, n_canon, n_nocall, n_diff, n_delete, reserved;
} hm_bedmethyl_t;
int64_t hm_pileup_fetch_bedmethyl(hm_pileup_t* p, int32_t part, int64_t lo, int64_t hi, int64_t min_valid, hm_bedmethyl_t* out,
                                  int64_t cap);

typedef struct {
    uint32_t dist, reserved;
    uint64_t n_uu, n_um, n_mu, n_mm;
} hm_linkage_t;
int64_t hm_pileup_fetch_linkage(hm_pileup_t* p, int64_t min_pairs, hm_linkage_t* out, int64_t cap);
int hm_linkage_stats(const hm_linkage_t* w, double out[2]);

typedef struct {
    uint32_t motif, end, dist, reserved;
    uint64_t n_m, n_u, sum_ml;
} hm_readpos_t;
#define HM_READPOS_5P 0
#define HM_READPOS_3P 1
#define HM_READPOS_INTERIOR 2
int64_t hm_pileup_fetch_readpos(hm_pileup_t* p, int64_t min_calls, hm_readpos_t* out, int64_t cap);
int64_t hm_pileup_readpos_histograms(hm_pileup_t* p, uint64_t* hist, int64_t cap);
int hm_pileup_add_readpos(hm_pileup_t* p, const uint64_t* hist, int64_t n);
int hm_readpos_stats(const hm_readpos_t* w, double out[2]);

#ifndef HM_REGION_BLOCK
#define HM_REGION_BLOCK 4096
#endif
#define HM_REGION_SCAN_BLOCKS 1024
typedef struct {
    int64_t n_loci, pcov, ncov, ppm;
} hm_region_sum_t;
int hm_region_geometry(int64_t out[2]);
int hm_pileup_fetch_regions(hm_pileup_t* p, const void* pcov, const void* ncov, const void* key, int64_t plane_base, int64_t lo,
                            int64_t hi, int64_t min_cov, const int64_t* start, const int64_t* end, int64_t n, hm_region_sum_t* out);
typedef struct {
    int32_t motif, bin;
    int64_t n_regions, n_loci, pcov, ncov, ppm;
} hm_metabin_t;
int hm_pileup_fetch_metaplot(hm_pileup_t* p, const void* pcov, const void* ncov, const void* key, int64_t plane_base, int64_t lo,
                             int64_t hi, int64_t min_cov, const int64_t* start, const int64_t* end, const int64_t* seq_start,
                             const int64_t* seq_end, const char* strand, int64_t n, int32_t bins, int64_t flank, int32_t flank_bins,
                             hm_metabin_t* out, int64_t* n_used);
int hm_region_stats(const hm_region_sum_t* w, double out[2]);

#define HM_CONTEXT_SPAN 1024
#define HM_CONTEXT_LDS_MAX_FLANK 1
#ifndef HM_CONTEXT_LDS_FLANK
#define HM_CONTEXT_LDS_FLANK 1
#endif
#define HM_CONTEXT_PATH_AUTO (-1)
#define HM_CONTEXT_PATH_LDS 0
#define HM_CONTEXT_PATH_GLOBAL 1
int hm_context_geometry(int64_t out[3]);
int64_t hm_pileup_fetch_context(hm_pileup_t* p, const void* pcov, const void* ncov, const void* key, int64_t plane_base, int64_t lo,
                                int64_t hi, int64_t min_cov, int32_t flank, hm_region_sum_t* out, int64_t cap);
int64_t hm_pileup_fetch_context_path(hm_pileup_t* p, const void* pcov, const void* ncov, const void* key, int64_t plane_base, int64_t lo,
                                     int64_t hi, int64_t min_cov, int32_t flank, int32_t path, hm_region_sum_t* out, int64_t cap);

#ifdef __cplusplus
}
#endif
#endif
```

Measured before the change: 67.21 million.

## Recompute conv1 edge rows in edge kernel instead of storing E1 map from trunk

The trunk kernel no longer writes the layer-1 (E1) activation map to global memory when edge_impl is 2 (the new default). The edge kernel instead recomputes the few E1 rows it needs from raw features with extra MFMA tiles and stores them into its LDS set, skipping the DMA of those rows. This trades global writes and reads of a large map, plus its allocation, for extra conv1 compute in the edge kernel. A debug entry point for dumping edge rows is also added.

Result: faster. 68.01 million, median of 6 (+1.2%).

```diff
diff --git a/hifimeth_amd/_lib.py b/hifimeth_amd/_lib.py
--- a/hifimeth_amd/_lib.py
+++ b/hifimeth_amd/_lib.py
@@ -87,6 +87,7 @@
         "hm_batch_release": (C.c_int, [vp]),
         "hm_scan_sites": (i64, [vp, C.c_int, vp, vp, vp, i64]),
         "hm_site_logits": (i64, [vp, C.c_int, vp, i64]),
+        "hm_debug_edge_rows": (C.c_int, [vp, i64, vp]),
         "hm_windows": (C.c_int, [vp, C.c_int, i64, i64, vp]),
         "hm_cnn_logits": (C.c_int, [vp, C.c_int, vp, i64, vp, vp, vp]),
         "hm_debug_layer": (i64, [vp, C.c_int, vp, C.c_int, vp, i64]),
diff --git a/hifimeth_amd/caller.py b/hifimeth_amd/caller.py
--- a/hifimeth_amd/caller.py
+++ b/hifimeth_amd/caller.py
@@ -182,6 +182,12 @@
         out = np.empty((n, 2), np.float32)
         got = self._check(self._L.hm_site_logits(self._h, ctx, _vp(out), n), "hm_site_logits")
         return out[:got]
+
+    def edge_rows(self, sites: int) -> np.ndarray:
+        self.sync()
+        out = np.empty((sites, 2, 192), np.uint16)
+        self._check(self._L.hm_debug_edge_rows(self._h, sites, _vp(out)), "hm_debug_edge_rows")
+        return out
 
     def windows(self, ctx: int, first: int = 0, n: Optional[int] = None, fetch: bool = True):
         if n is None:
diff --git a/hifimeth_amd/csrc/hm_edge.h b/hifimeth_amd/csrc/hm_edge.h
--- a/hifimeth_amd/csrc/hm_edge.h
+++ b/hifimeth_amd/csrc/hm_edge.h
@@ -35,7 +35,11 @@
     static constexpr int R1 = -201 + 2 * (2 * (L2 - 1) - 1), R2 = -203 + 4 * (2 * (L3 - 1) - 1), R3 = -207 + 8 * (2 * (C4_LEN - 1) - 1);
     static constexpr int LEFT = -199;
     static constexpr int X_LEFT = -201, X_RIGHT = -201 + 2 * (L1 - 1);
+    static constexpr int NE1 = PAD2 ? 2 : 3;
+    static constexpr int X_PAD = X_RIGHT + K1 - 1 - R1;
 };
+static_assert(EdgeGeo<11>::X_RIGHT - EdgeGeo<11>::R1 == 2 && EdgeGeo<11>::X_PAD == 12 && EdgeGeo<13>::X_RIGHT - EdgeGeo<13>::R1 == 4 && EdgeGeo<13>::X_PAD == 16 &&
+              EdgeGeo<11>::LEFT - EdgeGeo<11>::X_LEFT == 2, "feature spans of the edge kernel's E1 rows");
 static_assert(EdgeGeo<11>::PAD2 && EdgeGeo<11>::PAD3 && !EdgeGeo<11>::PAD4 && EdgeGeo<11>::R1 == 189 && EdgeGeo<11>::R2 == 185 && EdgeGeo<11>::R3 == 169, "k1 = 11 edge geometry");
 static_assert(!EdgeGeo<13>::PAD2 && !EdgeGeo<13>::PAD3 && EdgeGeo<13>::PAD4 && EdgeGeo<13>::R1 == 185 && EdgeGeo<13>::R2 == 177 && EdgeGeo<13>::R3 == 169, "k1 = 13 edge geometry");
 
diff --git a/hifimeth_amd/csrc/hm_edge2.hip b/hifimeth_amd/csrc/hm_edge2.hip
--- a/hifimeth_amd/csrc/hm_edge2.hip
+++ b/hifimeth_amd/csrc/hm_edge2.hip
@@ -86,7 +86,7 @@
 
 }
 
-template <int K1>
+template <int K1, bool E1C>
 __global__ __launch_bounds__(512) void edge2_kernel(SiteRange sr, const RInfo* __restrict__ rinfo, const uint8_t* __restrict__ bases,
                                                      const uint32_t* __restrict__ kin, CtxWeights W, TrunkMaps mp,
                                                      uint16_t* __restrict__ edge4, int32_t* __restrict__ e4row) {
@@ -101,6 +101,7 @@
     half_t* sp_hi = smem + 2 * E2_MSET;
     half_t* sp_lo = sp_hi + E2_SPLANE;
     half_t* xb = sp_lo + E2_SPLANE;
+    static_assert(sizeof(smem) == 2 * 51200 + 2 * 17408 + 17408 && EdgeGeo<K1>::X_PAD <= EG_XROWS && 2 * (EdgeGeo<K1>::NE1 - 2) + K1 <= EG_XROWS, "LDS plan");
     if ((int)blockIdx.x * EG_S >= n_sites) return;
     int tid = threadIdx.x, lane = tid & 63, wave = __builtin_amdgcn_readfirstlane(tid >> 6);
     int li = lane & 15, lk = lane >> 4;
@@ -152,9 +153,9 @@
 #pragma unroll
         for (int u = 0; u < NR; ++u) {
             const int tt = t0 + u;
-            const int x = es.off + (side ? G::X_RIGHT : G::X_LEFT) + tt;
-            const bool is_pad = side ? tt == K1 - 1 : tt == 0;
-            live[u] = tt < K1 && !is_pad && x >= 0 && x < es.L;
+            const int x = es.off + (side ? (E1C ? G::R1 : G::X_RIGHT) : G::X_LEFT) + tt;
+            const bool is_pad = side ? tt == (E1C ? G::X_PAD : K1 - 1) : tt == 0;
+            live[u] = (E1C || tt < K1) && !is_pad && x >= 0 && x < es.L;
             const int xc = min(max(x, 0), es.L - 1);
             const int64_t j = es.bo + (es.view ? es.L - 1 - xc : xc);
             b[u] = bases[j];
@@ -218,34 +219,60 @@
         const int col = wave * 16 + 4 * lk;
         h.bz = *reinterpret_cast<const float4*>(W.c1f_bias + col);
     };
-    auto conv1 = [&](const Head1& h) __attribute__((always_inline)) {
+    auto conv1 = [&](const Head1& h, half_t* e1set) __attribute__((always_inline)) {
         const float4 c0 = *reinterpret_cast<const float4*>(W.c1f_corr + wave * 16 + 4 * lk);
         const float4 c1 = *reinterpret_cast<const float4*>(W.c1f_corr + 128 + wave * 16 + 4 * lk);
-        f32x4 acc[4];
-#pragma unroll
-        for (int i = 0; i < 4; ++i) acc[i] = f32x4{h.bz.x, h.bz.y, h.bz.z, h.bz.w};
         auto stack_off = [&](int kb) __attribute__((always_inline)) {
             int t = 4 * kb + lk;
             t = t >= 2 * K1 ? 0 : t >= K1 ? t - K1 : t;
             return t * TR_WRS;
         };
+        auto tiles = [&](auto nt_, f32x4 (&acc)[4], auto xa) __attribute__((always_inline)) {
+            constexpr int NT = decltype(nt_)::value;
+#pragma unroll
+            for (int i = 0; i < NT; ++i) acc[i] = f32x4{h.bz.x, h.bz.y, h.bz.z, h.bz.w};
+            half8 x[2][NT];
+#pragma unroll
+            for (int i = 0; i < NT; ++i) x[0][i] = *reinterpret_cast<const half8*>(xb + xa(i) + stack_off(0));
+#pragma unroll
+            for (int kb = 0; kb < KB1; ++kb) {
+                if (kb + 1 < KB1) {
+                    const int bo = stack_off(kb + 1);
+#pragma unroll
+                    for (int i = 0; i < NT; ++i) x[(kb + 1) & 1][i] = *reinterpret_cast<const half8*>(xb + xa(i) + bo);
+                }
+#pragma unroll
+                for (int i = 0; i < NT; ++i) acc[i] = __builtin_amdgcn_mfma_f32_16x16x32_f16(h.w[kb], x[kb & 1][i], acc[i], 0, 0, 0);
+            }
+        };
         const int a0 = li * E2_XRS;
-        half8 x[2][4];
-#pragma unroll
-        for (int i = 0; i < 4; ++i) x[0][i] = *reinterpret_cast<const half8*>(xb + a0 + i * (16 * E2_XRS) + stack_off(0));
-#pragma unroll
-        for (int kb = 0; kb < KB1; ++kb) {
-            if (kb + 1 < KB1) {
-                const int bo = stack_off(kb + 1);
-#pragma unroll
-                for (int i = 0; i < 4; ++i) x[(kb + 1) & 1][i] = *reinterpret_cast<const half8*>(xb + a0 + i * (16 * E2_XRS) + bo);
+        f32x4 acc[4];
+        tiles(std::integral_constant<int, 4>{}, acc, [&](int i) __attribute__((always_inline)) {
+            return a0 + i * (16 * E2_XRS) + (E1C && i >= 2 ? (G::X_RIGHT - G::R1) * TR_WRS : 0);
+        });
+        const EpiSpecC1 epi{sp_hi, sp_lo, nullptr, c0, c1};
+#pragma unroll
+        for (int i = 0; i < 4; ++i) epi(i * 16 + li, wave * 16 + 4 * lk, acc[i]);
+        if constexpr (E1C) {
+            auto xa = [&](int j) __attribute__((always_inline)) {
+                return a0 + (j < 4 ? j : j - 2) * (16 * E2_XRS) + (j < 2 ? (G::LEFT - G::X_LEFT) * TR_WRS : j < 4 ? 0 : 2 * TR_WRS);
+            };
+            auto store = [&](int j, const f32x4& a) __attribute__((always_inline)) {
+                half4 hh, ll;
+                split4(a, hh, ll);
+                half_t* o = e1set + (j * 16 + li) * E2_MRS + wave * 16 + 4 * lk;
+                *reinterpret_cast<half4*>(o) = hh;
+                *reinterpret_cast<half4*>(o + 128) = ll;
+            };
+            tiles(std::integral_constant<int, 4>{}, acc, xa);
+#pragma unroll
+            for (int j = 0; j < 4; ++j) store(j, acc[j]);
+            if constexpr (G::NE1 == 3) {
+                tiles(std::integral_constant<int, 2>{}, acc, [&](int i) __attribute__((always_inline)) { return xa(4 + i); });
+#pragma unroll
+                for (int j = 0; j < 2; ++j) store(4 + j, acc[j]);
             }
-#pragma unroll
-            for (int i = 0; i < 4; ++i) acc[i] = __builtin_amdgcn_mfma_f32_16x16x32_f16(h.w[kb], x[kb & 1][i], acc[i], 0, 0, 0);
-        }
-        const EpiSpecC1 epi{sp_hi, sp_lo, nullptr, c0, c1};
-#pragma unroll
-        for (int i = 0; i < 4; ++i) epi(i * 16 + li, wave * 16 + 4 * lk, acc[i]);
+        }
     };
 
     struct LW {
@@ -340,10 +367,11 @@
         desc_c();
         desc_d(s0, sinfo2[0], rowtab[0]);
         load_head1(h1);
+        if (E1C && tid < EG_M) *reinterpret_cast<uint4*>(xb + tid * E2_XRS + EG_XROWS * TR_WRS) = make_uint4(0u, 0u, 0u, 0u);
         __syncthreads();
         build_rows(sinfo2[0], tid, std::integral_constant<int, NW * 64>{}, [] {});
         e2_vmwait<0>();
-        dma_maps(L2t{}, rowtab[0][0], 0, wave, NW8{});
+        if constexpr (!E1C) dma_maps(L2t{}, rowtab[0][0], 0, wave, NW8{});
         e2_vmwait<0>();
     }
     int cur = 0, sel = 0;
@@ -363,7 +391,7 @@
         const int sn = s0 + gridDim.x * EG_S;
         desc_a(sn);
         e2_for<0, 12>([&](auto k_) __attribute__((always_inline)) { load_kb(L2t{}, k_, lw); });
-        conv1(h1);
+        conv1(h1, mset + (size_t)sel * E2_MSET);
         ETS(1);
         e2_vmwait<0>();
         e2_barrier();
@@ -424,8 +452,8 @@
             }, [&](auto b_) __attribute__((always_inline)) {
                 constexpr int b = decltype(b_)::value, NP = (E2L<K1, 2>::NI + NWC - 1) / NWC;
                 static_assert(NP < E2L<K1, 4>::NB, "the pieces fit the layer's blocks");
-                if constexpr (b >= 1 && b - 1 < NP) dma_issue(L2t{}, ds, sel ^ 1, wave + NWC * (b - 1));
-                if constexpr (b < NP) ds = dma_src(L2t{}, rowtab[cur ^ 1][0], wave + NWC * b);
+                if constexpr (!E1C && b >= 1 && b - 1 < NP) dma_issue(L2t{}, ds, sel ^ 1, wave + NWC * (b - 1));
+                if constexpr (!E1C && b < NP) ds = dma_src(L2t{}, rowtab[cur ^ 1][0], wave + NWC * b);
             });
             const EpiEdgeOut epi{reinterpret_cast<half_t*>(edge4) + (size_t)s0 * (4 * C4_CH), nullptr, nvalid};
 #pragma unroll
@@ -453,11 +481,16 @@
 }
 
 void launch_edge2(hipStream_t st, int k1, const SiteRange& sr, const RInfo* rinfo, const uint8_t* bases, const uint32_t* kin,
-                  const CtxWeights& w, const TrunkMaps& maps, uint16_t* edge4, int32_t* e4row, int grid) {
+                  const CtxWeights& w, const TrunkMaps& maps, uint16_t* edge4, int32_t* e4row, int grid, bool own_e1) {
     if (sr.cap <= 0) return;
     const dim3 g(sr.totals ? grid : max(1, min((sr.cap + EG_S - 1) / EG_S, grid))), b(512);
-    if (k1 == 11) hipLaunchKernelGGL(edge2_kernel<11>, g, b, 0, st, sr, rinfo, bases, kin, w, maps, edge4, e4row);
-    else hipLaunchKernelGGL(edge2_kernel<13>, g, b, 0, st, sr, rinfo, bases, kin, w, maps, edge4, e4row);
-}
-
-}
+    if (own_e1) {
+        if (k1 == 11) hipLaunchKernelGGL((edge2_kernel<11, true>), g, b, 0, st, sr, rinfo, bases, kin, w, maps, edge4, e4row);
+        else hipLaunchKernelGGL((edge2_kernel<13, true>), g, b, 0, st, sr, rinfo, bases, kin, w, maps, edge4, e4row);
+    } else {
+        if (k1 == 11) hipLaunchKernelGGL((edge2_kernel<11, false>), g, b, 0, st, sr, rinfo, bases, kin, w, maps, edge4, e4row);
+        else hipLaunchKernelGGL((edge2_kernel<13, false>), g, b, 0, st, sr, rinfo, bases, kin, w, maps, edge4, e4row);
+    }
+}
+
+}
diff --git a/hifimeth_amd/csrc/hm_engine.cpp b/hifimeth_amd/csrc/hm_engine.cpp
--- a/hifimeth_amd/csrc/hm_engine.cpp
+++ b/hifimeth_amd/csrc/hm_engine.cpp
@@ -109,7 +109,7 @@
     int max_slots = 3;
     int trunk = 2;
     int trunk_impl = 3;
-    int edge_impl = 1;
+    int edge_impl = 2;
     int tail_impl = 3;
     int64_t tail_slice = int64_t(1) << 21;
     int trunk_mask_auto = -1;
@@ -481,6 +481,8 @@
     b->ran = b->have_totals = b->have_calls = false;
 }
 
+bool trunk_stores_e1(const hm_engine* e) { return e->precision == 0 || e->trunk_impl != 3 || e->edge_impl != 2 || e->conv3_w16 != 0; }
+
 void run_trunk_path(hm_batch* b, std::vector<TimedSpan>* spans, int ctx_mask) {
     hm_engine* e = b->e;
     int64_t max_rows = 1, max_bases = 1;
@@ -488,7 +490,8 @@
         max_rows = std::max(max_rows, g.rows);
         max_bases = std::max(max_bases, g.bases);
     }
-    for (int i = 0; i < 3; ++i) e->grp.d_map[i].reserve((size_t)max_rows * 2 * 256 * sizeof(uint16_t));
+    const bool store_e1 = trunk_stores_e1(e);
+    for (int i = store_e1 ? 0 : 1; i < 3; ++i) e->grp.d_map[i].reserve((size_t)max_rows * 2 * 256 * sizeof(uint16_t));
     e->grp.d_e4.reserve((size_t)max_rows * 2 * C4_CH * sizeof(float));
     e->grp.d_rowlist.reserve(std::max((size_t)(max_rows / TR_OWN + 1) * 2 * 3 * TR_OWN, trunk3_rowlist_bytes((max_rows / TR_OWN + 1) * 2)));
     e->grp.d_dump.reserve(trunk3_dump_bytes(e->num_cu));
@@ -508,7 +511,7 @@
     }
     const int32_t* offs = b->d_offs.as<int32_t>();
     for (const auto& g : b->groups) {
-        const TrunkMaps maps{{e->grp.d_map[0].as<uint16_t>(), e->grp.d_map[1].as<uint16_t>(), e->grp.d_map[2].as<uint16_t>()},
+        const TrunkMaps maps{{store_e1 ? e->grp.d_map[0].as<uint16_t>() : nullptr, e->grp.d_map[1].as<uint16_t>(), e->grp.d_map[2].as<uint16_t>()},
                              e->grp.d_e4.as<uint16_t>(), g.rows, e->d_zeros.as<uint16_t>(), e->grp.d_rowlist.as<uint8_t>()};
         const int n_tiles = g.tile_hi - g.tile_lo;
         for (int c = 0; c < 3; ++c) {
@@ -541,7 +544,7 @@
                 if (e->trunk_impl == 3)
                     launch_trunk3(e->stream, dm.k1, b->d_tiles.as<TrunkTile>() + g.tile_lo, n_tiles, n_views, c, b->d_rinfo.as<RInfo>(),
                                   b->d_bases.as<uint8_t>(), b->d_kin.as<uint32_t>(), b->d_sctx.as<uint8_t>(), b->total_bases, dm.w, maps, e->grp.d_dump.as<uint16_t>(),
-                                  b->d_totals.as<int32_t>() + TOT_LIST_STEPS, b->d_tcost.as<int32_t>() + g.cost_lo, e->num_cu, e->conv3_w16 != 0);
+                                  b->d_totals.as<int32_t>() + TOT_LIST_STEPS, b->d_tcost.as<int32_t>() + g.cost_lo, e->num_cu, e->conv3_w16 != 0, store_e1);
                 else if (e->trunk_impl)
                     launch_trunk2(e->stream, dm.k1, b->d_tiles.as<TrunkTile>() + g.tile_lo, n_tiles, n_views, c, b->d_rinfo.as<RInfo>(),
                                   b->d_bases.as<uint8_t>(), b->d_kin.as<uint32_t>(), b->d_sctx.as<uint8_t>(), dm.w, maps, e->num_cu,
@@ -553,9 +556,9 @@
             }
             {
                 Span sp(e, spans, K_EDGE, c);
-                if (e->edge_impl == 1)
+                if (e->edge_impl >= 1)
                     launch_edge2(e->stream, dm.k1, sr, b->d_rinfo.as<RInfo>(), b->d_bases.as<uint8_t>(), b->d_kin.as<uint32_t>(), dm.w,
-                                 maps, e->grp.d_edge4.as<uint16_t>(), e->grp.d_e4row.as<int32_t>(), e->num_cu);
+                                 maps, e->grp.d_edge4.as<uint16_t>(), e->grp.d_e4row.as<int32_t>(), e->num_cu, e->edge_impl == 2);
                 else
                     launch_edge(e->stream, dm.k1, sr, b->d_rinfo.as<RInfo>(), b->d_bases.as<uint8_t>(), b->d_kin.as<uint32_t>(), dm.w,
                                 maps, e->grp.d_edge4.as<uint16_t>(), e->grp.d_e4row.as<int32_t>(), e->num_cu);
@@ -822,7 +825,7 @@
         if (value < 1 || value > 1024) return fail(e, HM_EINVAL, "num_cu must be 1..1024");
         e->num_cu = (int)value;
     } else if (k == "edge_impl") {
-        if (value < 0 || value > 1) return fail(e, HM_EINVAL, "edge_impl must be 0 or 1");
+        if (value < 0 || value > 2) return fail(e, HM_EINVAL, "edge_impl must be 0, 1 or 2");
         e->edge_impl = (int)value;
     } else if (k == "tail_impl") {
         if (value < 0 || value > 3) return fail(e, HM_EINVAL, "tail_impl must be 0, 1, 2 or 3");
@@ -1124,6 +1127,21 @@
             logits[2 * i + 1] = lg[2 * u + 1];
         }
         return n;
+    });
+}
+
+int hm_debug_edge_rows(hm_engine_t* e, int64_t sites, uint16_t* rows) {
+    if (!e || sites < 0 || (sites > 0 && !rows)) return HM_EINVAL;
+    hm_batch* b = legacy(e);
+    if (!b->ran) return fail(e, HM_ESTATE, "hm_debug_edge_rows: hm_run first");
+    int rc = hm_sync(e);
+    if (rc < 0) return rc;
+    const size_t bytes = (size_t)sites * 4 * C4_CH * sizeof(uint16_t);
+    if (bytes > e->grp.d_edge4.cap) return fail(e, HM_EINVAL, "hm_debug_edge_rows: the edge-row buffer holds fewer sites");
+    if (sites == 0) return HM_OK;
+    return guarded(e, [&] {
+        HIP_TRY(hipMemcpy(rows, e->grp.d_edge4.p, bytes, hipMemcpyDeviceToHost));
+        return (int)HM_OK;
     });
 }
 
diff --git a/hifimeth_amd/csrc/hm_kernels.h b/hifimeth_amd/csrc/hm_kernels.h
--- a/hifimeth_amd/csrc/hm_kernels.h
+++ b/hifimeth_amd/csrc/hm_kernels.h
@@ -48,7 +48,7 @@
 void launch_edge(hipStream_t st, int k1, const SiteRange& sr, const RInfo* rinfo, const uint8_t* bases,
                  const uint32_t* kin, const CtxWeights& w, const TrunkMaps& maps, uint16_t* edge4, int32_t* e4row, int grid);
 void launch_edge2(hipStream_t st, int k1, const SiteRange& sr, const RInfo* rinfo, const uint8_t* bases, const uint32_t* kin,
-                  const CtxWeights& w, const TrunkMaps& maps, uint16_t* edge4, int32_t* e4row, int grid);
+                  const CtxWeights& w, const TrunkMaps& maps, uint16_t* edge4, int32_t* e4row, int grid, bool own_e1 = false);
 void launch_tail_gather(hipStream_t st, const SiteRange& sr, const CtxWeights& w, const TrunkMaps& maps, const uint16_t* edge4,
                         const int32_t* e4row, float* logits, float* p, uint8_t* ml, int grid);
 void launch_tail_gather_r(hipStream_t st, const SiteRange& sr, const CtxWeights& w, const TrunkMaps& maps, const uint16_t* edge4,
@@ -73,7 +73,7 @@
 size_t trunk3_dump_bytes(int grid);
 void launch_trunk3(hipStream_t st, int k1, const TrunkTile* tiles, int n_tiles, int n_views, int ctx, const RInfo* rinfo,
                    const uint8_t* bases, const uint32_t* kin, const uint8_t* sctx, int64_t n_bases, const CtxWeights& w, const TrunkMaps& maps,
-                   uint16_t* dump, int32_t* list_steps, const int32_t* tcost, int grid, bool w3_single = false);
+                   uint16_t* dump, int32_t* list_steps, const int32_t* tcost, int grid, bool w3_single = false, bool store_e1 = true);
 void launch_trunk_f32(hipStream_t st, int k1, const TrunkTile* tiles, int n_tiles, int n_views, int ctx, const RInfo* rinfo,
                       const uint8_t* bases, const uint32_t* kin, const uint8_t* sctx, const CtxWeights& w,
                       const TrunkMaps& maps, int grid);
diff --git a/hifimeth_amd/csrc/hm_trunk3.hip b/hifimeth_amd/csrc/hm_trunk3.hip
--- a/hifimeth_amd/csrc/hm_trunk3.hip
+++ b/hifimeth_amd/csrc/hm_trunk3.hip
@@ -237,7 +237,7 @@
     }
 }
 
-template <int K1, bool W3LO = true>
+template <int K1, bool W3LO = true, bool E1S = true>
 __global__ __launch_bounds__(256) __attribute__((amdgpu_waves_per_eu(1, 1)))
 void trunk3_kernel(const TrunkTile* __restrict__ tiles, int n_tiles, int n_views, int ctx, const RInfo* __restrict__ rinfo,
                    const uint8_t* __restrict__ bases, const uint32_t* __restrict__ kin, CtxWeights W, TrunkMaps mp, half_t* __restrict__ dump,
@@ -413,7 +413,7 @@
         }
         const int wn = cur_warm ? w : w + 1;
         const bool last = wn >= w1;
-        half_t* g1 = cur_calib ? dump_rows : reinterpret_cast<half_t*>(mp.e[0]) + (grow0 + T3_S2) * 256;
+        half_t* g1 = cur_calib || !E1S ? dump_rows : reinterpret_cast<half_t*>(mp.e[0]) + (grow0 + T3_S2) * 256;
         half_t* g2 = cur_calib ? dump_rows : reinterpret_cast<half_t*>(mp.e[1]) + (grow0 + T3_S3) * 256;
         half_t* g3 = cur_calib ? dump_rows : reinterpret_cast<half_t*>(mp.e[2]) + grow0 * 256;
         const uint8_t* rl = reinterpret_cast<const uint8_t*>(rlist[buf]);
@@ -452,7 +452,7 @@
                 }
             }
 #pragma unroll
-            for (int l = 0; l < 3; ++l) {
+            for (int l = E1S ? 0 : 1; l < 3; ++l) {
                 const uint8_t* rows = rl + 128 * l;
                 half_t* g = l == 0 ? g1 : l == 1 ? g2 : g3;
                 const int fill = first_new[l] + TR_OWN - 1, ch = t & 31;
@@ -507,7 +507,8 @@
         __syncthreads();
         TS(2);
         build_desc2(cur_warm, cur_calib != 0);
-        L2::run(a_hi, a_lo, wr, EpiTrunk3{b_hi + T3_H2 * TR_RS, b_lo + T3_H2 * TR_RS}, wf(2), W.bias[2], nt0, nt0, Cp23{{rl, g1}, (int)((cw >> 8) & 255)});
+        if constexpr (E1S) L2::run(a_hi, a_lo, wr, EpiTrunk3{b_hi + T3_H2 * TR_RS, b_lo + T3_H2 * TR_RS}, wf(2), W.bias[2], nt0, nt0, Cp23{{rl, g1}, (int)((cw >> 8) & 255)});
+        else L2::run(a_hi, a_lo, wr, EpiTrunk3{b_hi + T3_H2 * TR_RS, b_lo + T3_H2 * TR_RS}, wf(2), W.bias[2], nt0, nt0);
         move_rows<T3_H1, NW * 64>(h1_hi, h1_lo, a_hi + T3_M * TR_RS, a_lo + T3_M * TR_RS, threadIdx.x);
         TS(3);
         __syncthreads();
@@ -595,10 +596,20 @@
 
 void launch_trunk3(hipStream_t st, int k1, const TrunkTile* tiles, int n_tiles, int n_views, int ctx, const RInfo* rinfo,
                    const uint8_t* bases, const uint32_t* kin, const uint8_t* sctx, int64_t n_bases, const CtxWeights& w, const TrunkMaps& maps,
-                   uint16_t* dump, int32_t* list_steps, const int32_t* tcost, int grid, bool w3_single) {
+                   uint16_t* dump, int32_t* list_steps, const int32_t* tcost, int grid, bool w3_single, bool store_e1) {
     if (n_tiles <= 0) return;
     const int n_work = n_tiles * n_views;
     const dim3 g(min(n_work, grid));
+    if (!store_e1 && !w3_single) {
+        if (k1 == 11) {
+            hipLaunchKernelGGL(rowlist3_kernel<11>, dim3((2 * n_work + T3_RPB) / T3_RPB), dim3(64), 0, st, tiles, n_tiles, n_work, ctx, rinfo, sctx, n_bases, maps.rowlist);
+            hipLaunchKernelGGL((trunk3_kernel<11, true, false>), g, dim3(256), 0, st, tiles, n_tiles, n_views, ctx, rinfo, bases, kin, w, maps, reinterpret_cast<half_t*>(dump), list_steps, tcost);
+        } else {
+            hipLaunchKernelGGL(rowlist3_kernel<13>, dim3((2 * n_work + T3_RPB) / T3_RPB), dim3(64), 0, st, tiles, n_tiles, n_work, ctx, rinfo, sctx, n_bases, maps.rowlist);
+            hipLaunchKernelGGL((trunk3_kernel<13, true, false>), g, dim3(256), 0, st, tiles, n_tiles, n_views, ctx, rinfo, bases, kin, w, maps, reinterpret_cast<half_t*>(dump), list_steps, tcost);
+        }
+        return;
+    }
     if (k1 == 11) {
         hipLaunchKernelGGL(rowlist3_kernel<11>, dim3((2 * n_work + T3_RPB) / T3_RPB), dim3(64), 0, st, tiles, n_tiles, n_work, ctx, rinfo, sctx, n_bases, maps.rowlist);
         if (w3_single) hipLaunchKernelGGL((trunk3_kernel<11, false>), g, dim3(256), 0, st, tiles, n_tiles, n_views, ctx, rinfo, bases, kin, w, maps, reinterpret_cast<half_t*>(dump), list_steps, tcost);
diff --git a/include/hifimeth_hip.h b/include/hifimeth_hip.h
--- a/include/hifimeth_hip.h
+++ b/include/hifimeth_hip.h
@@ -96,6 +96,7 @@
 
 int64_t hm_scan_sites(hm_engine_t* e, int ctx, int32_t* read_id, int32_t* qoff, uint8_t* strand, int64_t cap);
 int64_t hm_site_logits(hm_engine_t* e, int ctx, float* logits, int64_t cap);
+int hm_debug_edge_rows(hm_engine_t* e, int64_t sites, uint16_t* rows);
 int hm_windows(hm_engine_t* e, int ctx, int64_t first, int64_t n, float* out_host);
 int hm_cnn_logits(hm_engine_t* e, int ctx, const float* windows, int64_t n, float* logits, float* p, uint8_t* ml);
 int64_t hm_debug_layer(hm_engine_t* e, int ctx, const float* window, int layer, float* out, int64_t cap);
```
